# sandyresearch/chipmunk

Measured on AMD Instinct MI355X. Metric: DiT denoise steps/sec at fixed sparsity, higher is better.
Workload: dtype bf16

## Files before the change

chipmunk_amd/_native.py:

```python
from __future__ import annotations

import ctypes
import os

_HERE = os.path.dirname(os.path.abspath(__file__))
LIB_PATH = os.environ.get("CHIPMUNK_HIP_LIB") or os.path.join(_HERE, "lib", "libchipmunk_hip.so")

SYMBOLS = [
    "chipmunk_last_error", "chipmunk_abi_version", "chipmunk_set_option", "chipmunk_set_random_seed",
    "chipmunk_csp_attn", "chipmunk_csp_attn_out", "chipmunk_csp_128_attn", "chipmunk_dense_attn", "chipmunk_dense_colsum_attn",
    "chipmunk_csp_mlp_mm1", "chipmunk_csp_mlp_mm1_scatter", "chipmunk_csp_mlp_mm1_fp8", "chipmunk_csp_mlp_mm2_and_scatter_add", "chipmunk_csp_scatter_add", "chipmunk_csp_mlp_mm2",
    "chipmunk_csp_mlp_mm1_ragged", "chipmunk_csp_mlp_mm1_scatter_ragged", "chipmunk_csp_mlp_mm1_fp8_ragged", "chipmunk_csp_mlp_mm2_ragged",
    "chipmunk_csp_mlp_mm2_and_scatter_add_ragged", "chipmunk_csp_scatter_add_ragged", "chipmunk_block_mean_ragged", "chipmunk_transpose16_pitched",
    "chipmunk_csp_mlp_mm1_batched", "chipmunk_csp_mlp_mm1_scatter_batched", "chipmunk_csp_mlp_mm1_fp8_batched", "chipmunk_csp_mlp_mm2_batched",
    "chipmunk_csp_mlp_mm2_and_scatter_add_batched", "chipmunk_csp_scatter_add_batched",
    "chipmunk_topk_indices", "chipmunk_topk_delta_indices", "chipmunk_topk_mask", "chipmunk_mask_to_indices", "chipmunk_mask_to_sorted_indices", "chipmunk_packed_mask_to_indices", "chipmunk_mask_row_counts", "chipmunk_mask_to_ragged_indices", "chipmunk_copy_indices",
    "chipmunk_bitpack", "chipmunk_bitunpack", "chipmunk_transpose16", "chipmunk_block_mean", "chipmunk_quantize_fp8", "chipmunk_gather_rows", "chipmunk_qkv_split_norm", "chipmunk_split_heads_rownorm", "chipmunk_dense_colsum_topk_mask", "chipmunk_dense_attn_strided", "chipmunk_csp_attn_out_ragged", "chipmunk_compact_indices", "chipmunk_residual_ln_modulate", "chipmunk_dense_colsum_attn_strided", "chipmunk_dense_colsum_topk_mask_strided", "chipmunk_release_scratch", "chipmunk_big_scratch_fallbacks",
    "chipmunk_host_alloc", "chipmunk_host_free", "chipmunk_copy_d2h_async", "chipmunk_copy_h2d_async", "chipmunk_host_bytes",
]

_lib = None


def lib() -> ctypes.CDLL:
    global _lib
    if _lib is None:
        if not os.path.exists(LIB_PATH):
            raise ImportError(
                f"{LIB_PATH} is missing: build it with `python -m chipmunk_amd.build` (hipcc --offload-arch=gfx950). "
                "chipmunk_amd has no CPU fallback.")
        _lib = ctypes.CDLL(LIB_PATH)
        _lib.chipmunk_last_error.restype = ctypes.c_char_p
        _lib.chipmunk_abi_version.restype = ctypes.c_int
        for item in filter(None, os.environ.get("CHIPMUNK_AMD_OPTIONS", "").split(",")):
            name, _, val = item.partition("=")
            if _lib.chipmunk_set_option(name.strip().encode(), int(val)) != 0:
                raise ValueError(f"CHIPMUNK_AMD_OPTIONS: {_lib.chipmunk_last_error().decode()}")
    return _lib


def last_error() -> str:
    return lib().chipmunk_last_error().decode()


def check(rc: int, what: str) -> None:
    if rc != 0:
        raise RuntimeError(f"{what}: {last_error()}")


def set_option(name: str, value: int) -> None:
    check(lib().chipmunk_set_option(name.encode(), int(value)), "chipmunk_set_option")


def manual_seed(seed: int) -> None:
    check(lib().chipmunk_set_random_seed(ctypes.c_uint64(int(seed) & 0xFFFFFFFFFFFFFFFF)), "chipmunk_set_random_seed")


class HostBuffer:

    def __init__(self, numel: int, dtype) -> None:
        import torch
        self.dtype = dtype
        self._numel = int(numel)
        self._itemsize = torch.empty(0, dtype=dtype).element_size()
        self.nbytes = self._numel * self._itemsize
        p = ctypes.c_void_p()
        check(lib().chipmunk_host_alloc(ctypes.c_size_t(max(self.nbytes, 1)), ctypes.byref(p)), "chipmunk_host_alloc")
        self.ptr = p.value

# ... 36 lines not shown
```

chipmunk_amd/csrc/attn.hip:

```cpp
#include "common.h"
#include "attn_params.h"
#include <type_traits>

namespace {

constexpr int QG = 192;
constexpr int QW = 48;
constexpr int KVT = 32;
constexpr int NST = 4;
constexpr int KRING = 8;
constexpr int HD = 128;
constexpr int TILE_BYTES = KVT * HD * 2;
constexpr float SCALE_LOG2E = 0.08838834764f * 1.44269504089f;
constexpr int NSTV = NST + 1;
constexpr int KEY_RING_OFF = (NST + NSTV) * TILE_BYTES;
constexpr int CS_OFF = KEY_RING_OFF + KRING * 256;
constexpr int ATTN_LDS_BYTES = CS_OFF + 2 * 2 * 4 * KVT * 4;

__device__ __forceinline__ f32x4 mfma16(bf16x8 a, bf16x8 b, f32x4 c) {
    return __builtin_amdgcn_mfma_f32_16x16x32_bf16(a, b, c, 0, 0, 0);
}

#ifdef ATTN_PROF
__device__ unsigned long long g_attn_prof[8 * 8];
// ... 1162 lines not shown
    p.B = B, p.H = H, p.Nq = Nq, p.Nk = Nk, p.G = (Nq + QG - 1) / QG;
    p.o_scale = 1.f;
    hipStream_t st = (hipStream_t)stream;
    int rc;
    if (chipmunk_get_option("attn_fused_colsum") == 5) {
        if (use_colsum64(B, H, Nq, Nk)) return chipmunk_colsum64_launch(p, st);
        return launch_attn<false, false, false, true>(p, st);
    }
    if (use_dense64(B, H, Nq, Nk)) {
        CM_CHECK((int64_t)Nk * p.ks[2] * 2 < (1ll << 32) && (int64_t)Nk * p.vs[2] * 2 < (1ll << 32),
                 "attention: one head's K or V spans more than 4 GiB (32-bit DMA offsets)");
        if (chipmunk_get_option("attn_fused_colsum") != 2) {
            int hc = H;
            uint16_t *part = nullptr;
            const int hc_min = chipmunk_get_option("attn_fused_colsum") == 4 ? 1 : 0;
            if (hc_min) hc = 1;
            for (; hc >= 1; hc /= 2) {
                part = (uint16_t *)chipmunk_big_scratch(st, chipmunk_colsum_part_bytes(hc == H ? B : 1, hc, Nq, Nk));
                if (part) break;
            }
            if (part && hc == H) return chipmunk_dense64_colsum_launch(p, part, st);
            if (part) {
                for (int b = 0; b < B; ++b)
                    for (int h0 = 0; h0 < H; h0 += hc) {
                        AttnParams c = p;
                        const int hn = H - h0 < hc ? H - h0 : hc;
                        const int64_t bh0 = (int64_t)b * H + h0;
                        c.q += b * p.qs[0] + h0 * p.qs[1], c.k += b * p.ks[0] + h0 * p.ks[1], c.v += b * p.vs[0] + h0 * p.vs[1];
                        c.o += b * p.os[0] + h0 * p.os[1];
                        c.l_out += bh0 * Nq, c.p_in += bh0 * Nq, c.cs += bh0 * p.G * (int64_t)cs_stride;
                        c.B = 1, c.H = hn;
                        if (int e = chipmunk_dense64_colsum_launch(c, part, st)) return e;
                    }
                return CHIPMUNK_OK;
            }
        }
        rc = chipmunk_dense64_launch(q, k, v, o, l, p.qs, p.ks, p.vs, p.os, B, H, Nq, Nk, st);
    } else {
        rc = launch_attn<false, false, true>(p, st);
    }
    if (rc != CHIPMUNK_OK) return rc;
    if (use_colsum64(B, H, Nq, Nk)) return chipmunk_colsum64_launch(p, st);
    return launch_attn<false, false, false, true>(p, st);
}

extern "C" int chipmunk_dense_colsum_attn(const void *q, const void *k, const void *v, const int64_t q_strides[3],
                                          const int64_t k_strides[3], const int64_t v_strides[3], const float *pin,
                                          void *o, void *cs, float *l, int B, int H, int Nq, int Nk, int cs_stride,
                                          void *stream) {
    return chipmunk_dense_colsum_attn_strided(q, k, v, q_strides, k_strides, v_strides, pin, o, nullptr, cs, l, B, H, Nq, Nk,
                                              cs_stride, stream);
}

extern "C" int chipmunk_dense_colsum_topk_mask_strided(const void *q, const void *k, const void *v, const int64_t q_strides[3],
                                               const int64_t k_strides[3], const int64_t v_strides[3], const float *pin, void *o,
                                               const int64_t *o_strides, float *l, int B, int H, int Nq, int Nk, const void *static_mask,
                                               int64_t static_stride, int static_rows, const void *group_flags, void *mask,
                                               int topk, double random_amount, void *stream) {
    if (int e = check_common(q, k, v, o, B, H, Nq, Nk)) return e;
    CM_CHECK(l && pin && mask, "dense_colsum_topk_mask: p / l / mask missing");
    if (int e = check_strides(q_strides, "q")) return e;
    if (int e = check_strides(k_strides, "k")) return e;
    if (int e = check_strides(v_strides, "v")) return e;
    hipStream_t st = (hipStream_t)stream;
    if (!use_dense64(B, H, Nq, Nk) || chipmunk_get_option("attn_fused_colsum") == 2 || (Nk & 3) || Nk > CHIPMUNK_TOPK_MASK_MAX_N)
        return CHIPMUNK_ERR_UNSUPPORTED;
    AttnParams p = {};
    p.q = (const uint16_t *)q, p.k = (const uint16_t *)k, p.v = (const uint16_t *)v, p.o = (uint16_t *)o;
    for (int i = 0; i < 3; ++i) p.qs[i] = q_strides[i], p.ks[i] = k_strides[i], p.vs[i] = v_strides[i];
    CM_CHECK((int64_t)Nk * p.ks[2] * 2 < (1ll << 32) && (int64_t)Nk * p.vs[2] * 2 < (1ll << 32),
             "attention: one head's K or V spans more than 4 GiB (32-bit DMA offsets)");
    if (int e = output_strides(p.os, o_strides, H, Nq)) return e;
    p.l_out = l, p.p_in = pin, p.cs = nullptr, p.cs_stride = 0;
    p.B = B, p.H = H, p.Nq = Nq, p.Nk = Nk, p.G = (Nq + QG - 1) / QG;
    p.o_scale = 1.f;
    uint16_t *part = (uint16_t *)chipmunk_big_scratch(st, chipmunk_colsum_part_bytes(B, H, Nq, Nk));
    if (!part) return CHIPMUNK_ERR_UNSUPPORTED;
    if (int e = chipmunk_dense64_colsum_launch(p, part, st)) return e;
    const int nrb = ((Nq + 255) / 256) * 2;
    return chipmunk_topk_mask_parts(part, chipmunk_colsum_part_stride(Nk), nrb, p.G, Nq, static_mask, static_stride, static_rows, group_flags, mask, B * H * p.G, Nk,
                                    topk, random_amount, st);
}

extern "C" int chipmunk_dense_colsum_topk_mask(const void *q, const void *k, const void *v, const int64_t q_strides[3],
                                               const int64_t k_strides[3], const int64_t v_strides[3], const float *pin, void *o,
                                               float *l, int B, int H, int Nq, int Nk, const void *static_mask,
                                               int64_t static_stride, int static_rows, const void *group_flags, void *mask,
                                               int topk, double random_amount, void *stream) {
    return chipmunk_dense_colsum_topk_mask_strided(q, k, v, q_strides, k_strides, v_strides, pin, o, nullptr, l, B, H, Nq, Nk,
                                                   static_mask, static_stride, static_rows, group_flags, mask, topk, random_amount,
                                                   stream);
}
```

chipmunk_amd/csrc/attn64.hip:

```cpp
#include "common.h"
#include "attn64_regs.h"
#include "attn_params.h"
#include "attn64_util.h"
#include <type_traits>

namespace {

constexpr int HD = 128;
constexpr int KT = 64;
constexpr int WROWS = 64, WGROWS = 256;
constexpr int TB = KT * HD * 2;
constexpr int NSL = 4;
constexpr int VRING = NSL * TB;
constexpr int LDS_BYTES = 2 * NSL * TB;
constexpr int PSTAGE = 64 * 128;
constexpr int LDS_BYTES_CSUM = LDS_BYTES + 4 * PSTAGE;
constexpr int CS_EXCH_BYTES = 2 * 4 * 64 * 4;
constexpr float SCALE_LOG2E = 0.08838834764f * 1.44269504089f;
constexpr float MAX_LAG = 4.0f;
#ifndef A64_ABL
#define A64_ABL 0
#endif
#ifndef A64_EB
#define A64_EB 20
#endif
#ifndef A64_EA
#define A64_EA 35
#endif
#ifndef A64_CSUM_VALU
#define A64_CSUM_VALU 1
#endif
#ifndef A64_VSPREAD
#define A64_VSPREAD 0
#endif
#ifndef A64_DMA_POS
#define A64_DMA_POS 2
#endif

constexpr int a64_ecum(int k) {
    return k <= 0 ? 0 : k <= 20 ? (k * A64_EB) / 20 : k <= 52 ? A64_EB + ((k - 20) * A64_EA) / 32
                                                              : (A64_EB + A64_EA + (k - 52) < 64 ? A64_EB + A64_EA + (k - 52) : 64);
}
constexpr int a64_cstep(int j) {
    int k = 0;
    while (a64_ecum(k) < 2 * j + 2) ++k;
    return k;
}
constexpr int a64_rk(int u) { return u == 0 ? 36 : u == 1 ? 38 : u == 2 ? 68 : 70; }
constexpr int a64_mk(int u) { return u == 0 ? 46 : u == 1 ? 48 : u == 2 ? 78 : 80; }

#ifdef ATTN64_PROF
__device__ unsigned long long g_a64_prof[4 * 8];
#define P64_DECL unsigned long long pt_ = 0, pacc_[7] = {0, 0, 0, 0, 0, 0, 0}; const bool prof_on_ = blockIdx.x == (gridDim.x / 2)
#define P64_START() do { if (prof_on_) pt_ = __builtin_amdgcn_s_memtime(); } while (0)
#define P64_MARK(i) do { if (prof_on_) { const unsigned long long n_ = __builtin_amdgcn_s_memtime(); pacc_[i] += n_ - pt_; pt_ = n_; } } while (0)
#define P64_END(w, n) do { if (prof_on_ && lane == 0) { for (int i_ = 0; i_ < 7; ++i_) g_a64_prof[(w) * 8 + i_] = pacc_[i_]; g_a64_prof[(w) * 8 + 7] = (n); } } while (0)
#else
#define P64_DECL
#define P64_START()
#define P64_MARK(i)
#define P64_END(w, n)
#endif

template <int KB, int QB, int KS>
__device__ __forceinline__ void mfma_qk(f32x16 &s) {
    constexpr int ka = 192 + (KB * 8 + KS) * 4, qa = 128 + (QB * 8 + KS) * 4;
    if constexpr (A64_ABL & 64) {
        constexpr int oa = (KB * 2 + QB) * 16;
        asm volatile("v_mfma_f32_32x32x16_bf16 a[%c0:%c1], a[%c2:%c3], a[%c4:%c5], a[%c0:%c1]" ::"i"(oa), "i"(oa + 15), "i"(ka), "i"(ka + 3), "i"(qa), "i"(qa + 3));
        return;
    }
    if constexpr (KS == 0)
        asm volatile("v_mfma_f32_32x32x16_bf16 %0, a[%c1:%c2], a[%c3:%c4], 0" : "=v"(s) : "i"(ka), "i"(ka + 3), "i"(qa), "i"(qa + 3));
    else
        asm volatile("v_mfma_f32_32x32x16_bf16 %0, a[%c1:%c2], a[%c3:%c4], %0" : "+v"(s) : "i"(ka), "i"(ka + 3), "i"(qa), "i"(qa + 3));
}
template <int QB, int DB>
__device__ __forceinline__ void mfma_pv(const u32x4 &vf, const u32x4 &pf) {
    constexpr int oa = (QB * 4 + DB) * 16;
    asm volatile("v_mfma_f32_32x32x16_bf16 a[%c2:%c3], %0, %1, a[%c2:%c3]" ::"v"(vf), "v"(pf), "i"(oa), "i"(oa + 15));
}
template <int KB, int KS, int SLOT>
__device__ __forceinline__ void lds_k(uint32_t addr) {
// ... 201 lines not shown

    if constexpr (!GATHER) {
        issue_k(0, 0);
        issue_k(1, 1), issue_v(0, 3);
        issue_k(2, 2), issue_v(0, 0);
        issue_k(3, 3), issue_v(1, 1);
        asm volatile("s_waitcnt vmcnt(24)" ::: "memory");
    }
    __syncthreads();
    static_for<0, 16>([&](auto i) {
        constexpr int I = decltype(i)::value;
        lds_k<(I >> 3), (I & 7), 0>(kad[I & 7]);
    });
    asm volatile("s_waitcnt lgkmcnt(0)" ::: "memory");

    f32x16 s[4];
    float px[64];
    uint32_t pw[2][4][4] = {};
    float m[2] = {-INFINITY, -INFINITY}, nmsc[2] = {0.f, 0.f};
    float mlag[2] = {-INFINITY, -INFINITY};
    float lacc[2][2] = {{0.f, 0.f}, {0.f, 0.f}};
    float alpha[2] = {1.f, 1.f};
    float wq[2] = {0.f, 0.f}, lpq[2] = {-1.0e30f, -1.0e30f}, c4[2] = {0.f, 0.f}, c5 = 0.f;
    uint32_t csoff = 0, ex_w = 0, ex_r = 0;
    int cs_extra = 0;
    float cs_own = 0.f;
    __amdgpu_buffer_rsrc_t prsrc = krsrc;
    uint32_t pst_w = 0, pst_r = 0, csoff_mx = 0;
    u32x2 csf[8] = {};
    f32x4 csacc[2] = {{0.f, 0.f, 0.f, 0.f}, {0.f, 0.f, 0.f, 0.f}};
    float csout = 0.f;
    u32x4 cs_ones = {0x3f803f80u, 0x3f803f80u, 0x3f803f80u, 0x3f803f80u};
    if constexpr (CSUM) {
        static_assert(A64_CSUM_VALU, "the matrix-pipe column-sum probe (A64_CSUM_VALU=0) fills all 160 KiB of LDS with its P stage: no room for the exchange area of the in-workgroup combine; build round 5's tree for it");
        pin(cs_ones);
        const uint32_t pst = lds0 + LDS_BYTES + (uint32_t)w * PSTAGE;
        pst_w = pst + l31 * 128 + ((uint32_t)(hf ^ (l31 & 7)) << 4);
        const int prow = lg * 4 + (l15 >> 2);
        pst_r = pst + prow * 128 + ((uint32_t)(((l15 & 3) >> 1) ^ (prow & 7)) << 4) + (l15 & 1) * 8;
        csoff_mx = 2u * (uint32_t)(16 * lg + 8 * ((l15 >> 2) & 1) + 4 * (l15 >> 3) + (l15 & 3));
#pragma unroll
        for (int qb = 0; qb < 2; ++qb) {
            const int qrow = row0 + qb * 32 + l31;
            const float pl = qrow < p.Nq ? p.p_in[(int64_t)bh * p.Nq + qrow] : 0.f;
            lpq[qb] = pl > 0.f ? __builtin_amdgcn_logf(pl) : -1.0e30f;
        }
        const int rr = ((lane >> 4) & 1) | (((lane >> 3) & 1) << 1) | (((lane >> 2) & 1) << 2);
        csoff = 2u * (uint32_t)(32 * (lane & 1) + (rr & 3) + 8 * (2 * ((lane >> 1) & 1) + (rr >> 2)) + 4 * hf);
        const int nA = 3 - (4 * g) % 3;
        const int lead = w < nA ? 0 : nA, members = w < nA ? nA : 4 - nA;
        cs_extra = w == lead ? members : 0;
        ex_w = lds0 + LDS_BYTES + (uint32_t)w * 256u + (uint32_t)lane * 4u;
        ex_r = lds0 + LDS_BYTES + (uint32_t)(lead + 1) * 256u + (uint32_t)lane * 4u;
        prsrc = make_rsrc(p.cs_part + ((int64_t)bh * (p.G * 2) + (g * 2 + (w < nA ? 0 : 1))) * p.cs_pstride);
    }
#pragma unroll
    for (int e = 0; e < 64; ++e) px[e] = e < 20 ? 0.f : -INFINITY;

    auto vfrag_read = [&](auto dbc, auto offc) __attribute__((always_inline)) {
        constexpr int DB = decltype(dbc)::value, OFF = decltype(offc)::value;
        u32x2 lo, hi;
        asm volatile("ds_read_b64_tr_b16 %0, %2 offset:%c3\n\tds_read_b64_tr_b16 %1, %2 offset:%c4"
                     : "=&v"(lo), "=&v"(hi) : "v"(vad[DB]), "i"(OFF), "i"(OFF + 2048) : "memory");
        return (u32x4){lo[0], lo[1], hi[0], hi[1]};
    };

    static_assert(64 - A64_EB - A64_EA >= 0 && 64 - A64_EB - A64_EA <= 9, "the last steps must finish before gap 12 of the next PV phase");
    auto ecum = [](int k) constexpr { return a64_ecum(k); };
    auto finish_step = [&](auto kk, auto uwc) __attribute__((always_inline)) {
        constexpr int K = decltype(kk)::value;
        constexpr bool UW = decltype(uwc)::value != 0;
        if constexpr (!(A64_ABL & 1)) {
            static_for<ecum(K), ecum(K + 1)>([&](auto ii) {
                constexpr int I = decltype(ii)::value;
                if constexpr (A64_ABL & 32) px[I] = px[I] * 0.5f;
                else px[I] = __builtin_amdgcn_exp2f(px[I]);
                pin(px[I]);
            });
            static_for<ecum(K - 1), ecum(K)>([&](auto ii) {
                constexpr int I = decltype(ii)::value;
                lacc[(I >> 3) & 1][I & 1] += px[I];
                pin(lacc[(I >> 3) & 1][I & 1]);
            });
            static_for<(ecum(K - 1) >> 1), (ecum(K) >> 1)>([&](auto jj) {
                constexpr int J = decltype(jj)::value, I = 2 * J;
                pw[(I >> 3) & 1][I >> 4][(I & 7) >> 1] = pack_bf16x2(px[I], px[I + 1]);
                pin(pw[(I >> 3) & 1][I >> 4][(I & 7) >> 1]);
            });
            if constexpr (CSUM && UW && !A64_CSUM_VALU) {
                static_assert(a64_cstep(8 * 1 + 7) + 1 < a64_rk(0) && a64_cstep(8 * 3 + 7) + 1 < a64_rk(2), "a unit is read after its second fragment is stored");
                static_for<0, 4>([&](auto uu) {
                    constexpr int U = decltype(uu)::value, S = (U & 1) * 4;
                    if constexpr (K == a64_mk(U) || K == a64_mk(U) + 1) {
                        constexpr int H2 = K - a64_mk(U);
                        if constexpr (H2 == 0 && (U & 1) == 0)
                            asm volatile("s_waitcnt lgkmcnt(0)" : "+v"(csf[0]), "+v"(csf[1]), "+v"(csf[2]), "+v"(csf[3]), "+v"(csf[4]), "+v"(csf[5]), "+v"(csf[6]), "+v"(csf[7]) :: "memory");
                        const u32x4 fr = {csf[S + 2 * H2][0], csf[S + 2 * H2][1], csf[S + 2 * H2 + 1][0], csf[S + 2 * H2 + 1][1]};
                        if constexpr (H2 == 0) asm volatile("v_mfma_f32_16x16x32_bf16 %0, %1, %2, 0" : "=&v"(csacc[U & 1]) : "v"(cs_ones), "v"(fr));
                        else asm volatile("v_mfma_f32_16x16x32_bf16 %0, %1, %2, %0" : "+v"(csacc[U & 1]) : "v"(cs_ones), "v"(fr));
                    }
                    if constexpr (K == a64_mk(U) + 3) {
                        if constexpr (U == 0) csout = csacc[0][0];
                        else csout = lg == U ? csacc[U & 1][0] : csout;
                        pin(csout);
                    }
                    if constexpr (K == a64_rk(U) || K == a64_rk(U) + 1) {
                        constexpr int H2 = K - a64_rk(U);
// ... 57 lines not shown
        constexpr int KNSL = (SL + 1) & 3;
        uint32_t ldsw = w * 4096, ksoff = 0, vsoff = 0;
        if constexpr (!(A64_ABL & 16)) {
            if constexpr (!(A64_ABL & 256) && !GATHER) asm volatile("s_waitcnt vmcnt(16)" ::: "memory");
            if constexpr (!(A64_ABL & 128)) __builtin_amdgcn_s_barrier();
            if constexpr (!GATHER) {
                asm volatile("" : "+s"(ldsw));
                ksoff = (uint32_t)tile_base(t + 4) * kstride_b;
                vsoff = (uint32_t)tile_base(t + 2) * vstride_b;
            }
        }
        __builtin_amdgcn_sched_barrier(0);
        P64_MARK(0);

        u32x4 vf[16];
        static_for<0, 32>([&](auto gg) {
            constexpr int G = decltype(gg)::value;
            constexpr int ks = G >> 2, kb = (G >> 1) & 1, qb = G & 1;
            mfma_qk<kb, qb, ks>(s[kb * 2 + qb]);
            if constexpr (!(A64_ABL & 16) && !GATHER && ((A64_DMA_POS == 0 && G < 8) || (A64_DMA_POS == 2 && G >= 16 && (G & 1) == 0))) {
                constexpr int PC = A64_DMA_POS == 0 ? G : (G - 16) >> 1;
                if constexpr (PC < 4) issue_k1(ksoff, ldsw, SL, PC);
                else issue_v1(vsoff, ldsw, (SL + 2) & 3, PC - 4);
            }
            finish_step(ic<20 + G>{}, uwc);
            if constexpr (A64_VSPREAD ? (G & 1) == 0 : G < 16) {
                constexpr int f = A64_VSPREAD ? G >> 1 : G;
                if constexpr (A64_ABL & 4) vf[f] = (u32x4){(uint32_t)t, 1u, 2u, 3u};
                else vf[f] = vfrag_read(ic<(f & 3)>{}, ic<VSL * TB + (f >> 2) * 4096>{});
            }
            __builtin_amdgcn_sched_barrier(0);
        });
        P64_MARK(1);
        asm volatile("s_waitcnt lgkmcnt(0)"
                     : "+v"(vf[0]), "+v"(vf[1]), "+v"(vf[2]), "+v"(vf[3]), "+v"(vf[4]), "+v"(vf[5]), "+v"(vf[6]), "+v"(vf[7]), "+v"(vf[8]),
                       "+v"(vf[9]), "+v"(vf[10]), "+v"(vf[11]), "+v"(vf[12]), "+v"(vf[13]), "+v"(vf[14]), "+v"(vf[15]));
        __builtin_amdgcn_sched_barrier(0);
        P64_MARK(2);

        float mx[2];
        bool moved = false;
        const int dead = GATHER ? 0 : (t * KT - tile_base(t) < KT ? t * KT - tile_base(t) : KT);
        const int vleft = !GATHER ? KT : (t < ntiles ? valid - (tbeg + t) * KT : 0);
        auto phase_b_gap = [&](auto gg) __attribute__((always_inline)) {
            constexpr int G = decltype(gg)::value;
            constexpr int up = G >> 3, db = (G >> 1) & 3, qb = G & 1;
            const u32x4 pf = {pw[qb][up][0], pw[qb][up][1], pw[qb][up][2], pw[qb][up][3]};
            mfma_pv<qb, db>(vf[G >> 1], pf);
            constexpr bool UWT = decltype(uwc)::value != 0 && !A64_CSUM_VALU;
            if constexpr (G < (CSUM ? (UWT ? 32 : 17) : 12)) finish_step(ic<52 + G>{}, uwc);
            if constexpr (CSUM && G == (UWT ? 31 : 17)) {
                const uint32_t par2 = (uint32_t)(t & 1) * 1024u;
                const float mine = UWT ? csout : c5;
                if (!cs_extra) {
                    asm volatile("ds_write_b32 %0, %1" ::"v"(ex_w + (par2 ^ 1024u)), "v"(mine) : "memory");
                } else {
                    float x1 = 0.f, x2 = 0.f;
                    if (cs_extra >= 2) asm volatile("ds_read_b32 %0, %1" : "=v"(x1) : "v"(ex_r + par2) : "memory");
                    if (cs_extra >= 3) asm volatile("ds_read_b32 %0, %1 offset:256" : "=v"(x2) : "v"(ex_r + par2) : "memory");
                    asm volatile("ds_write_b32 %0, %1" ::"v"(ex_w + (par2 ^ 1024u)), "v"(mine) : "memory");
                    asm volatile("s_waitcnt lgkmcnt(1)" : "+v"(x1), "+v"(x2)::"memory");
                    const int tb2 = tile_base(t - 2), dd = (t - 2) * KT - tb2;
                    if (t > 1 && dd < KT) {
                        const uint32_t off = UWT ? csoff_mx : csoff;
                        if (dd <= 0 || (int)(off >> 1) >= dd) {
                            const uint16_t val = (uint16_t)(pack_bf16x2((cs_own + x1) + x2, 0.f) & 0xffffu);
                            if (p.probe & 16) __builtin_amdgcn_raw_buffer_store_b16(val, prsrc, off, (uint32_t)tb2 * 2u, 2);
                            else __builtin_amdgcn_raw_buffer_store_b16(val, prsrc, off, (uint32_t)tb2 * 2u, 0);
                        }
                    }
                }
                cs_own = mine;
            }
            if constexpr (!(A64_ABL & 16) && !GATHER && A64_DMA_POS == 1 && G >= 16 && (G & 1) == 0) {
                constexpr int PC = (G - 16) >> 1;
                if constexpr (PC < 4) issue_k1(ksoff, ldsw, SL, PC);
                else issue_v1(vsoff, ldsw, (SL + 2) & 3, PC - 4);
            }
            if constexpr (G < 16 && !(A64_ABL & 8)) {
                constexpr int J = G;
                lds_k<(J >> 3), (J & 7), KNSL>(kad[J & 7]);
            }
            if constexpr (G == 1 && !(A64_ABL & 2)) {
                if (!GATHER && __builtin_expect(dead > 0, 0)) {
                    int thr = dead - 4 * hf;
                    asm volatile("" : "+v"(thr));
#pragma unroll
                    for (int blk = 0; blk < 4; ++blk)
#pragma unroll
                        for (int r = 0; r < 16; ++r)
                            if ((blk >> 1) * 32 + (r & 3) + 8 * (r >> 2) < thr) s[blk][r] = -INFINITY;
                }
                if (GATHER && __builtin_expect(vleft < KT, 0)) {
                    int thr = vleft - hf;
                    asm volatile("" : "+v"(thr));
#pragma unroll
                    for (int blk = 0; blk < 4; ++blk)
#pragma unroll
                        for (int r = 0; r < 16; ++r)
                            if ((r & 3) * 16 + (blk >> 1) * 8 + 2 * (r >> 2) >= thr) s[blk][r] = -INFINITY;
                }
            }
            if constexpr (G >= 2 && G <= 9 && !(A64_ABL & 2) && !NOMAX) {
                constexpr int j = G - 2;
                constexpr int kb2 = j >> 2, r0 = (j & 3) * 4;
                if constexpr (j == 0)
                    asm volatile("v_max_f32 %0, %2, %3\n\tv_max_f32 %1, %6, %7\n\tv_max3_f32 %0, %0, %4, %5\n\tv_max3_f32 %1, %1, %8, %9"
                                 : "=&v"(mx[0]), "=&v"(mx[1])
                                 : "v"(s[0][0]), "v"(s[0][1]), "v"(s[0][2]), "v"(s[0][3]), "v"(s[1][0]), "v"(s[1][1]), "v"(s[1][2]), "v"(s[1][3]));
                else
                asm volatile("v_max3_f32 %0, %0, %2, %3\n\tv_max3_f32 %1, %1, %6, %7\n\tv_max3_f32 %0, %0, %4, %5\n\tv_max3_f32 %1, %1, %8, %9"
                             : "+v"(mx[0]), "+v"(mx[1])
                             : "v"(s[kb2 * 2][r0]), "v"(s[kb2 * 2][r0 + 1]), "v"(s[kb2 * 2][r0 + 2]), "v"(s[kb2 * 2][r0 + 3]),
                               "v"(s[kb2 * 2 + 1][r0]), "v"(s[kb2 * 2 + 1][r0 + 1]), "v"(s[kb2 * 2 + 1][r0 + 2]), "v"(s[kb2 * 2 + 1][r0 + 3]));
            }
            if constexpr (G == 10 && !(A64_ABL & 2) && !NOMAX) {
#pragma unroll
                for (int q2 = 0; q2 < 2; ++q2) {
                    float a = mx[q2], c = mx[q2];
                    lane_swap32(a, c);
                    mx[q2] = max2(a, c);
                    pin(mx[q2]);
                }
            }
// ... 311 lines not shown
        uint32_t ldsw = w * 4096;
        asm volatile("" : "+s"(ldsw));
        const uint32_t ksoff = (uint32_t)tile_base(t + 4) * kstride_b;
        __builtin_amdgcn_sched_barrier(0);
        static_for<0, 6>([&](auto qq) {
            constexpr int QB = decltype(qq)::value;
            constexpr int PP = SL * 6 + QB;
            constexpr int BUF = PP % 3, B1 = (PP + 2) % 3, B2 = (PP + 1) % 3;
            static_for<0, 16>([&](auto gg) {
                constexpr int G = decltype(gg)::value, ks = G >> 1, kb = G & 1;
                mfma_cs<QB, kb, ks>(s[BUF][kb], offs[QB]);
                if constexpr (QB == 0 && G >= 8 && G < 12) issue_k1(ksoff, ldsw, SL, G - 8);
                if constexpr (QB == 5 && kb == 1) {
                    lds_k<0, ks, KNSL>(kad[ks]);
                    lds_k<1, ks, KNSL>(kad[ks]);
                }
                constexpr int TP1 = QB == 0 ? TP ^ 1 : TP, TP2 = QB <= 1 ? TP ^ 1 : TP;
                if constexpr (G > 2) drain2(ic<B1>{}, ic<TP1>{}, ic<(G - 2) * 2>{}, ic<TP1>{}, ic<(G - 3) * 2>{});
                else if constexpr (G == 2) drain2(ic<B1>{}, ic<TP1>{}, ic<0>{}, ic<TP2>{}, ic<30>{});
                else if constexpr (G == 1) drain2(ic<B2>{}, ic<TP2>{}, ic<30>{}, ic<TP2>{}, ic<28>{});
                else drain2(ic<B2>{}, ic<TP2>{}, ic<28>{}, ic<TP2>{}, ic<26>{});
                if constexpr (QB == 1 && G == 3) {
                    float a = cacc[TP ^ 1][0], c = cacc[TP ^ 1][1];
                    lane_swap32(a, c);
                    const float tot = a + c;
                    cacc[TP ^ 1][0] = 0.f, cacc[TP ^ 1][1] = 0.f;
                    if (g < p.G && t > 0)
                    {
                        const uint32_t u = __float_as_uint(tot);
                        const uint32_t rne = (u + 0x7fffu + ((u >> 16) & 1u)) >> 16, qn = (u >> 16) | 0x0040u;
                        p.cs[((int64_t)bh * p.G + g) * p.cs_stride + tile_base(t - 1) + lane] = (uint16_t)((u & 0x7fffffffu) > 0x7f800000u ? qn : rne);
                    }
                }
                __builtin_amdgcn_sched_barrier(0);
            });
        });
        asm volatile("s_waitcnt lgkmcnt(0)" ::: "memory");
        __builtin_amdgcn_sched_barrier(0);
    };
    for (int tb = 0;; tb += 4) {
        tile(ic<0>{}, tb);
        if (tb >= T4) break;
        tile(ic<1>{}, tb + 1);
        tile(ic<2>{}, tb + 2);
        tile(ic<3>{}, tb + 3);
    }
    asm volatile("s_waitcnt vmcnt(0)" ::: "memory");
}

template <int MODE>
int launch64(const AttnParams &p, int64_t grid, hipStream_t stream) {
    auto kern = attn64_kernel<MODE>;
    static uint64_t lds_set = 0;
    constexpr int LDS = (MODE == 3 && !A64_CSUM_VALU) ? LDS_BYTES_CSUM + CS_EXCH_BYTES : MODE == 3 ? LDS_BYTES + CS_EXCH_BYTES : LDS_BYTES;
    ensure_dynamic_lds((const void *)kern, LDS, lds_set);
    hipLaunchKernelGGL(kern, dim3((unsigned)grid), dim3(256), LDS, stream, p);
    CM_LAUNCH_CHECK();
    return CHIPMUNK_OK;
}

}

#ifdef ATTN64_PROF
extern "C" int chipmunk_attn64_prof_read(unsigned long long *out) {
    return hipMemcpyFromSymbol(out, HIP_SYMBOL(g_a64_prof), sizeof(g_a64_prof)) == hipSuccess ? 0 : 2;
}
#endif

const float *chipmunk_knorm_max(const uint16_t *k, const int64_t ks[3], int B, int H, int Nk, hipStream_t stream) {
    if (chipmunk_get_option("attn_nomax") == 2 || (size_t)B * H * sizeof(float) > (32 << 10)) return nullptr;
    unsigned char *sc = (unsigned char *)chipmunk_scratch(stream, 64 << 10);
    if (!sc) return nullptr;
    float *km = (float *)(sc + (32 << 10));
    if (hipMemsetAsync(km, 0, (size_t)B * H * sizeof(float), stream) != hipSuccess) return nullptr;
    hipLaunchKernelGGL(knorm_max_kernel, dim3(Nk >= 4096 ? 64 : 8, B * H), dim3(256), 0, stream, k, ks[0], ks[1], ks[2], H, Nk, km);
    return km;
}

int chipmunk_dense64_launch(const void *q, const void *k, const void *v, void *o, float *l, const int64_t qs[3],
                            const int64_t ks[3], const int64_t vs[3], const int64_t os[3], int B, int H, int Nq, int Nk,
                            hipStream_t stream) {
    AttnParams p = {};
    p.q = (const uint16_t *)q, p.k = (const uint16_t *)k, p.v = (const uint16_t *)v, p.o = (uint16_t *)o;
    for (int i = 0; i < 3; ++i) p.qs[i] = qs[i], p.ks[i] = ks[i], p.vs[i] = vs[i], p.os[i] = os[i];
    p.l_out = l;
    p.B = B, p.H = H, p.Nq = Nq, p.Nk = Nk, p.G = (Nq + WGROWS - 1) / WGROWS;
    p.o_scale = 1.f;
    p.kmax = chipmunk_knorm_max(p.k, ks, B, H, Nk, stream);
    return launch64<0>(p, (int64_t)B * H * p.G, stream);
}

namespace {
__global__ __launch_bounds__(256) void cs_combine_kernel(const uint16_t *part, int pstride, uint16_t *cs, int NRB, int G, int Nq, int Nk, int cs_stride) {
    const int g = blockIdx.y, bh = blockIdx.z;
    int r0, r1;
    const int nrows = colsum_part_rows(g, NRB / 2, r0, r1);
    const uint16_t *src = part + ((int64_t)bh * NRB + r0) * pstride;
    const int64_t row1 = (int64_t)(r1 - r0) * pstride;
    uint16_t *dst = cs + ((int64_t)bh * G + g) * cs_stride;
    if (((Nk | cs_stride) & 3) == 0) {
        const int j = (blockIdx.x * 256 + threadIdx.x) * 4;
        if (j >= Nk) return;
        float acc[4];
        {
            const u32x2 x = *(const u32x2 *)(src + j);
            acc[0] = __uint_as_float(x[0] << 16), acc[1] = __uint_as_float(x[0] & 0xffff0000u);
            acc[2] = __uint_as_float(x[1] << 16), acc[3] = __uint_as_float(x[1] & 0xffff0000u);
        }
        if (nrows == 2) {
            const u32x2 x = *(const u32x2 *)(src + row1 + j);
            acc[0] += __uint_as_float(x[0] << 16), acc[1] += __uint_as_float(x[0] & 0xffff0000u);
            acc[2] += __uint_as_float(x[1] << 16), acc[3] += __uint_as_float(x[1] & 0xffff0000u);
        }
        *(u32x2 *)(dst + j) = (u32x2){pack_bf16x2(acc[0], acc[1]), pack_bf16x2(acc[2], acc[3])};
    } else {
        for (int e = 0; e < 4; ++e) {
            const int j = (blockIdx.x * 256 + threadIdx.x) * 4 + e;
            if (j >= Nk) return;
            float acc = bf16_bits_to_f32(src[j]);
            if (nrows == 2) acc += bf16_bits_to_f32(src[row1 + j]);
            dst[j] = f32_to_bf16_bits(acc);
        }
    }
}
}

int chipmunk_colsum64_launch(const AttnParams &p, hipStream_t stream) {
    static uint64_t lds_set = 0;
    ensure_dynamic_lds((const void *)colsum64_kernel, NSL * TB, lds_set);
    const int64_t grid = (int64_t)p.B * p.H * ((p.G + 3) / 4);
    hipLaunchKernelGGL(colsum64_kernel, dim3((unsigned)grid), dim3(256), NSL * TB, stream, p);
    CM_LAUNCH_CHECK();
    return CHIPMUNK_OK;
}

int chipmunk_colsum_part_stride(int Nk) { return (chipmunk_get_option("attn_cs_probe") & 1) ? Nk : (Nk + 63) & ~63; }

size_t chipmunk_colsum_part_bytes(int B, int H, int Nq, int Nk) {
    return (size_t)B * H * (((Nq + WGROWS - 1) / WGROWS) * 2) * (size_t)chipmunk_colsum_part_stride(Nk) * sizeof(uint16_t);
}

int chipmunk_dense64_colsum_launch(const AttnParams &p0, uint16_t *part, hipStream_t stream) {
    AttnParams p = p0;
    const int G192 = p.G;
    p.G = (p.Nq + WGROWS - 1) / WGROWS;
    p.cs_part = part, p.cs_pstride = chipmunk_colsum_part_stride(p.Nk);
    if (chipmunk_get_option("attn_cs_probe") & 2) p.probe |= 16;
    if (chipmunk_get_option("attn_fused_colsum") == 3) p.probe |= 4;
    p.kmax = chipmunk_knorm_max(p.k, p.ks, p.B, p.H, p.Nk, stream);
    if (int rc = launch64<3>(p, (int64_t)p.B * p.H * p.G, stream)) return rc;
    if (!p.cs) return CHIPMUNK_OK;
    hipLaunchKernelGGL(cs_combine_kernel, dim3((unsigned)((p.Nk + 1023) / 1024), (unsigned)G192, (unsigned)(p.B * p.H)), dim3(256), 0, stream,
                       part, p.cs_pstride, p.cs, p.G * 2, G192, p.Nq, p.Nk, p.cs_stride);
    CM_LAUNCH_CHECK();
    return CHIPMUNK_OK;
}

int chipmunk_csp64_launch(const AttnParams &p, int inplace, int grid, hipStream_t stream) {
    CM_CHECK(p.plan && p.tickets && p.ws, "csp64: work plan missing");
    return inplace ? launch64<2>(p, grid, stream) : launch64<1>(p, grid, stream);
}
```

chipmunk_amd/csrc/attn_params.h:

```cpp
#pragma once
#include <stdint.h>
#include <hip/hip_runtime.h>

struct AttnParams {
    const uint16_t *q, *k, *v;
    uint16_t *o;
    const uint16_t *o_in;
    int64_t qs[3], ks[3], vs[3], os[3];
    const int32_t *indices, *counts;
    const int64_t *idx_off;
    float *l_out;
    const float *p_in;
    uint16_t *cs;
    int cs_stride;
    int B, H, Nq, Nk, G, idx_stride;
    float o_scale;
    int split_full, nsplit;
    float *ws;
    int32_t *tickets;
    const int32_t *plan;
    int xcd_chunks;
    const float *kmax;
    uint16_t *cs_part;
    int cs_pstride;
    int probe;
};


int chipmunk_csp64_launch(const AttnParams &p, int inplace, int grid, hipStream_t stream);
int chipmunk_dense64_colsum_launch(const AttnParams &p, uint16_t *part, hipStream_t stream);
int chipmunk_topk_mask_parts(const uint16_t *part, int part_stride, int nrb, int groups_per_bh, int Nq, const void *static_mask, int64_t static_stride,
                             int static_rows, const void *group_flags, void *mask, int rows, int n, int k, double random_amount,
                             hipStream_t stream);
size_t chipmunk_colsum_part_bytes(int B, int H, int Nq, int Nk);
int chipmunk_colsum_part_stride(int Nk);
int chipmunk_colsum64_launch(const AttnParams &p, hipStream_t stream);
int chipmunk_csp96_launch(const AttnParams &p, int inplace, int grid, hipStream_t stream);
const float *chipmunk_knorm_max(const uint16_t *k, const int64_t ks[3], int B, int H, int Nk, hipStream_t stream);

__host__ __device__ inline int colsum_part_rows(int j, int nwg, int &r0, int &r1) {
    const int a = (3 * j) >> 2, w0 = 3 * j - 4 * a;
    r0 = 2 * a + (w0 ? 1 : 0);
    r1 = 2 * (a + 1);
    return (w0 >= 2 && a + 1 < nwg) ? 2 : 1;
}

struct IndexRow {
    const int32_t *ptr;
    int width;
};
__device__ __forceinline__ IndexRow index_row(const AttnParams &p, int64_t item) {
    if (p.idx_off) {
        const int64_t o = p.idx_off[item];
        return {p.indices + o, (int)(p.idx_off[item + 1] - o)};
    }
    return {p.indices + item * p.idx_stride, p.idx_stride};
}
```

chipmunk_amd/csrc/indexed_io.hip:

```cpp
#include "common.h"
#include "attn_params.h"

namespace {

__device__ __forceinline__ uint32_t wave_incl_scan(uint32_t x) {
    x += (uint32_t)__builtin_amdgcn_update_dpp(0, (int)x, 0x111, 0xf, 0xf, true);
    x += (uint32_t)__builtin_amdgcn_update_dpp(0, (int)x, 0x112, 0xf, 0xf, true);
    x += (uint32_t)__builtin_amdgcn_update_dpp(0, (int)x, 0x114, 0xf, 0xf, true);
    x += (uint32_t)__builtin_amdgcn_update_dpp(0, (int)x, 0x118, 0xf, 0xf, true);
    x += (uint32_t)__builtin_amdgcn_update_dpp(0, (int)x, 0x142, 0xa, 0xf, false);
    x += (uint32_t)__builtin_amdgcn_update_dpp(0, (int)x, 0x143, 0xc, 0xf, false);
    return x;
}
struct M2IParams {
    const uint8_t *mask;
    int32_t *indices;
    int32_t *counts;
    int n, pad_n, multiple_of;
    const int64_t *offsets;
};

template <bool PACKED, bool SORTED = false, bool RAGGED = false>
__global__ __launch_bounds__(256) void mask_to_indices_kernel(const M2IParams p) {
    extern __shared__ __attribute__((aligned(16))) unsigned char smem[];
// ... 485 lines not shown
    int32_t *dst = flat + o;
    const int width = (int)(offsets[r + 1] - o);
    int c = counts[r];
    c = c < 0 ? 0 : (c < width ? c : width);
    c = c < idx_stride ? c : (int)idx_stride;
    if ((((uintptr_t)src | (uintptr_t)dst) & 15) == 0) {
        const int c4 = c >> 2;
        for (int i = threadIdx.x; i < c4; i += 256) ((u32x4 *)dst)[i] = ((const u32x4 *)src)[i];
        for (int i = (c4 << 2) + threadIdx.x; i < c; i += 256) dst[i] = src[i];
    } else {
        for (int i = threadIdx.x; i < c; i += 256) dst[i] = src[i];
    }
    for (int i = c + threadIdx.x; i < width; i += 256) dst[i] = 0;
}

size_t m2i_lds_bytes(int n, bool sorted) {
    const int NI = (n + 31) >> 5, NB = (NI + 63) >> 6;
    if (sorted) return (size_t)NB * 64 * 4 + (size_t)(NB + 1) * 4 + 16;
    return (size_t)NB * 64 * 4 + (size_t)32 * NB * 8 + (size_t)32 * NB * 4 + 33 * 4 + 16;
}

template <bool PACKED, bool SORTED = false, bool RAGGED = false>
int launch_m2i(const void *mask, int32_t *indices, int32_t *counts, int64_t rows, int n, int pad_n, int multiple_of,
               void *stream, const int64_t *offsets = nullptr) {
    CM_CHECK(mask && indices && (RAGGED ? (const void *)offsets : (const void *)counts), "mask_to_indices: null pointer");
    CM_CHECK(rows >= 0 && n > 0 && pad_n >= n && multiple_of > 0, "mask_to_indices: bad sizes rows=%lld n=%d pad_n=%d multiple_of=%d",
             (long long)rows, n, pad_n, multiple_of);
    CM_CHECK(rows < (1ll << 31), "mask_to_indices: too many rows");
    if (PACKED) CM_CHECK(n % 8 == 0, "packed_mask_to_indices: n must be a multiple of 8 (got %d)", n);
    const size_t lds = m2i_lds_bytes(n, SORTED);
    CM_CHECK(lds <= 160 * 1024, "mask_to_indices: row length %d needs %zu B of LDS (> 160 KiB)", n, lds);
    if (rows == 0) return CHIPMUNK_OK;
    auto kern = mask_to_indices_kernel<PACKED, SORTED, RAGGED>;
    if (lds > 64 * 1024) (void)hipFuncSetAttribute((const void *)kern, hipFuncAttributeMaxDynamicSharedMemorySize, (int)lds);
    M2IParams p = {(const uint8_t *)mask, indices, counts, n, pad_n, multiple_of, offsets};
    hipLaunchKernelGGL(kern, dim3((unsigned)rows), dim3(256), lds, (hipStream_t)stream, p);
    CM_LAUNCH_CHECK();
    return CHIPMUNK_OK;
}


struct TopkMaskParams {
    const uint16_t *cs;
    const uint8_t *stat;
    const uint8_t *groups;
    uint8_t *mask;
    int64_t cs_stride, stat_stride;
    int rows, n, k, stat_rows;
    float random_amount;
    uint32_t salt;
    const uint16_t *parts;
    int64_t pstride;
    int nrb, ngroups, nq;
};

__device__ __forceinline__ uint32_t bf16_key(uint32_t u) {
    return (u & 0x8000u) ? (~u & 0xffffu) : (u | 0x8000u);
}

template <int KPT, bool ALIGNED, bool PARTS = false>
__global__ __launch_bounds__(1024) void topk_mask_kernel(const TopkMaskParams p) {
    constexpr int NV = KPT / 4;
    __shared__ int wave_cnt[16];
    const int tid = threadIdx.x, lane = tid & 63, w = tid >> 6;
    const int row = blockIdx.x;
    const int n = p.n;
    const uint16_t *x = nullptr;
    int prow = 1;
    int64_t row1 = 0;
    if constexpr (PARTS) {
        const int bh = row / p.ngroups, g = row - bh * p.ngroups;
        int r0, r1;
        prow = colsum_part_rows(g, p.nrb / 2, r0, r1);
        x = p.parts + ((int64_t)bh * p.nrb + r0) * p.pstride;
        row1 = (int64_t)(r1 - r0) * p.pstride;
    } else {
        x = p.cs + (int64_t)row * p.cs_stride;
    }
    const uint32_t lane_off8 = 8u * (uint32_t)tid;
    const uint32_t lane_off4 = 4u * (uint32_t)tid;
    uint32_t key[NV][2];
    constexpr int LB = NV % 10 == 0 ? 10 : (NV % 8 == 0 ? 8 : (NV % 6 == 0 ? 6 : 4));
    static_assert(NV % LB == 0, "NV must split into whole load batches");
#pragma unroll
    for (int j0 = 0; j0 < NV; j0 += LB) {
        uint32_t raw[LB][2];
#pragma unroll
        for (int jj = 0; jj < LB; ++jj) {
            const int c = 4 * tid + 4096 * (j0 + jj);
            uint32_t v0 = 0xffffffffu, v1 = 0xffffffffu;
            if constexpr (ALIGNED) {
                if (c < n) {
                    const u32x2 v = *(const u32x2 *)((const unsigned char *)(x + 4096 * (j0 + jj)) + lane_off8);
                    v0 = v[0], v1 = v[1];
                    if constexpr (PARTS) {
                        if (prow == 2) {
                            float a0 = __uint_as_float(v0 << 16), a1 = __uint_as_float(v0 & 0xffff0000u);
                            float a2 = __uint_as_float(v1 << 16), a3 = __uint_as_float(v1 & 0xffff0000u);
                            const u32x2 y = *(const u32x2 *)((const unsigned char *)(x + row1 + 4096 * (j0 + jj)) + lane_off8);
                            a0 += __uint_as_float(y[0] << 16), a1 += __uint_as_float(y[0] & 0xffff0000u);
                            a2 += __uint_as_float(y[1] << 16), a3 += __uint_as_float(y[1] & 0xffff0000u);
                            v0 = pack_bf16x2(a0, a1), v1 = pack_bf16x2(a2, a3);
                        }
                    }
                }
            } else if (c < n) {
                v0 = v1 = 0;
#pragma unroll
                for (int e = 0; e < 4; ++e) {
                    const uint32_t u = c + e < n ? x[c + e] : 0xffffu;
                    if (e < 2) v0 |= u << (16 * e);
                    else v1 |= u << (16 * (e - 2));
                }
            }
// ... 28 lines not shown
            const uint32_t cm1 = (cand - 1u) | ((cand - 1u) << 16);
            const uint32_t one2 = 0x00010001u;
            uint32_t cnt2 = 0;
#pragma unroll
            for (int j = 0; j < NV; ++j)
#pragma unroll
                for (int h = 0; h < 2; ++h) {
                    uint32_t d;
                    asm volatile("v_pk_sub_u16 %0, %1, %2 clamp\n\tv_pk_min_u16 %0, %0, %3" : "=&v"(d) : "v"(key[j][h]), "v"(cm1), "v"(one2));
                    asm volatile("v_pk_add_u16 %0, %0, %1" : "+v"(cnt2) : "v"(d));
                }
            const int mine = (int)(cnt2 & 0xffffu) + (int)(cnt2 >> 16);
            if (block_count(mine) >= k) res = cand;
        }
        thr = res;
        int gt = 0;
#pragma unroll
        for (int j = 0; j < NV; ++j)
#pragma unroll
            for (int h = 0; h < 2; ++h) {
                uint32_t kw = key[j][h];
                asm volatile("" : "+v"(kw));
                gt += ((kw & 0xffffu) > thr ? 1 : 0) + ((kw >> 16) > thr ? 1 : 0);
            }
        ties_to_take = k - block_count(gt);
    }
    int my_ties = 0;
    if (ties_to_take > 0) {
#pragma unroll
        for (int j = 0; j < NV; ++j)
#pragma unroll
            for (int h = 0; h < 2; ++h) {
                uint32_t kw = key[j][h];
                asm volatile("" : "+v"(kw));
                my_ties += ((kw & 0xffffu) == thr ? 1 : 0) + ((kw >> 16) == thr ? 1 : 0);
            }
    }
    int tie_budget = 0;
    {
        int incl = my_ties;
#pragma unroll
        for (int d = 1; d < 64; d <<= 1) {
            const int o = __shfl_up(incl, d);
            if (lane >= d) incl += o;
        }
        if (lane == 63) wave_cnt[w] = incl;
        __syncthreads();
        int before = incl - my_ties;
#pragma unroll
        for (int i = 0; i < 16; ++i) before += i < w ? wave_cnt[i] : 0;
        __syncthreads();
        tie_budget = ties_to_take - before;
    }
    uint8_t *out = p.mask + (int64_t)row * n;
    const uint8_t *st = p.stat ? p.stat + (int64_t)(row % p.stat_rows) * p.stat_stride : nullptr;
    const bool rnd = active && p.random_amount > 0.f;
    auto combined4 = [&](int c0, uint32_t &v0, uint32_t &v1) {
        const u32x2 v = *(const u32x2 *)(x + c0);
        v0 = v[0], v1 = v[1];
        if constexpr (PARTS) {
            float a0 = __uint_as_float(v0 << 16), a1 = __uint_as_float(v0 & 0xffff0000u);
            float a2 = __uint_as_float(v1 << 16), a3 = __uint_as_float(v1 & 0xffff0000u);
            if (prow == 2) {
                const u32x2 y = *(const u32x2 *)(x + row1 + c0);
                a0 += __uint_as_float(y[0] << 16), a1 += __uint_as_float(y[0] & 0xffff0000u);
                a2 += __uint_as_float(y[1] << 16), a3 += __uint_as_float(y[1] & 0xffff0000u);
            }
            v0 = pack_bf16x2(a0, a1), v1 = pack_bf16x2(a2, a3);
        }
    };
    uint32_t first = x[0];
    if constexpr (PARTS) {
        uint32_t f0, f1;
        combined4(0, f0, f1);
        first = f0 & 0xffffu;
    }
    const uint32_t salt = p.salt ^ (first * 0x27D4EB2Fu);
    const int nsteps = (n + 4095) / 4096;
    auto emit = [&](auto keyed, int c, uint32_t v0, uint32_t v1, uint32_t sb) {
        uint32_t bytes = 0;
        if constexpr (decltype(keyed)::value) asm volatile("" : "+v"(v0), "+v"(v1));
#pragma unroll
        for (int e = 0; e < 4; ++e) {
            const uint32_t half = ((e < 2 ? v0 : v1) >> (16 * (e & 1))) & 0xffffu;
            const uint32_t kv = decltype(keyed)::value ? half : bf16_key(half);
            bool keep = kv > thr;
            const bool tie = kv == thr && tie_budget > 0 && c + e < n;
            tie_budget -= tie ? 1 : 0;
            keep = keep || tie;
            if (rnd && !keep) keep = hash_uniform(row, c + e, salt) < p.random_amount;
            keep = keep || ((sb >> (8 * e)) & 0xffu) != 0;
            bytes |= (keep ? 1u : 0u) << (8 * e);
        }
        if constexpr (ALIGNED) {
            *(uint32_t *)(out + c) = bytes;
        } else {
#pragma unroll
            for (int e = 0; e < 4; ++e)
                if (c + e < n) out[c + e] = (uint8_t)(bytes >> (8 * e));
        }
    };
    if constexpr (ALIGNED) {
        constexpr int OB = 5;
#pragma unroll
        for (int j0 = 0; j0 < NV; j0 += OB) {
            uint32_t sbv[OB];
#pragma unroll
            for (int jj = 0; jj < OB; ++jj) {
                const int c = 4 * tid + 4096 * (j0 + jj);
                sbv[jj] = (j0 + jj < NV && st && c < n) ? *(const uint32_t *)(st + c) : 0u;
            }
            __builtin_amdgcn_sched_barrier(0);
#pragma unroll
            for (int jj = 0; jj < OB; ++jj) {
                if constexpr (true) {
                    const int c = 4 * tid + 4096 * (j0 + jj);
                    if (j0 + jj < NV && c < n) emit(std::integral_constant<int, 1>{}, c, key[(j0 + jj) < NV ? (j0 + jj) : 0][0], key[(j0 + jj) < NV ? (j0 + jj) : 0][1], sbv[jj]);
                    asm volatile("" ::: "memory");
                }
            }
            __builtin_amdgcn_sched_barrier(0);
        }
    } else {
        for (int j = 0; j < nsteps; ++j) {
            const int c = 4 * tid + 4096 * j;
            if (c >= n) break;
            uint32_t v0 = 0, v1 = 0, sb = 0;
#pragma unroll
            for (int e = 0; e < 4; ++e) {
                const uint32_t u = c + e < n ? x[c + e] : 0xffffu;
                if (e < 2) v0 |= u << (16 * e);
                else v1 |= u << (16 * (e - 2));
                if (st && c + e < n) sb |= (uint32_t)st[c + e] << (8 * e);
            }
            emit(std::integral_constant<int, 0>{}, c, v0, v1, sb);
        }
    }
}

__device__ __forceinline__ uint32_t bf16_key2(uint32_t u) {
    uint32_t s;
    const uint32_t fifteen2 = 0x000f000fu;
    asm("v_pk_ashrrev_i16 %0, %1, %2" : "=v"(s) : "v"(fifteen2), "v"(u));
    return u ^ (s | 0x80008000u);
}

template <bool ALIGNED, bool PARTS>
__global__ __launch_bounds__(1024) void topk_mask_stream_kernel(const TopkMaskParams p) {
    __shared__ int wave_cnt[16];
    const int tid = threadIdx.x, lane = tid & 63, w = tid >> 6;
    const int row = blockIdx.x;
    const int n = p.n;
    const uint16_t *x = nullptr;
    int prow = 1;
    int64_t row1 = 0;
    if constexpr (PARTS) {
        const int bh = row / p.ngroups, g = row - bh * p.ngroups;
        int r0, r1;
        prow = colsum_part_rows(g, p.nrb / 2, r0, r1);
        x = p.parts + ((int64_t)bh * p.nrb + r0) * p.pstride;
        row1 = (int64_t)(r1 - r0) * p.pstride;
    } else {
        x = p.cs + (int64_t)row * p.cs_stride;
    }
    const uint32_t lane_off8 = 8u * (uint32_t)tid;
    const int nsteps = (n + 4095) / 4096;
    const bool active = p.groups == nullptr || p.groups[row] != 0;
    const int k = p.k < n ? p.k : n;
    const bool select = active && k > 0;
    const bool rnd = active && p.random_amount > 0.f;

    auto combined4 = [&](int c0, uint32_t &v0, uint32_t &v1) {
        const u32x2 v = *(const u32x2 *)(x + c0);
        v0 = v[0], v1 = v[1];
        if constexpr (PARTS) {
            if (prow == 2) {
                float a0 = __uint_as_float(v0 << 16), a1 = __uint_as_float(v0 & 0xffff0000u);
                float a2 = __uint_as_float(v1 << 16), a3 = __uint_as_float(v1 & 0xffff0000u);
                const u32x2 y = *(const u32x2 *)(x + row1 + c0);
                a0 += __uint_as_float(y[0] << 16), a1 += __uint_as_float(y[0] & 0xffff0000u);
                a2 += __uint_as_float(y[1] << 16), a3 += __uint_as_float(y[1] & 0xffff0000u);
                v0 = pack_bf16x2(a0, a1), v1 = pack_bf16x2(a2, a3);
            }
        }
    };
    uint32_t first = 0;
    if (rnd) {
        first = x[0];
        if constexpr (PARTS) {
            uint32_t f0, f1;
            combined4(0, f0, f1);
            first = f0 & 0xffffu;
        }
    }
    const uint32_t salt = p.salt ^ (first * 0x27D4EB2Fu);
    if constexpr (PARTS) {
        __syncthreads();
        if (select) {
            uint16_t *xk = const_cast<uint16_t *>(x);
            for (int j = 0; j < nsteps; ++j) {
                const int c = 4 * tid + 4096 * j;
// ... 55 lines not shown
            for (int j0 = 0; j0 < nsteps; j0 += U) {
                uint32_t kw[U][2];
#pragma unroll
                for (int jj = 0; jj < U; ++jj) load_raw(j0 + jj, kw[jj][0], kw[jj][1]);
#pragma unroll
                for (int jj = 0; jj < U; ++jj) {
                    to_keys(kw[jj][0], kw[jj][1]);
#pragma unroll
                    for (int h = 0; h < 2; ++h) {
                        uint32_t d;
                        asm volatile("v_pk_sub_u16 %0, %1, %2 clamp\n\tv_pk_min_u16 %0, %0, %3" : "=&v"(d) : "v"(kw[jj][h]), "v"(cm1), "v"(one2));
                        asm volatile("v_pk_add_u16 %0, %0, %1" : "+v"(cnt2) : "v"(d));
                    }
                }
            }
            const int mine = (int)(cnt2 & 0xffffu) + (int)(cnt2 >> 16);
            if (block_count(mine) >= k) res = cand;
        }
        thr = res;
        int gt = 0;
        for (int j0 = 0; j0 < nsteps; j0 += U) {
            uint32_t kw[U][2];
#pragma unroll
            for (int jj = 0; jj < U; ++jj) load_raw(j0 + jj, kw[jj][0], kw[jj][1]);
#pragma unroll
            for (int jj = 0; jj < U; ++jj) {
                to_keys(kw[jj][0], kw[jj][1]);
#pragma unroll
                for (int h = 0; h < 2; ++h) {
                    const uint32_t lo = kw[jj][h] & 0xffffu, hi = kw[jj][h] >> 16;
                    gt += (lo > thr ? 1 : 0) + (hi > thr ? 1 : 0);
                    my_ties += (lo == thr ? 1 : 0) + (hi == thr ? 1 : 0);
                }
            }
        }
        ties_to_take = k - block_count(gt);
    }
    int tie_budget = 0;
    {
        int incl = my_ties;
#pragma unroll
        for (int d = 1; d < 64; d <<= 1) {
            const int o = __shfl_up(incl, d);
            if (lane >= d) incl += o;
        }
        if (lane == 63) wave_cnt[w] = incl;
        __syncthreads();
        int before = incl - my_ties;
#pragma unroll
        for (int i = 0; i < 16; ++i) before += i < w ? wave_cnt[i] : 0;
        __syncthreads();
        tie_budget = ties_to_take - before;
    }
    uint8_t *out = p.mask + (int64_t)row * n;
    const uint8_t *st = p.stat ? p.stat + (int64_t)(row % p.stat_rows) * p.stat_stride : nullptr;
    for (int j0 = 0; j0 < nsteps; j0 += U) {
        uint32_t kw[U][2], sbv[U];
#pragma unroll
        for (int jj = 0; jj < U; ++jj) {
            const int c = 4 * tid + 4096 * (j0 + jj);
            kw[jj][0] = kw[jj][1] = 0;
            if (select) load_raw(j0 + jj, kw[jj][0], kw[jj][1]);
            sbv[jj] = 0;
            if constexpr (ALIGNED) {
                if (st && c < n) sbv[jj] = *(const uint32_t *)(st + c);
            } else if (st) {
#pragma unroll
                for (int e = 0; e < 4; ++e)
                    if (c + e < n) sbv[jj] |= (uint32_t)st[c + e] << (8 * e);
            }
        }
#pragma unroll
        for (int jj = 0; jj < U; ++jj) {
            const int c = 4 * tid + 4096 * (j0 + jj);
            if (c >= n) continue;
            if (select) to_keys(kw[jj][0], kw[jj][1]);
            uint32_t bytes = 0;
#pragma unroll
            for (int e = 0; e < 4; ++e) {
                const uint32_t kv = (kw[jj][e >> 1] >> (16 * (e & 1))) & 0xffffu;
                bool keep = kv > thr;
                const bool tie = kv == thr && tie_budget > 0 && c + e < n;
                tie_budget -= tie ? 1 : 0;
                keep = keep || tie;
                if (rnd && !keep) keep = hash_uniform(row, c + e, salt) < p.random_amount;
                keep = keep || ((sbv[jj] >> (8 * e)) & 0xffu) != 0;
                bytes |= (keep ? 1u : 0u) << (8 * e);
            }
            if constexpr (ALIGNED) {
                *(uint32_t *)(out + c) = bytes;
            } else {
#pragma unroll
                for (int e = 0; e < 4; ++e)
                    if (c + e < n) out[c + e] = (uint8_t)(bytes >> (8 * e));
            }
        }
    }
}

}

extern "C" int chipmunk_mask_to_indices(const void *mask, int32_t *indices, int32_t *counts, int64_t rows, int n,
                                        int pad_n, int multiple_of, void *stream) {
    return launch_m2i<false>(mask, indices, counts, rows, n, pad_n, multiple_of, stream);
}

extern "C" int chipmunk_packed_mask_to_indices(const void *packed, int32_t *indices, int32_t *counts, int64_t rows,
                                               int n, int pad_n, int multiple_of, void *stream) {
    return launch_m2i<true>(packed, indices, counts, rows, n, pad_n, multiple_of, stream);
}

static int launch_topk(const void *activation, void *cache, int dtype, int32_t *indices, int32_t *counts, int rows,
                       int cols, double sparsity_amount, int multiple_of, double random_amount, void *stream) {
    CM_CHECK(activation && indices && counts, "topk_indices: null pointer");
    CM_CHECK(rows >= 0 && cols >= 1024, "topk_indices: rows >= 0 and cols >= 1024 required (the quantile is taken over the first 1024 columns); got rows=%d cols=%d", rows, cols);
    CM_CHECK(multiple_of > 0, "topk_indices: multiple_of must be positive");
    CM_CHECK(sparsity_amount >= 0.0 && sparsity_amount <= 1.0, "topk_indices: sparsity_amount must be in [0,1]");
    if (rows == 0) return CHIPMUNK_OK;
    TopkParams p = {activation, cache, indices, counts, rows, cols, multiple_of, (float)sparsity_amount, (float)random_amount,
                    random_amount > 0.0 ? chipmunk_next_random_salt() : 0u};
    hipStream_t s = (hipStream_t)stream;
#define LAUNCH_TOPK(T)                                                                                           \
    do {                                                                                                         \
        if (cache) hipLaunchKernelGGL((topk_indices_kernel<T, true>), dim3(rows), dim3(1024), 0, s, p);          \
        else hipLaunchKernelGGL((topk_indices_kernel<T, false>), dim3(rows), dim3(1024), 0, s, p);               \
    } while (0)
    switch (dtype) {
        case CHIPMUNK_DTYPE_BF16: LAUNCH_TOPK(uint16_t); break;
        case CHIPMUNK_DTYPE_FP16: LAUNCH_TOPK(_Float16); break;
        case CHIPMUNK_DTYPE_FP32: LAUNCH_TOPK(float); break;
        default: CM_CHECK(false, "topk_indices: unsupported dtype code %d", dtype);
    }
#undef LAUNCH_TOPK
    CM_LAUNCH_CHECK();
    return CHIPMUNK_OK;
}

extern "C" int chipmunk_mask_to_sorted_indices(const void *mask, int packed, int32_t *indices, int32_t *counts,
                                               int64_t rows, int n, int pad_n, int multiple_of, void *stream) {
    return packed ? launch_m2i<true, true>(mask, indices, counts, rows, n, pad_n, multiple_of, stream)
                  : launch_m2i<false, true>(mask, indices, counts, rows, n, pad_n, multiple_of, stream);
}

extern "C" int chipmunk_mask_row_counts(const void *mask, int packed, int32_t *counts, int64_t *lengths, int64_t rows, int n,
                                        int pad_n, int multiple_of, void *stream) {
    CM_CHECK(mask && counts && lengths, "mask_row_counts: null pointer");
    CM_CHECK(rows >= 0 && n > 0 && pad_n >= n && multiple_of > 0, "mask_row_counts: bad sizes rows=%lld n=%d pad_n=%d multiple_of=%d",
             (long long)rows, n, pad_n, multiple_of);
    CM_CHECK(rows < (1ll << 31), "mask_row_counts: too many rows");
// ... 75 lines not shown

extern "C" int chipmunk_transpose16(const void *src, void *dst, int B, int R, int C, void *stream) {
    CM_CHECK(src && dst && B > 0 && R > 0 && C > 0, "transpose16: bad arguments");
    CM_CHECK((C & 7) == 0 || true, "unreachable");
    hipLaunchKernelGGL(transpose16_kernel, dim3((C + 63) / 64, (R + 63) / 64, B), dim3(256), 0, (hipStream_t)stream,
                       (const uint16_t *)src, (uint16_t *)dst, R, C, R);
    CM_LAUNCH_CHECK();
    return CHIPMUNK_OK;
}

extern "C" int chipmunk_transpose16_pitched(const void *src, void *dst, int B, int R, int C, int ld, void *stream) {
    CM_CHECK(src && dst && B > 0 && R > 0 && C > 0, "transpose16: bad arguments");
    CM_CHECK(ld >= R, "transpose16: the output pitch ld (%d) must be at least R (%d)", ld, R);
    hipLaunchKernelGGL(transpose16_kernel, dim3((C + 63) / 64, (ld + 63) / 64, B), dim3(256), 0, (hipStream_t)stream,
                       (const uint16_t *)src, (uint16_t *)dst, R, C, ld);
    CM_LAUNCH_CHECK();
    return CHIPMUNK_OK;
}

template <typename V>
__global__ __launch_bounds__(256) void gather_rows_kernel(const V *src, V *dst, const int32_t *map, int64_t n_out,
                                                          int64_t n_src, int64_t cpr, int64_t total) {
    for (int64_t idx = (int64_t)blockIdx.x * 256 + threadIdx.x; idx < total; idx += (int64_t)gridDim.x * 256) {
        const int64_t row = idx / cpr, c = idx - row * cpr;
        const int64_t o = row / n_out, r = row - o * n_out;
        dst[idx] = src[(o * n_src + map[r]) * cpr + c];
    }
}

extern "C" int chipmunk_gather_rows(const void *src, void *dst, const int32_t *map, int64_t outer, int64_t n_src,
                                    int64_t n_out, int64_t row_bytes, void *stream) {
    CM_CHECK(src && dst && map, "gather_rows: null pointer");
    CM_CHECK(outer >= 0 && n_src > 0 && n_out >= 0 && row_bytes > 0, "gather_rows: bad sizes");
    if (outer == 0 || n_out == 0) return CHIPMUNK_OK;
    hipStream_t s = (hipStream_t)stream;
    const uintptr_t align = (uintptr_t)src | (uintptr_t)dst | (uintptr_t)row_bytes;
#define LAUNCH_GATHER(V)                                                                                              \
    do {                                                                                                              \
        const int64_t cpr = row_bytes / (int64_t)sizeof(V), total = outer * n_out * cpr;                               \
        const int64_t blocks = (total + 255) / 256;                                                                    \
        hipLaunchKernelGGL((gather_rows_kernel<V>), dim3((unsigned)(blocks > 65536 * 16 ? 65536 * 16 : blocks)),       \
                           dim3(256), 0, s, (const V *)src, (V *)dst, map, n_out, n_src, cpr, total);                  \
    } while (0)
    if ((align & 15) == 0) LAUNCH_GATHER(u32x4);
    else if ((align & 3) == 0) LAUNCH_GATHER(uint32_t);
    else if ((align & 1) == 0) LAUNCH_GATHER(uint16_t);
    else LAUNCH_GATHER(uint8_t);
#undef LAUNCH_GATHER
    CM_LAUNCH_CHECK();
    return CHIPMUNK_OK;
}

int chipmunk_topk_mask_parts(const uint16_t *part, int part_stride, int nrb, int groups_per_bh, int Nq, const void *static_mask, int64_t static_stride,
                             int static_rows, const void *group_flags, void *mask, int rows, int n, int k, double random_amount,
                             hipStream_t s) {
    CM_CHECK(part && mask && rows >= 0 && n > 0 && (n & 3) == 0 && n <= CHIPMUNK_TOPK_MASK_MAX_N && k >= 0 && part_stride >= n && (part_stride & 3) == 0, "topk_mask_parts: bad arguments");
    CM_CHECK(!static_mask || (static_rows > 0 && static_stride >= n && (static_stride & 3) == 0 && ((uintptr_t)static_mask & 3) == 0),
             "topk_mask_parts: bad static mask geometry");
    CM_CHECK(((uintptr_t)mask & 3) == 0 && ((uintptr_t)part & 7) == 0, "topk_mask_parts: unaligned buffers");
    if (rows == 0) return CHIPMUNK_OK;
    TopkMaskParams p = {nullptr, (const uint8_t *)static_mask, (const uint8_t *)group_flags, (uint8_t *)mask, 0, static_stride,
                        rows, n, k, static_mask ? static_rows : 1, (float)random_amount,
                        random_amount > 0.0 ? chipmunk_next_random_salt() : 0u};
    p.parts = part, p.pstride = part_stride, p.nrb = nrb, p.ngroups = groups_per_bh, p.nq = Nq;
    if (n > 1024 * 120 || chipmunk_get_option("topk_mask_stream") == 1) hipLaunchKernelGGL((topk_mask_stream_kernel<true, true>), dim3(rows), dim3(1024), 0, s, p);
    else if (n <= 1024 * 16) hipLaunchKernelGGL((topk_mask_kernel<16, true, true>), dim3(rows), dim3(1024), 0, s, p);
    else if (n <= 1024 * 48) hipLaunchKernelGGL((topk_mask_kernel<48, true, true>), dim3(rows), dim3(1024), 0, s, p);
    else hipLaunchKernelGGL((topk_mask_kernel<120, true, true>), dim3(rows), dim3(1024), 0, s, p);
    CM_LAUNCH_CHECK();
    return CHIPMUNK_OK;
}

__global__ __launch_bounds__(256) void qkv_split_norm_kernel(const uint16_t *qkv, int64_t row_stride, const uint16_t *qw,
                                                             const uint16_t *kw, uint16_t *q, uint16_t *k, uint16_t *v, int64_t n,
                                                             int H, float eps, int64_t segments, const float *fcos, const float *fsin,
                                                             int64_t rope_rows) {
    const int l15 = threadIdx.x & 15;
    u32x4 wq = {0x3f803f80u, 0x3f803f80u, 0x3f803f80u, 0x3f803f80u}, wk = wq;
    if (qw) wq = *(const u32x4 *)(qw + l15 * 8);
    if (kw) wk = *(const u32x4 *)(kw + l15 * 8);
    for (int64_t seg = ((int64_t)blockIdx.x * 256 + threadIdx.x) >> 4; seg < segments; seg += ((int64_t)gridDim.x * 256) >> 4) {
        const int64_t tok = seg / (3 * H);
        const int rem = (int)(seg - tok * 3 * H), which = rem / H, h = rem - which * H;
        u32x4 x = *(const u32x4 *)(qkv + tok * row_stride + (int64_t)rem * 128 + l15 * 8);
        uint16_t *dst = (which == 0 ? q : which == 1 ? k : v) + ((int64_t)h * n + tok) * 128 + l15 * 8;
        if (which < 2) {
            float f[8], ss = 0.f;
#pragma unroll
            for (int e = 0; e < 4; ++e) {
                f[2 * e] = __uint_as_float(x[e] << 16), f[2 * e + 1] = __uint_as_float(x[e] & 0xffff0000u);
                ss = __builtin_fmaf(f[2 * e], f[2 * e], ss);
                ss = __builtin_fmaf(f[2 * e + 1], f[2 * e + 1], ss);
            }
            ss = row16_sum(ss);
            const float r = 1.0f / __builtin_sqrtf(ss * (1.0f / 128.0f) + eps);
            const u32x4 w = which == 0 ? wq : wk;
#pragma unroll
            for (int e = 0; e < 4; ++e) {
                float a = f[2 * e] * r, b = f[2 * e + 1] * r;
                round_bf16_pair(a, b);
                x[e] = pack_bf16x2(a * __uint_as_float(w[e] << 16), b * __uint_as_float(w[e] & 0xffff0000u));
            }
            if (fcos && tok < rope_rows) {
                const f32x4 c0 = *(const f32x4 *)(fcos + tok * 128 + l15 * 8), c1 = *(const f32x4 *)(fcos + tok * 128 + l15 * 8 + 4);
                const f32x4 s0 = *(const f32x4 *)(fsin + tok * 128 + l15 * 8), s1 = *(const f32x4 *)(fsin + tok * 128 + l15 * 8 + 4);
#pragma unroll
                for (int e = 0; e < 4; ++e) {
                    const float re = __uint_as_float(x[e] << 16), im = __uint_as_float(x[e] & 0xffff0000u);
                    const float cr = e < 2 ? c0[2 * e] : c1[2 * e - 4], ci = e < 2 ? c0[2 * e + 1] : c1[2 * e - 3];
                    const float sr = e < 2 ? s0[2 * e] : s1[2 * e - 4], si = e < 2 ? s0[2 * e + 1] : s1[2 * e - 3];
                    x[e] = pack_bf16x2(re * cr + (-im) * sr, im * ci + re * si);
                }
            }
        }
        *(u32x4 *)dst = x;
    }
}

extern "C" int chipmunk_qkv_split_norm(const void *qkv, int64_t row_stride, const void *q_weight, const void *k_weight, void *q,
                                       void *k, void *v, int64_t n, int heads, float eps, const float *freqs_cos,
                                       const float *freqs_sin, int64_t rope_rows, void *stream) {
    CM_CHECK(qkv && q && k && v, "qkv_split_norm: null pointer");
    CM_CHECK(n >= 0 && heads > 0 && row_stride >= (int64_t)3 * heads * 128, "qkv_split_norm: bad sizes");
    CM_CHECK((((uintptr_t)qkv | (uintptr_t)q | (uintptr_t)k | (uintptr_t)v | (uintptr_t)q_weight | (uintptr_t)k_weight) & 15) == 0 &&
                 (row_stride & 7) == 0 && (((uintptr_t)freqs_cos | (uintptr_t)freqs_sin) & 15) == 0,
             "qkv_split_norm: pointers and the row stride must be 16-byte aligned");
    CM_CHECK((freqs_cos == nullptr) == (freqs_sin == nullptr) && rope_rows >= 0 && rope_rows <= n, "qkv_split_norm: bad rotary arguments");
    if (n == 0) return CHIPMUNK_OK;
    const int64_t segments = n * 3 * heads, blocks = (segments + 15) / 16;
    hipLaunchKernelGGL(qkv_split_norm_kernel, dim3((unsigned)(blocks > 256 * 64 ? 256 * 64 : blocks)), dim3(256), 0, (hipStream_t)stream,
                       (const uint16_t *)qkv, row_stride, (const uint16_t *)q_weight, (const uint16_t *)k_weight, (uint16_t *)q,
                       (uint16_t *)k, (uint16_t *)v, n, heads, eps, segments, freqs_cos, freqs_sin, freqs_cos ? rope_rows : 0);
    CM_LAUNCH_CHECK();
    return CHIPMUNK_OK;
}

extern "C" int chipmunk_topk_mask(const void *cs, int64_t cs_stride, const void *static_mask, int64_t static_stride,
                                  int static_rows, const void *group_flags, void *mask, int rows, int n, int k,
                                  double random_amount, void *stream) {
    CM_CHECK(cs && mask, "topk_mask: null pointer");
    CM_CHECK(rows >= 0 && n > 0 && k >= 0, "topk_mask: bad sizes (rows=%d n=%d k=%d)", rows, n, k);
    CM_CHECK(cs_stride >= n, "topk_mask: cs row stride %lld < n %d", (long long)cs_stride, n);
    CM_CHECK(n <= CHIPMUNK_TOPK_MASK_MAX_N, "topk_mask: rows of more than %d columns are not supported (got %d)", CHIPMUNK_TOPK_MASK_MAX_N, n);
    CM_CHECK(!static_mask || (static_rows > 0 && static_stride >= n), "topk_mask: bad static mask geometry");
    CM_CHECK(random_amount >= 0.0 && random_amount <= 1.0, "topk_mask: random_amount must be in [0,1]");
    if (rows == 0) return CHIPMUNK_OK;
    TopkMaskParams p = {(const uint16_t *)cs, (const uint8_t *)static_mask, (const uint8_t *)group_flags, (uint8_t *)mask,
                        cs_stride, static_stride, rows, n, k, static_mask ? static_rows : 1, (float)random_amount,
                        random_amount > 0.0 ? chipmunk_next_random_salt() : 0u};
    hipStream_t s = (hipStream_t)stream;
    const bool aligned = n % 4 == 0 && (((uintptr_t)cs) & 7) == 0 && (cs_stride * 2) % 8 == 0 && (((uintptr_t)mask) & 3) == 0 &&
                         (!static_mask || ((((uintptr_t)static_mask) & 3) == 0 && static_stride % 4 == 0));
#define LAUNCH_TM(KPT)                                                                                       \
    do {                                                                                                     \
        if (aligned) hipLaunchKernelGGL((topk_mask_kernel<KPT, true>), dim3(rows), dim3(1024), 0, s, p);     \
        else hipLaunchKernelGGL((topk_mask_kernel<KPT, false>), dim3(rows), dim3(1024), 0, s, p);            \
    } while (0)
    if (n > 1024 * 120 || chipmunk_get_option("topk_mask_stream") == 1) {
        if (aligned) hipLaunchKernelGGL((topk_mask_stream_kernel<true, false>), dim3(rows), dim3(1024), 0, s, p);
        else hipLaunchKernelGGL((topk_mask_stream_kernel<false, false>), dim3(rows), dim3(1024), 0, s, p);
    } else if (n <= 1024 * 16) LAUNCH_TM(16);
    else if (n <= 1024 * 48) LAUNCH_TM(48);
    else LAUNCH_TM(120);
#undef LAUNCH_TM
    CM_LAUNCH_CHECK();
    return CHIPMUNK_OK;
}

extern "C" int chipmunk_compact_indices(const int32_t *indices, int64_t idx_stride, const int32_t *counts, const int64_t *offsets,
                                        int32_t *flat, int64_t rows, void *stream) {
    CM_CHECK(indices && counts && offsets && flat, "compact_indices: null pointer");
    CM_CHECK(rows >= 0 && rows < (1ll << 31) && idx_stride > 0, "compact_indices: bad sizes rows=%lld idx_stride=%lld", (long long)rows,
             (long long)idx_stride);
    if (rows == 0) return CHIPMUNK_OK;
    hipLaunchKernelGGL(compact_indices_kernel, dim3((unsigned)rows), dim3(256), 0, (hipStream_t)stream, indices, idx_stride, counts,
                       offsets, flat);
    CM_LAUNCH_CHECK();
    return CHIPMUNK_OK;
}
```

chipmunk_amd/csrc/torch_registry.cpp:

```cpp
#include <ATen/ATen.h>
#include <ATen/hip/impl/HIPStreamMasqueradingAsCUDA.h>
#include <Python.h>
#include <c10/core/DeviceGuard.h>
#include <torch/library.h>

#include <vector>

#include "../../include/chipmunk_hip.h"

extern "C" {
PyObject *PyInit_cuda(void) {
    static struct PyModuleDef module_def = {PyModuleDef_HEAD_INIT, "cuda", NULL, -1, NULL};
    return PyModule_Create(&module_def);
}
}

namespace chipmunk {
namespace {

void *cur_stream(const at::Tensor &t) {
    return (void *)c10::hip::getCurrentHIPStreamMasqueradingAsCUDA(t.device().index()).stream();
}
void check(int rc, const char *op) { TORCH_CHECK(rc == 0, "chipmunk::", op, ": ", chipmunk_last_error()); }

// ... 620 lines not shown
}

std::vector<at::Tensor> mask_to_sorted_indices(at::Tensor mask, at::IntArrayRef shape, int64_t multiple_of,
                                               int64_t pad_to_multiple_of) {
    CHECK_DEV(mask);
    const bool packed = mask.scalar_type() == at::kByte;
    TORCH_CHECK(packed || mask.scalar_type() == at::kBool, "mask must be bool, or uint8 bit-packed with a shape");
    mask = mask.contiguous();
    std::vector<int64_t> shp = packed ? shape.vec() : mask.sizes().vec();
    TORCH_CHECK(shp.size() == 4, "shape must be [b, h, m, n]");
    const int64_t b = shp[0], h = shp[1], m = shp[2], n = shp[3];
    if (packed) TORCH_CHECK(n % 8 == 0 && mask.numel() * 8 >= b * h * m * n, "bad packed mask");
    const int64_t pad_n = ((n + pad_to_multiple_of - 1) / pad_to_multiple_of) * pad_to_multiple_of;
    c10::DeviceGuard guard(mask.device());
    at::Tensor indices = at::empty({b, h, m, pad_n}, mask.options().dtype(at::kInt));
    at::Tensor counts = at::empty({b, h, m}, mask.options().dtype(at::kInt));
    check(chipmunk_mask_to_sorted_indices(mask.data_ptr(), packed ? 1 : 0, indices.data_ptr<int>(),
                                          counts.data_ptr<int>(), b * h * m, (int)n, (int)pad_n, (int)multiple_of,
                                          cur_stream(mask)),
          "mask_to_sorted_indices");
    return {indices, counts};
}

std::vector<at::Tensor> mask_to_ragged_indices(at::Tensor mask, at::IntArrayRef shape, int64_t multiple_of, int64_t pad_to_multiple_of,
                                               bool sorted) {
    CHECK_DEV(mask);
    const bool packed = mask.scalar_type() == at::kByte;
    TORCH_CHECK(packed || mask.scalar_type() == at::kBool, "mask must be bool, or uint8 bit-packed with a shape");
    TORCH_CHECK(multiple_of > 0 && pad_to_multiple_of > 0, "multiple_of and pad_to_multiple_of must be positive");
    mask = mask.contiguous();
    std::vector<int64_t> shp = packed ? shape.vec() : mask.sizes().vec();
    TORCH_CHECK(shp.size() == 4, "shape must be [b, h, m, n]");
    const int64_t b = shp[0], h = shp[1], m = shp[2], n = shp[3], rows = b * h * m;
    if (packed) TORCH_CHECK(n % 8 == 0 && mask.numel() * 8 >= rows * n, "bad packed mask");
    const int64_t pad_n = ((n + pad_to_multiple_of - 1) / pad_to_multiple_of) * pad_to_multiple_of;
    TORCH_CHECK(n > 0 && pad_n <= INT_MAX, "rows must have between 1 and 2^31 - 1 columns");
    c10::DeviceGuard guard(mask.device());
    at::Tensor counts = at::empty({b, h, m}, mask.options().dtype(at::kInt));
    at::Tensor len = at::empty({rows}, mask.options().dtype(at::kLong));
    check(chipmunk_mask_row_counts(mask.data_ptr(), packed ? 1 : 0, counts.data_ptr<int>(), len.data_ptr<int64_t>(), rows, (int)n,
                                   (int)pad_n, (int)multiple_of, cur_stream(mask)),
          "mask_to_ragged_indices");
    at::Tensor offsets = at::zeros({rows + 1}, len.options());
    if (rows) offsets.narrow(0, 1, rows).copy_(len.cumsum(0));
    const int64_t total = rows ? offsets[rows].item<int64_t>() : 0;
    at::Tensor flat = at::empty({total + 64}, counts.options());
    flat.narrow(0, total, 64).zero_();
    check(chipmunk_mask_to_ragged_indices(mask.data_ptr(), packed ? 1 : 0, sorted ? 1 : 0, offsets.data_ptr<int64_t>(), flat.data_ptr<int>(),
                                          rows, (int)n, (int)multiple_of, cur_stream(mask)),
          "mask_to_ragged_indices");
    return {flat, offsets, counts};
}

std::vector<at::Tensor> dense_colsum_attn_layout(at::Tensor q, at::Tensor k, at::Tensor v, at::Tensor p, bool token_major_o);
at::Tensor topk_mask(at::Tensor cs, int64_t k, double random_amount, const c10::optional<at::Tensor> &groups,
                     const c10::optional<at::Tensor> &static_mask);
std::vector<at::Tensor> dense_colsum_topk_mask(at::Tensor q, at::Tensor k, at::Tensor v, at::Tensor p, int64_t k_top, double random_amount,
                                               const c10::optional<at::Tensor> &groups, const c10::optional<at::Tensor> &static_mask,
                                               bool token_major_o) {
    CHECK_DEV(q); CHECK_DEV(k); CHECK_DEV(v); CHECK_DEV(p);
    CHECK_BF16(q); CHECK_BF16(k); CHECK_BF16(v);
    const bool shapes_ok = q.dim() == 4 && k.dim() == 4 && v.dim() == 4 && q.size(3) == 128 && q.stride(3) == 1 && k.stride(3) == 1 &&
                           v.stride(3) == 1 && p.scalar_type() == at::kFloat && p.is_contiguous();
    if (shapes_ok) {
        const int64_t B = q.size(0), H = q.size(1), Nq = q.size(2), Nk = k.size(2), G = (Nq + 191) / 192;
        const void *st = nullptr, *gf = nullptr;
        int64_t st_stride = 0, st_rows = 1;
        at::Tensor stc, gfc;
        bool ok = p.numel() == B * H * Nq;
        if (ok && static_mask.has_value() && static_mask->defined()) {
            stc = *static_mask;
            ok = stc.is_cuda() && stc.scalar_type() == at::kBool && stc.dim() == 4 && stc.size(3) == Nk && stc.size(2) == G && stc.size(1) == H &&
                 (stc.size(0) == 1 || stc.size(0) == B) && stc.stride(3) == 1 && stc.stride(1) == G * stc.stride(2) &&
                 (stc.size(0) == 1 || stc.stride(0) == H * stc.stride(1));
            if (ok) st = stc.data_ptr(), st_stride = stc.stride(2), st_rows = stc.size(0) * H * G;
        }
        if (ok && groups.has_value() && groups->defined()) {
            gfc = *groups;
            ok = gfc.is_cuda() && gfc.scalar_type() == at::kBool && gfc.dim() == 4 && gfc.size(3) == 1 && gfc.size(2) == G && gfc.size(1) == H &&
                 (gfc.size(0) == 1 || gfc.size(0) == B);
            if (ok) {
                gfc = gfc.expand({B, H, G, 1}).contiguous();
                gf = gfc.data_ptr();
            }
        }
        if (ok) {
            c10::DeviceGuard guard(q.device());
            at::Tensor o = alloc_o(q, q, token_major_o);
            const int64_t os[3] = {o.stride(0), o.stride(1), o.stride(2)};
            at::Tensor l = at::empty({B, H, Nq, 1}, q.options().dtype(at::kFloat));
            at::Tensor mask = at::empty({B, H, G, Nk}, q.options().dtype(at::kBool));
            const int64_t qs[3] = {q.stride(0), q.stride(1), q.stride(2)}, ks[3] = {k.stride(0), k.stride(1), k.stride(2)},
                          vs[3] = {v.stride(0), v.stride(1), v.stride(2)};
            const int rc = chipmunk_dense_colsum_topk_mask_strided(q.data_ptr(), k.data_ptr(), v.data_ptr(), qs, ks, vs, p.data_ptr<float>(), o.data_ptr(),
                                                           os, l.data_ptr<float>(), (int)B, (int)H, (int)Nq, (int)Nk, st, st_stride, (int)st_rows, gf,
                                                           mask.data_ptr(), (int)k_top, random_amount, cur_stream(q));
            if (rc == CHIPMUNK_OK) return {o, mask, l};
            if (rc != CHIPMUNK_ERR_UNSUPPORTED) check(rc, "dense_colsum_topk_mask");
        }
    }
    auto ocl = dense_colsum_attn_layout(q, k, v, p, token_major_o);
    at::Tensor cs = ocl[1];
    const int64_t Nk = k.size(2), G = (q.size(2) + 191) / 192;
    if (cs.size(-1) != Nk || cs.size(-2) != G) cs = cs.slice(-2, 0, G).slice(-1, 0, Nk);
    return {ocl[0], topk_mask(cs, k_top, random_amount, groups, static_mask), ocl[2]};
}

at::Tensor topk_mask(at::Tensor cs, int64_t k, double random_amount, const c10::optional<at::Tensor> &groups,
                     const c10::optional<at::Tensor> &static_mask) {
    CHECK_DEV(cs); CHECK_BF16(cs);
    TORCH_CHECK(cs.dim() == 4 && cs.stride(3) == 1, "cs must be [B, H, G, N] with a contiguous last dim");
    const int64_t B = cs.size(0), H = cs.size(1), G = cs.size(2), N = cs.size(3);
    if (!(cs.stride(1) == G * cs.stride(2) && (B == 1 || cs.stride(0) == H * cs.stride(1)))) cs = cs.contiguous();
    const int64_t rows = B * H * G;
    c10::DeviceGuard guard(cs.device());
    at::Tensor mask = at::empty({B, H, G, N}, cs.options().dtype(at::kBool));
    const void *st = nullptr, *gf = nullptr;
    int64_t st_stride = 0, st_rows = 1;
    at::Tensor stc, gfc;
    if (static_mask.has_value() && static_mask->defined()) {
        stc = *static_mask;
        CHECK_DEV(stc);
        TORCH_CHECK(stc.scalar_type() == at::kBool && stc.dim() == 4 && stc.size(3) == N && stc.size(2) == G &&
                    stc.size(1) == H && (stc.size(0) == 1 || stc.size(0) == B), "static_mask must be bool [1|B, H, G, N]");
        if (!(stc.stride(3) == 1 && stc.stride(1) == G * stc.stride(2) && (stc.size(0) == 1 || stc.stride(0) == H * stc.stride(1))))
            stc = stc.contiguous();
        st = stc.data_ptr(), st_stride = stc.stride(2), st_rows = stc.size(0) * H * G;
    }
    if (groups.has_value() && groups->defined()) {
        gfc = *groups;
        CHECK_DEV(gfc);
        TORCH_CHECK(gfc.scalar_type() == at::kBool && gfc.dim() == 4 && gfc.size(3) == 1 && gfc.size(2) == G &&
                    gfc.size(1) == H && (gfc.size(0) == 1 || gfc.size(0) == B), "groups must be bool [1|B, H, G, 1]");
        gfc = gfc.expand({B, H, G, 1}).contiguous();
        gf = gfc.data_ptr();
    }
    check(chipmunk_topk_mask(cs.data_ptr(), cs.stride(2), st, st_stride, (int)st_rows, gf, mask.data_ptr(), (int)rows, (int)N,
                             (int)k, random_amount, cur_stream(cs)),
          "topk_mask");
    return mask;
}

at::Tensor bitpack(at::Tensor mask) {
    TORCH_CHECK(mask.scalar_type() == at::kBool, "mask must be bool type");
    CHECK_DEV(mask);
    mask = mask.contiguous();
    c10::DeviceGuard guard(mask.device());
    at::Tensor packed = at::empty({(mask.numel() + 7) / 8}, mask.options().dtype(at::kByte));
    check(chipmunk_bitpack(mask.data_ptr(), packed.data_ptr(), mask.numel(), cur_stream(mask)), "bitpack");
    return packed;
}
at::Tensor bitunpack(at::Tensor packed, at::IntArrayRef shape) {
    TORCH_CHECK(packed.scalar_type() == at::kByte && packed.is_contiguous(), "packed must be a contiguous uint8 tensor");
    CHECK_DEV(packed);
    int64_t n = 1;
    for (auto d : shape) n *= d;
    TORCH_CHECK(packed.numel() * 8 >= n, "packed is too short for the given shape");
    c10::DeviceGuard guard(packed.device());
// ... 80 lines not shown
          "split_heads_rownorm");
    return res;
}

at::Tensor gather_rows(at::Tensor src, at::Tensor map) {
    CHECK_DEV(src);
    CHECK_DEV(map);
    TORCH_CHECK(src.dim() >= 2, "gather_rows: src must be [..., n, d]");
    TORCH_CHECK(map.scalar_type() == at::kInt && map.dim() == 1 && map.is_contiguous(), "gather_rows: map must be a contiguous int32 vector");
    src = src.contiguous();
    const int64_t n_src = src.size(-2), d = src.size(-1), n_out = map.numel();
    const int64_t outer = n_src * d == 0 ? 0 : src.numel() / (n_src * d);
    auto sizes = src.sizes().vec();
    sizes[sizes.size() - 2] = n_out;
    c10::DeviceGuard guard(src.device());
    at::Tensor dst = at::empty(sizes, src.options());
    if (dst.numel() == 0) return dst;
    check(chipmunk_gather_rows(src.data_ptr(), dst.data_ptr(), map.data_ptr<int>(), outer, n_src, n_out,
                               d * (int64_t)src.element_size(), cur_stream(src)),
          "gather_rows");
    return dst;
}

}

TORCH_LIBRARY(chipmunk, m) {
    m.def("csp_mlp_mm1(Tensor a, Tensor b_colmajor, Tensor(c!) c, Tensor bias, Tensor pa_cache_colmajor, Tensor indices, Tensor indices_counts) -> ()");
    m.def("csp_mlp_mm2_and_scatter_add(Tensor packed, Tensor(unpacked_colmajor!) unpacked_colmajor, Tensor sp_inds, Tensor sp_counts, Tensor mma_a, Tensor mma_b, Tensor mma_c, int num_sms_scatter_add, int matmul_kernel) -> ()");

    m.def("csp_attn(Tensor q, Tensor k, Tensor v, Tensor o, Tensor indices, Tensor indices_counts, int o_scale) -> ()");
    m.def("csp_128_attn(Tensor q, Tensor k, Tensor v, Tensor indices, Tensor indices_counts) -> Tensor");
    m.def("dense_attn(Tensor q, Tensor k, Tensor v) -> Tensor[]");
    m.def("dense_colsum_attn(Tensor q, Tensor k, Tensor v, Tensor p) -> Tensor[]");

    m.def("copy_indices(Tensor bmfc1, Tensor(bm_mid_cache!) bm_mid_cache, Tensor sp_inds, Tensor sp_counts) -> ()");
    m.def("topk_indices(Tensor activation, Tensor(indices!) indices, Tensor counts, float sparsity_amount, int multiple_of, float random_amount) -> ()");
    m.def("csp_scatter_add(Tensor packed, Tensor(unpacked_colmajor!) unpacked_colmajor, Tensor sp_inds, Tensor sp_counts, int num_sms) -> ()");
    m.def("mask_to_indices(Tensor mask, int multiple_of, int pad_to_multiple_of) -> Tensor[]");

    m.def("csp_attn_out(Tensor q, Tensor k, Tensor v, Tensor o_in, Tensor indices, Tensor indices_counts, int o_scale) -> Tensor");
    m.def("csp_mlp_mm1_scatter(Tensor a, Tensor b_colmajor, Tensor(c!) c, Tensor bias, Tensor(pa_cache_colmajor!) pa_cache_colmajor, Tensor indices, Tensor indices_counts) -> ()");
    m.def("csp_mlp_mm2(Tensor mma_a, Tensor mma_b, Tensor indices, Tensor counts, Tensor(mma_c!) mma_c) -> ()");
    m.def("csp_mlp_mm1_fp8(Tensor a, Tensor b, Tensor(c!) c, Tensor bias, Tensor(pa_cache_colmajor!) pa_cache_colmajor, Tensor indices, Tensor indices_counts, Tensor scale_a, Tensor scale_b, bool update_cache) -> ()");
    m.def("csp_mlp_mm1_fp8_scatter(Tensor a, Tensor b, Tensor(c!) c, Tensor bias, Tensor(pa_cache_colmajor!) pa_cache_colmajor, Tensor indices, Tensor indices_counts, Tensor scale_a, Tensor scale_b) -> ()");
    m.def("topk_delta_indices(Tensor activation, Tensor(cache!) cache, Tensor(indices!) indices, Tensor(counts!) counts, float sparsity_amount, int multiple_of, float random_amount) -> ()");
    m.def("packed_mask_to_indices(Tensor packed, int[] shape, int multiple_of, int pad_to_multiple_of) -> Tensor[]");
    m.def("mask_to_sorted_indices(Tensor mask, int[] shape, int multiple_of, int pad_to_multiple_of) -> Tensor[]");
    m.def("topk_mask(Tensor cs, int k, float random_amount, Tensor? groups, Tensor? static_mask) -> Tensor");
    m.def("dense_colsum_topk_mask(Tensor q, Tensor k, Tensor v, Tensor p, int k_top, float random_amount, Tensor? groups, Tensor? static_mask, bool token_major_o=False) -> Tensor[]");
    m.def("dense_attn_layout(Tensor q, Tensor k, Tensor v, bool token_major_o) -> Tensor[]");
    m.def("dense_colsum_attn_layout(Tensor q, Tensor k, Tensor v, Tensor p, bool token_major_o) -> Tensor[]");
    m.def("compact_indices(Tensor indices, Tensor counts) -> Tensor[]");
    m.def("mask_to_ragged_indices(Tensor mask, int[] shape, int multiple_of, int pad_to_multiple_of, bool sorted) -> Tensor[]");
    m.def("csp_attn_out_ragged(Tensor q, Tensor k, Tensor v, Tensor o_in, Tensor indices, Tensor offsets, Tensor indices_counts, int o_scale) -> Tensor");
    m.def("residual_ln_modulate(Tensor x, Tensor? y, Tensor? gate, Tensor shift, Tensor scale, float eps) -> Tensor[]");
    m.def("transpose_last2(Tensor x) -> Tensor");
    m.def("transpose_last2_pitched(Tensor x, int ld) -> Tensor");
    m.def("block_mean(Tensor x, int mbm) -> Tensor");
    m.def("quantize_fp8(Tensor x, Tensor scale, float max_value) -> Tensor");
    m.def("bitpack(Tensor mask) -> Tensor");
    m.def("bitunpack(Tensor packed, int[] shape) -> Tensor");
    m.def("gather_rows(Tensor src, Tensor map) -> Tensor");
    m.def("qkv_split_norm(Tensor qkv, Tensor? q_weight, Tensor? k_weight, int heads, float eps, Tensor? freqs_cos=None, Tensor? freqs_sin=None) -> Tensor[]");
    m.def("split_heads_rownorm(Tensor x, int heads, int parts, Tensor? w0, Tensor? w1, Tensor? w2, int norm_mask, int rope_mask, float eps, Tensor? freqs_cos=None, Tensor? freqs_sin=None) -> Tensor[]");
}

TORCH_LIBRARY_IMPL(chipmunk, CUDA, m) {
    m.impl("qkv_split_norm", &qkv_split_norm);
    m.impl("split_heads_rownorm", &split_heads_rownorm);
    m.impl("csp_mlp_mm1_fp8_scatter", &csp_mlp_mm1_fp8_scatter);
    m.impl("dense_colsum_topk_mask", &dense_colsum_topk_mask);
    m.impl("csp_mlp_mm1", &csp_mlp_mm1);
    m.impl("csp_mlp_mm2_and_scatter_add", &csp_mlp_mm2_and_scatter_add);
    m.impl("copy_indices", &copy_indices);
    m.impl("topk_indices", &topk_indices);
    m.impl("csp_scatter_add", &csp_scatter_add);
    m.impl("mask_to_indices", &mask_to_indices);
    m.impl("csp_attn", &csp_attn);
    m.impl("csp_128_attn", &csp_128_attn);
    m.impl("dense_attn", &dense_attn);
    m.impl("dense_colsum_attn", &dense_colsum_attn);
    m.impl("compact_indices", &compact_indices);
    m.impl("residual_ln_modulate", &residual_ln_modulate);
    m.impl("csp_attn_out_ragged", &csp_attn_out_ragged);
    m.impl("dense_attn_layout", &dense_attn_layout);
    m.impl("dense_colsum_attn_layout", &dense_colsum_attn_layout);
    m.impl("csp_attn_out", &csp_attn_out);
    m.impl("csp_mlp_mm1_scatter", &csp_mlp_mm1_scatter);
    m.impl("csp_mlp_mm2", &csp_mlp_mm2);
    m.impl("csp_mlp_mm1_fp8", &csp_mlp_mm1_fp8);
    m.impl("topk_delta_indices", &topk_delta_indices);
    m.impl("packed_mask_to_indices", &packed_mask_to_indices);
    m.impl("mask_to_sorted_indices", &mask_to_sorted_indices);
    m.impl("mask_to_ragged_indices", &mask_to_ragged_indices);
    m.impl("topk_mask", &topk_mask);
    m.impl("transpose_last2", &transpose_last2);
    m.impl("transpose_last2_pitched", &transpose_last2_pitched);
    m.impl("block_mean", &block_mean);
    m.impl("quantize_fp8", &quantize_fp8);
    m.impl("bitpack", &bitpack);
    m.impl("bitunpack", &bitunpack);
    m.impl("gather_rows", &gather_rows);
}

}
```

chipmunk_amd/modules/attn.py:

```python
from __future__ import annotations

from typing import Optional, Tuple

import torch
import torch.nn.functional as F
from torch import Tensor, nn

from .. import ops
from ..ops.voxel import get_local_indices_with_text
from ..util.config import GLOBAL_CONFIG, amd_key
from ..util.layer_counter import LayerCounter
from ..util.storage import AttnStorage
from ..util.storage.offloaded_tensor import release_kept_offloaded, release_resident, reserve_kept_offloaded, reserve_resident

singleton_static_mask: Optional[Tensor] = None
singleton_video_query_groups: Optional[Tensor] = None


def _cdiv(a: int, b: int) -> int:
    return (a + b - 1) // b


def _dense_attn_raw(q: Tensor, k: Tensor, v: Tensor, token_major_o: bool):
    return torch.ops.chipmunk.dense_attn_layout(q, k, v, True) if token_major_o else torch.ops.chipmunk.dense_attn(q, k, v)
# ... 102 lines not shown
    def _stored_mask(self):
        if self.storage.indices.is_suppressed():
            self.storage.indices.suppress_current(False)
            self.storage.indices.load_async()
            self.storage.indices.load_async_wait()
        return self.storage.get_indices(), self.mask_shape[self.layer_counter.cur_model_invocation_per_step]

    @staticmethod
    def _ragged_enabled(x: Tensor) -> bool:
        return bool(x.is_cuda and GLOBAL_CONFIG["attn"]["should_compress_indices"] and amd_key("attn", "fused_residual")
                    and amd_key("attn", "fused_packed_mask_to_indices") and amd_key("attn", "ragged_mask_to_indices"))

    @torch.compiler.disable
    def _ragged_indices(self, packed: Tensor, shape, multiple_of: int, bm: int, mask: Optional[Tensor] = None):
        if shape[-1] % 8 != 0:
            packed = mask if mask is not None else ops.bitunpack(packed, shape)
        return ops.mask_to_ragged_indices(packed, shape, multiple_of, bm, bool(amd_key("attn", "sorted_indices")))

    def _stored_indices(self, multiple_of: int, bm: int):
        cfg = GLOBAL_CONFIG["attn"]
        if cfg["should_compress_indices"]:
            packed, shape = self._stored_mask()
            if amd_key("attn", "fused_packed_mask_to_indices") and packed.is_cuda and shape[-1] % 8 == 0:
                if amd_key("attn", "sorted_indices"):
                    return ops.mask_to_sorted_indices(packed, shape, multiple_of, bm)
                return ops.packed_mask_to_indices(packed, shape, multiple_of, bm)
            return ops.mask_to_indices(ops.bitunpack(packed, shape), multiple_of, bm)
        return self.storage.get_indices(), self.storage.get_counts()

    def _fast_attention(self, q: Tensor, k: Tensor, v: Tensor, inference_step: int, do_full_step: bool) -> Tensor:
        cfg = GLOBAL_CONFIG["attn"]
        bm = cfg["mbm"]
        assert bm == 192, "The kernel was written for BM=192. You may need to change the kernel."
        do_padding = cfg["pad_qkv_before_kernel"]
        multiple_of = 128 if do_padding else cfg["counts_multiple_of"]

        tm = bool(q.is_cuda and amd_key("attn", "token_major_output"))
        use_ragged = self._ragged_enabled(q)
        if self.layer_num < cfg["first_n_dense_layers"]:
            o, _ = ops.dense_attn(q, k, v, tm)
            return o

        if do_full_step:
            if inference_step == 0:
                o, lse = ops.dense_attn(q, k, v, tm) if do_padding else _dense_attn_raw(q, k, v, tm)
                lse[..., k.shape[-2]:, :] = 0
                self.storage.set_lse_constants(lse)
                return o

            ragged = None
            if inference_step == 1 or cfg["recompute_mask"]:
                prev_lse = self.storage.get_lse_constants()
                tk = int(multiple_of * round((cfg["top_keys"] * k.shape[-2]) / multiple_of))
                mask = bs = None
                if (q.is_cuda and cfg["should_compress_indices"] and tk > 0 and amd_key("attn", "fused_colsum_topk")
                        and amd_key("attn", "fused_topk_mask") and k.shape[-2] <= ops.TOPK_MASK_MAX_N):
                    static, groups = self._static(q.shape[1], _cdiv(q.shape[-2], bm), k.shape[-2])
                    o, mask, lse = ops.dense_colsum_topk_mask(q, k, v, prev_lse, tk, 0.01, groups, static, tm)
                elif do_padding:
                    o, bs, lse = ops.dense_colsum_attn(q, k, v, prev_lse, tm)
                else:
                    o, bs, lse = (torch.ops.chipmunk.dense_colsum_attn_layout(q, k, v, prev_lse, True) if tm else
                                  torch.ops.chipmunk.dense_colsum_attn(q, k, v, prev_lse))
                lse[..., k.shape[-2]:, :] = 0
                self.storage.set_lse_constants(lse)
                if cfg["should_compress_indices"]:
                    if mask is not None:
                        pass
                    elif tk > 0:
                        mask = self.random_and_topk(bs, tk)
                    else:
                        mask = self._static(bs.shape[1], bs.shape[-2], bs.shape[-1])[0]
                    packed, mask_shape = ops.bitpack(mask)
                    self.mask_shape[self.layer_counter.cur_model_invocation_per_step] = mask_shape
                    self.storage.set_indices(packed)
                    if use_ragged:
                        ragged = self._ragged_indices(packed, mask_shape, multiple_of, bm, mask)
                        self._remember_indices(None, ragged[2], ragged[:2])
                    else:
                        if mask.is_cuda and amd_key("attn", "fused_packed_mask_to_indices") and amd_key("attn", "sorted_indices"):
                            inds, counts = ops.mask_to_sorted_indices(mask, mask.shape, multiple_of, bm)
                        else:
                            inds, counts = ops.mask_to_indices(mask, multiple_of, bm)
                        self._remember_indices(inds, counts)
                else:
                    kseq = k.shape[-2]
                    bs = bs[..., :_cdiv(kseq, bm), :kseq]
                    inds = torch.topk(bs, k=tk, dim=-1).indices
                    counts = torch.full((q.shape[0], q.shape[1], _cdiv(q.shape[-2], bm)), tk, device=q.device,
                                        dtype=torch.int32)
                    pad = torch.empty((*counts.shape, q.shape[-2] - tk), device=q.device, dtype=torch.int32)
                    inds = torch.cat([inds, pad], dim=-1).to(torch.int32)
                    self.storage.set_indices(inds)
                    self.storage.set_counts(counts)
            else:
                o, _ = ops.dense_attn(q, k, v, tm)

            if use_ragged:
                if ragged is None:
                    ragged = self._ragged_indices(*self._stored_mask(), multiple_of, bm)
            elif not cfg["recompute_mask"]:
                inds, counts = self._stored_indices(multiple_of, bm)

            if ragged is not None:
                o_cache = ops.csp_attn_out_ragged(q, k, v, o, ragged[0], ragged[1], ragged[2], -1)
            elif o.is_cuda and amd_key("attn", "fused_residual"):
                o_cache = ops.csp_attn_out(q, k, v, o, inds, counts, -1)
            elif do_padding:
                o_cache = o - ops.csp_attn(q, k, v, inds, counts)
            else:
                o_cache = o.clone()
                ops.csp_attn_inplace(q, k, v, o_cache, inds, counts, -1)
            self.storage.set_out_cache(o_cache)
            return o

        o = self.storage.get_out_cache()
        kept = self._kept_indices() if (o.is_cuda and amd_key("attn", "fused_residual")) else None
        if kept is not None:
            return ops.csp_attn_out_ragged(q, k, v, o, kept[0], kept[1], kept[2], 1)
# ... 27 lines not shown
```

chipmunk_amd/ops/__init__.py:

```python
from .mlp import run_e2e as mlp
from .indexed_io import (copy_indices, topk_indices, mask_to_indices, scatter_add, packed_mask_to_indices,
                         mask_to_sorted_indices, mask_to_ragged_indices, topk_mask, manual_seed, TOPK_MASK_MAX_N)
from .attn import compact_indices, csp_attn, csp_attn_inplace, csp_attn_out, csp_attn_out_ragged, dense_attn, dense_colsum_attn, dense_colsum_topk_mask
from .patch import patchify, unpatchify, patchify_rope
from .bitpack import bitpack, bitunpack
from . import voxel
from .qkv import qkv_split_norm, residual_ln_modulate, split_heads_rownorm, wan_rope_table

__all__ = ["mlp", "copy_indices", "topk_indices", "mask_to_indices", "scatter_add", "csp_attn", "dense_attn",
           "dense_colsum_attn", "patchify", "unpatchify", "patchify_rope", "bitpack", "bitunpack",
           "packed_mask_to_indices", "mask_to_sorted_indices", "csp_attn_inplace", "csp_attn_out", "topk_mask", "TOPK_MASK_MAX_N", "voxel", "manual_seed", "qkv_split_norm", "dense_colsum_topk_mask", "compact_indices", "csp_attn_out_ragged", "residual_ln_modulate",
           "split_heads_rownorm", "wan_rope_table", "mask_to_ragged_indices"]

from . import _fake
```

chipmunk_amd/ops/_fake.py:

```python
import torch


def _o_like(q, token_major):
    B, H, N, D = q.shape
    return q.new_empty((B, N, H, D)).permute(0, 2, 1, 3) if token_major else q.new_empty((B, H, N, D))


def _register():
    lib = torch.library

    @lib.register_fake("chipmunk::csp_128_attn")
    def _(q, k, v, indices, indices_counts):
        return torch.empty_like(q)

    @lib.register_fake("chipmunk::csp_attn_out")
    def _(q, k, v, o_in, indices, indices_counts, o_scale):
        return torch.empty_like(o_in)

    @lib.register_fake("chipmunk::residual_ln_modulate")
    def _(x, y, gate, shift, scale, eps):
        return [torch.empty_like(x), torch.empty_like(x)] if y is not None else [torch.empty_like(x)]

    @lib.register_fake("chipmunk::csp_attn_out_ragged")
    def _(q, k, v, o_in, indices, offsets, indices_counts, o_scale):
# ... 24 lines not shown
    @lib.register_fake("chipmunk::mask_to_indices")
    def _(mask, multiple_of, pad_to_multiple_of):
        b, h, m, n = mask.shape
        pad_n = (n + pad_to_multiple_of - 1) // pad_to_multiple_of * pad_to_multiple_of
        return [mask.new_empty((b, h, m, pad_n), dtype=torch.int32), mask.new_empty((b, h, m), dtype=torch.int32)]

    @lib.register_fake("chipmunk::packed_mask_to_indices")
    def _(packed, shape, multiple_of, pad_to_multiple_of):
        b, h, m, n = shape
        pad_n = (n + pad_to_multiple_of - 1) // pad_to_multiple_of * pad_to_multiple_of
        return [packed.new_empty((b, h, m, pad_n), dtype=torch.int32), packed.new_empty((b, h, m), dtype=torch.int32)]

    @lib.register_fake("chipmunk::topk_mask")
    def _(cs, k, random_amount, groups, static_mask):
        return cs.new_empty(cs.shape, dtype=torch.bool)

    @lib.register_fake("chipmunk::block_mean")
    def _(x, mbm):
        return x.new_empty((x.shape[0], (x.shape[1] + mbm - 1) // mbm, x.shape[2]))

    @lib.register_fake("chipmunk::transpose_last2")
    def _(x):
        return x.new_empty(x.shape[:-2] + (x.shape[-1], x.shape[-2]))

    @lib.register_fake("chipmunk::transpose_last2_pitched")
    def _(x, ld):
        return x.new_empty(x.shape[:-2] + (x.shape[-1], ld))

    @lib.register_fake("chipmunk::quantize_fp8")
    def _(x, scale, max_value):
        return x.new_empty(x.shape, dtype=torch.float8_e4m3fn)

    @lib.register_fake("chipmunk::bitpack")
    def _(mask):
        return mask.new_empty(((mask.numel() + 7) // 8,), dtype=torch.uint8)

    @lib.register_fake("chipmunk::bitunpack")
    def _(packed, shape):
        return packed.new_empty(tuple(shape), dtype=torch.bool)

    @lib.register_fake("chipmunk::gather_rows")
    def _(src, map):
        shape = list(src.shape)
        shape[-2] = map.shape[0]
        return src.new_empty(shape)

    @lib.register_fake("chipmunk::dense_colsum_topk_mask")
    def _(q, k, v, p, k_top, random_amount, groups, static_mask, token_major_o=False):
        B, H, Nq, D = q.shape
        G = (Nq + 191) // 192
        return [_o_like(q, token_major_o), q.new_empty((B, H, G, k.shape[2]), dtype=torch.bool),
                q.new_empty((B, H, Nq, 1), dtype=torch.float32)]

    @lib.register_fake("chipmunk::qkv_split_norm")
    def _(qkv, q_weight, k_weight, heads, eps, freqs_cos=None, freqs_sin=None):
        out = qkv.new_empty((3, 1, heads, qkv.shape[0], 128))
        return [out[0], out[1], out[2]]

    @lib.register_fake("chipmunk::split_heads_rownorm")
    def _(x, heads, parts, w0, w1, w2, norm_mask, rope_mask, eps, freqs_cos=None, freqs_sin=None):
        out = x.new_empty((parts, x.shape[0] if x.dim() == 3 else 1, heads, x.shape[-2], 128))
        return [out[p] for p in range(parts)]


_register()
```

chipmunk_amd/ops/attn.py:

```python
from __future__ import annotations

from typing import Tuple

import torch
import torch.nn.functional as F

PM = 192


def _pad_len(n: int) -> int:
    return ((n + PM - 1) // PM) * PM


def _last_dim_contiguous(t: torch.Tensor) -> torch.Tensor:
    return t if t.stride(-1) == 1 else t.contiguous()


def dense_attn(q: torch.Tensor, k: torch.Tensor, v: torch.Tensor, token_major_o: bool = False) -> Tuple[torch.Tensor, torch.Tensor]:
    n = q.shape[-2]
    q, k, v = _last_dim_contiguous(q), _last_dim_contiguous(k), _last_dim_contiguous(v)
    o, l = torch.ops.chipmunk.dense_attn_layout(q, k, v, True) if token_major_o else torch.ops.chipmunk.dense_attn(q, k, v)
    padded = _pad_len(n)
    if padded != n:
        l = F.pad(l, (0, 0, 0, padded - n))
    return o, l


def dense_colsum_attn(q: torch.Tensor, k: torch.Tensor, v: torch.Tensor, p: torch.Tensor, token_major_o: bool = False
                      ) -> Tuple[torch.Tensor, torch.Tensor, torch.Tensor]:
    n = q.shape[-2]
    padded = _pad_len(n)
    assert p.shape[-2] in (n, padded), "p must be the l vector of the previous full step"
    p_rows = p[..., :n, :].contiguous()
    q, k, v = _last_dim_contiguous(q), _last_dim_contiguous(k), _last_dim_contiguous(v)
    if token_major_o:
        o, cs, l = torch.ops.chipmunk.dense_colsum_attn_layout(q, k, v, p_rows, True)
    else:
        o, cs, l = torch.ops.chipmunk.dense_colsum_attn(q, k, v, p_rows)
    if padded != n:
        l = F.pad(l, (0, 0, 0, padded - n))
    kseq = k.shape[-2]
    kgroups = (kseq + PM - 1) // PM
    if cs.shape[-2] != kgroups or cs.shape[-1] != kseq:
        cs = cs[..., :kgroups, :kseq]
    return o, cs, l


def dense_colsum_topk_mask(q: torch.Tensor, k: torch.Tensor, v: torch.Tensor, p: torch.Tensor, k_top: int, random_amount: float,
                           groups, static_mask, token_major_o: bool = False) -> Tuple[torch.Tensor, torch.Tensor, torch.Tensor]:
    n = q.shape[-2]
    padded = _pad_len(n)
    assert p.shape[-2] in (n, padded), "p must be the l vector of the previous full step"
    o, mask, l = torch.ops.chipmunk.dense_colsum_topk_mask(_last_dim_contiguous(q), _last_dim_contiguous(k), _last_dim_contiguous(v),
                                                           p[..., :n, :].contiguous(), k_top, random_amount, groups, static_mask,
                                                           token_major_o)
    if padded != n:
        l = F.pad(l, (0, 0, 0, padded - n))
    return o, mask, l


def csp_attn(q: torch.Tensor, k: torch.Tensor, v: torch.Tensor, indices: torch.Tensor,
             indices_counts: torch.Tensor) -> torch.Tensor:
    return torch.ops.chipmunk.csp_128_attn(q.contiguous(), k.contiguous(), v.contiguous(), indices.contiguous(),
                                           indices_counts.contiguous())


def csp_attn_inplace(q: torch.Tensor, k: torch.Tensor, v: torch.Tensor, o: torch.Tensor, indices: torch.Tensor,
                     indices_counts: torch.Tensor, o_scale: int) -> None:
    torch.ops.chipmunk.csp_attn(q, k, v, o, indices, indices_counts, o_scale)


def csp_attn_out(q: torch.Tensor, k: torch.Tensor, v: torch.Tensor, o_in: torch.Tensor, indices: torch.Tensor,
                 indices_counts: torch.Tensor, o_scale: int) -> torch.Tensor:
    return torch.ops.chipmunk.csp_attn_out(q, k, v, o_in, indices, indices_counts, o_scale)


def compact_indices(indices: torch.Tensor, indices_counts: torch.Tensor) -> Tuple[torch.Tensor, torch.Tensor]:
    return tuple(torch.ops.chipmunk.compact_indices(indices.contiguous(), indices_counts.contiguous()))


def csp_attn_out_ragged(q: torch.Tensor, k: torch.Tensor, v: torch.Tensor, o_in: torch.Tensor, indices: torch.Tensor,
                        offsets: torch.Tensor, indices_counts: torch.Tensor, o_scale: int) -> torch.Tensor:
    return torch.ops.chipmunk.csp_attn_out_ragged(q, k, v, o_in, indices, offsets, indices_counts, o_scale)


__all__ = ["csp_attn", "csp_attn_inplace", "csp_attn_out", "csp_attn_out_ragged", "compact_indices", "dense_attn", "dense_colsum_attn",
           "dense_colsum_topk_mask"]
```

chipmunk_amd/ops/indexed_io.py:

```python
from __future__ import annotations

from typing import List, Optional, Sequence

import torch

TOPK_MASK_MAX_N = 1024 * 512


def copy_indices(bm_fc1: torch.Tensor, bm_mid_cache: torch.Tensor, indices: torch.Tensor, counts: torch.Tensor) -> None:
    torch.ops.chipmunk.copy_indices(bm_fc1, bm_mid_cache, indices, counts)


def topk_indices(activations: torch.Tensor, indices_out: torch.Tensor, counts_out: torch.Tensor,
                 sparsity_amount: float, multiple_of: int, rk: float) -> None:
    torch.ops.chipmunk.topk_indices(activations, indices_out, counts_out, sparsity_amount, multiple_of, rk)


def scatter_add(packed: torch.Tensor, unpacked: torch.Tensor, indices: torch.Tensor, counts: torch.Tensor,
                num_sms: int) -> None:
    if packed.ndim == 3:
        torch.ops.chipmunk.csp_scatter_add(packed, unpacked, indices, counts, num_sms)
        return
    torch.ops.chipmunk.csp_scatter_add(packed.unsqueeze(0), unpacked.unsqueeze(0), indices.unsqueeze(0),
                                       counts.unsqueeze(0), num_sms)


def mask_to_indices(mask: torch.Tensor, multiple_of: int, pad_to_multiple_of: int) -> List[torch.Tensor]:
    return torch.ops.chipmunk.mask_to_indices(mask, multiple_of, pad_to_multiple_of)


def packed_mask_to_indices(packed: torch.Tensor, shape: Sequence[int], multiple_of: int,
                           pad_to_multiple_of: int) -> List[torch.Tensor]:
    return torch.ops.chipmunk.packed_mask_to_indices(packed, list(shape), multiple_of, pad_to_multiple_of)


def mask_to_sorted_indices(mask: torch.Tensor, shape: Sequence[int], multiple_of: int,
                           pad_to_multiple_of: int) -> List[torch.Tensor]:
    return torch.ops.chipmunk.mask_to_sorted_indices(mask, list(shape), multiple_of, pad_to_multiple_of)


def mask_to_ragged_indices(mask: torch.Tensor, shape: Sequence[int], multiple_of: int, pad_to_multiple_of: int,
                           sorted: bool = True) -> List[torch.Tensor]:
    if mask.is_cuda:
        return torch.ops.chipmunk.mask_to_ragged_indices(mask, list(shape), multiple_of, pad_to_multiple_of, sorted)
    if mask.dtype == torch.uint8:
        from .bitpack import bitunpack
        mask = bitunpack(mask, shape)
    b, h, m, n = mask.shape
    pad_n = (n + pad_to_multiple_of - 1) // pad_to_multiple_of * pad_to_multiple_of
    rows = mask.reshape(-1, n) != 0
    kept = rows.sum(dim=1)
    counts = (kept + multiple_of - 1) // multiple_of * multiple_of
    lengths = (counts.clamp(max=pad_n) + 31) // 32 * 32
    offsets = torch.zeros(rows.shape[0] + 1, dtype=torch.int64)
    offsets[1:] = lengths.cumsum(0)
    flat = torch.zeros(int(offsets[-1]) + 64, dtype=torch.int32)
    cols = torch.arange(n, dtype=torch.int32)
    for r in range(rows.shape[0]):
        true = cols[rows[r]]
        if not sorted:
            true = true[torch.argsort(true % 32, stable=True)]
        row = torch.cat([true, cols[~rows[r]][:int(counts[r] - kept[r])]])
        flat[int(offsets[r]):int(offsets[r]) + row.numel()] = row
    return [flat, offsets, counts.to(torch.int32).view(b, h, m)]


def topk_mask(cs: torch.Tensor, k: int, random_amount: float = 0.0, groups: Optional[torch.Tensor] = None,
              static_mask: Optional[torch.Tensor] = None) -> torch.Tensor:
    return torch.ops.chipmunk.topk_mask(cs, k, random_amount, groups, static_mask)


def manual_seed(seed: int) -> None:
    from .._native import manual_seed as _seed
    _seed(seed)
```

chipmunk_amd/util/config.py:

```python
from __future__ import annotations

import copy
from typing import Any, Dict

import yaml

BASE_CONFIG: Dict[str, Any] = {
    "num_model_invocations_per_inference_step": 1,
    "should_profile": False,
    "generation_index": 0,
    "steps": 50,
    "world_size": 1,
    "mlp": {
        "is_enabled": True,
        "is_fp8": False,
        "top_keys": "dd",
        "random_keys": 0.05,
        "full_step_every": 10,
        "block_mask_cache": 2,
        "first_n_dense_layers": 2,
        "counts_multiple_of": 256,
        "bm": 128,
        "mbm": 128,
    },
# ... 5 lines not shown
    "attn": {
        "is_enabled": True,
        "top_keys": 0.05,
        "random_keys": 0.01,
        "local_voxels": 0,
        "local_1d_window": 0,
        "first_n_dense_layers": 2,
        "full_step_every": 10,
        "full_step_schedule": None,
        "recompute_mask": True,
        "should_compress_indices": True,
        "counts_multiple_of": 128,
        "pad_qkv_before_kernel": True,
        "mbm": 192,
    },
    "offloading": {
        "global_disable_offloading": False,
        "mlp.out_cache": False,
        "mlp.indices": False,
        "mlp.counts": False,
        "mlp.sparse_act_T": False,
        "mlp.blockmean_mid_cache": False,
        "attn.out_cache": True,
        "attn.indices": True,
        "attn.counts": False,
        "attn.lse_constants": False,
        "text_encoders": True,
    },
    "step_caching": {
        "is_enabled": True,
        "skip_step_schedule": {7, 11, 13, 14, 15, 17, 18, 19, 21, 22, 23, 25, 26, 27, 29, 31, 33, 34, 35, 37, 38, 39,
                               41, 42, 43},
    },
}

AMD_EXTRA_KEYS: Dict[str, Any] = {
    "offloading.keep_resident_if_fits": False,
    "offloading.hbm_budget_gb": 200.0,
    "offloading.native_host_pool": True,
    "attn.fused_packed_mask_to_indices": True,
    "attn.sorted_indices": True,
    "mlp.fused_topk_delta": True,
    "mlp.fused_block_mean": True,
    "mlp.fused_fp8_quantize": True,
    "attn.fused_residual": True,
    "attn.fused_topk_mask": True,
    "attn.fused_colsum_topk": True,
    "mlp.fused_scatter": True,
    "attn.token_major_output": False,
    "attn.keep_unpacked_indices": True,
    "attn.keep_unpacked_indices_offloaded": True,
    "attn.kept_indices_offloaded_budget_gb": 8.0,
    "attn.ragged_mask_to_indices": True,
}
BASE_CONFIG["offloading"]["keep_resident_if_fits"] = AMD_EXTRA_KEYS["offloading.keep_resident_if_fits"]
BASE_CONFIG["offloading"]["hbm_budget_gb"] = AMD_EXTRA_KEYS["offloading.hbm_budget_gb"]
BASE_CONFIG["offloading"]["native_host_pool"] = AMD_EXTRA_KEYS["offloading.native_host_pool"]
BASE_CONFIG["attn"]["fused_packed_mask_to_indices"] = AMD_EXTRA_KEYS["attn.fused_packed_mask_to_indices"]
BASE_CONFIG["attn"]["sorted_indices"] = AMD_EXTRA_KEYS["attn.sorted_indices"]
BASE_CONFIG["mlp"]["fused_topk_delta"] = AMD_EXTRA_KEYS["mlp.fused_topk_delta"]
BASE_CONFIG["attn"]["fused_residual"] = AMD_EXTRA_KEYS["attn.fused_residual"]
BASE_CONFIG["attn"]["fused_topk_mask"] = AMD_EXTRA_KEYS["attn.fused_topk_mask"]
BASE_CONFIG["attn"]["fused_colsum_topk"] = AMD_EXTRA_KEYS["attn.fused_colsum_topk"]
BASE_CONFIG["mlp"]["fused_scatter"] = AMD_EXTRA_KEYS["mlp.fused_scatter"]
BASE_CONFIG["attn"]["token_major_output"] = AMD_EXTRA_KEYS["attn.token_major_output"]
BASE_CONFIG["attn"]["keep_unpacked_indices"] = AMD_EXTRA_KEYS["attn.keep_unpacked_indices"]
BASE_CONFIG["attn"]["keep_unpacked_indices_offloaded"] = AMD_EXTRA_KEYS["attn.keep_unpacked_indices_offloaded"]
BASE_CONFIG["attn"]["kept_indices_offloaded_budget_gb"] = AMD_EXTRA_KEYS["attn.kept_indices_offloaded_budget_gb"]
BASE_CONFIG["attn"]["ragged_mask_to_indices"] = AMD_EXTRA_KEYS["attn.ragged_mask_to_indices"]

GLOBAL_CONFIG: Dict[str, Any] = copy.deepcopy(BASE_CONFIG)


def amd_key(section: str, key: str) -> Any:
    return GLOBAL_CONFIG.get(section, {}).get(key, AMD_EXTRA_KEYS[f"{section}.{key}"])


def update_global_config(config: Dict[str, Any]) -> None:
    GLOBAL_CONFIG.update(config)


def _deep_update(dst: Dict[str, Any], src: Dict[str, Any]) -> None:
    for key, value in src.items():
        if isinstance(value, dict) and isinstance(dst.get(key), dict):
            _deep_update(dst[key], value)
        else:
            dst[key] = value


def load_from_file(config_file: str) -> None:
    with open(config_file, "r") as f:
        loaded = yaml.safe_load(f)
    if loaded:
        _deep_update(GLOBAL_CONFIG, loaded)
        print(f"CHIPMUNK: using config file {config_file}")


def reset_to_base() -> None:
    fresh = copy.deepcopy(BASE_CONFIG)
    GLOBAL_CONFIG.clear()
    GLOBAL_CONFIG.update(fresh)
```

include/chipmunk_hip.h:

```cpp
#ifndef CHIPMUNK_HIP_H
#define CHIPMUNK_HIP_H

#include <stdint.h>

#ifdef __cplusplus
extern "C" {
#endif

#define CHIPMUNK_OK 0
#define CHIPMUNK_ERR_INVALID 1
#define CHIPMUNK_ERR_LAUNCH 2
#define CHIPMUNK_ERR_UNSUPPORTED 3

#define CHIPMUNK_DTYPE_BF16 0
#define CHIPMUNK_DTYPE_FP16 1
#define CHIPMUNK_DTYPE_FP32 2

const char *chipmunk_last_error(void);
int chipmunk_abi_version(void);
int chipmunk_set_option(const char *name, int value);
int chipmunk_set_random_seed(uint64_t seed);

int chipmunk_csp_attn(const void *q, const void *k, const void *v, void *o, const int64_t q_strides[3],
                      const int64_t k_strides[3], const int64_t v_strides[3], const int64_t o_strides[3],
                      const int32_t *indices, const int32_t *counts, int B, int H, int Nq, int Nk, int idx_stride,
                      int o_scale, void *stream);

int chipmunk_csp_attn_out(const void *q, const void *k, const void *v, const void *o_in, void *o_out,
                          const int64_t q_strides[3], const int64_t k_strides[3], const int64_t v_strides[3],
                          const int64_t o_strides[3], const int32_t *indices, const int32_t *counts, int B, int H,
                          int Nq, int Nk, int idx_stride, int o_scale, void *stream);

int chipmunk_csp_attn_out_ragged(const void *q, const void *k, const void *v, const void *o_in, void *o_out,
                                 const int64_t q_strides[3], const int64_t k_strides[3], const int64_t v_strides[3],
                                 const int64_t o_strides[3], const int32_t *indices, const int64_t *idx_offsets,
                                 const int32_t *counts, int B, int H, int Nq, int Nk, int o_scale, void *stream);
int chipmunk_compact_indices(const int32_t *indices, int64_t idx_stride, const int32_t *counts, const int64_t *offsets,
                             int32_t *flat, int64_t rows, void *stream);

int chipmunk_csp_128_attn(const void *q, const void *k, const void *v, void *o, const int32_t *indices,
                          const int32_t *counts, int B, int H, int Nq, int Nk, int idx_stride, void *stream);

int chipmunk_dense_attn(const void *q, const void *k, const void *v, const int64_t q_strides[3],
                        const int64_t k_strides[3], const int64_t v_strides[3], void *o, float *l, int B, int H,
                        int Nq, int Nk, void *stream);

int chipmunk_dense_attn_strided(const void *q, const void *k, const void *v, const int64_t q_strides[3],
                                const int64_t k_strides[3], const int64_t v_strides[3], void *o, const int64_t *o_strides,
                                float *l, int B, int H, int Nq, int Nk, void *stream);
int chipmunk_dense_colsum_attn_strided(const void *q, const void *k, const void *v, const int64_t q_strides[3],
                                       const int64_t k_strides[3], const int64_t v_strides[3], const float *p, void *o,
                                       const int64_t *o_strides, void *cs, float *l, int B, int H, int Nq, int Nk,
                                       int cs_stride, void *stream);
int chipmunk_dense_colsum_topk_mask_strided(const void *q, const void *k, const void *v, const int64_t q_strides[3],
                                            const int64_t k_strides[3], const int64_t v_strides[3], const float *p, void *o,
                                            const int64_t *o_strides, float *l, int B, int H, int Nq, int Nk,
                                            const void *static_mask, int64_t static_stride, int static_rows,
                                            const void *group_flags, void *mask, int k_top, double random_amount, void *stream);

int chipmunk_dense_colsum_attn(const void *q, const void *k, const void *v, const int64_t q_strides[3],
                               const int64_t k_strides[3], const int64_t v_strides[3], const float *p, void *o,
                               void *cs, float *l, int B, int H, int Nq, int Nk, int cs_stride, void *stream);

int chipmunk_residual_ln_modulate(const void *x, const void *y, const void *gate, const void *shift, const void *scale,
                                  void *x_out, void *xm, int64_t rows, int cols, double eps, void *stream);

int chipmunk_csp_mlp_mm1(const void *a, const void *b, void *c, const void *bias, const void *pa_cache,
                         const int32_t *indices, const int32_t *counts, int M, int K, int F, void *stream);

int chipmunk_csp_mlp_mm1_scatter(const void *a, const void *b, void *c, const void *bias, void *pa_cache,
                                 const int32_t *indices, const int32_t *counts, int M, int K, int F, void *stream);

int chipmunk_csp_mlp_mm1_fp8(const void *a, const void *b, void *c, const void *bias, void *pa_cache,
                             const int32_t *indices, const int32_t *counts, const float *scale_a,
                             const float *scale_b, int M, int K, int F, int update_cache, void *stream);

int chipmunk_csp_mlp_mm2_and_scatter_add(const void *packed, void *unpacked_colmajor, const int32_t *indices,
                                         const int32_t *counts, const void *mma_a, const void *mma_b, void *mma_c,
                                         int M, int F, int N2, int num_sms_scatter_add, void *stream);

int chipmunk_csp_scatter_add(const void *packed, void *unpacked_colmajor, const int32_t *indices,
                             const int32_t *counts, int M, int F, int num_sms, void *stream);

int chipmunk_csp_mlp_mm2(const void *mma_a, const void *mma_b, void *mma_c, const int32_t *indices,
                         const int32_t *counts, int M, int F, int N2, void *stream);

int chipmunk_csp_mlp_mm1_ragged(const void *a, const void *b, void *c, const void *bias, const void *pa_cache,
                                const int32_t *indices, const int32_t *counts, int M, int K, int F, int ldc, void *stream);
int chipmunk_csp_mlp_mm1_scatter_ragged(const void *a, const void *b, void *c, const void *bias, void *pa_cache,
                                        const int32_t *indices, const int32_t *counts, int M, int K, int F, int ldc,
                                        void *stream);
int chipmunk_csp_mlp_mm1_fp8_ragged(const void *a, const void *b, void *c, const void *bias, void *pa_cache,
                                    const int32_t *indices, const int32_t *counts, const float *scale_a,
                                    const float *scale_b, int M, int K, int F, int ldc, int update_cache, void *stream);
int chipmunk_csp_mlp_mm2_ragged(const void *mma_a, const void *mma_b, void *mma_c, const int32_t *indices,
                                const int32_t *counts, int M, int F, int N2, void *stream);
int chipmunk_csp_mlp_mm2_and_scatter_add_ragged(const void *packed, void *unpacked_colmajor, const int32_t *indices,
                                                const int32_t *counts, const void *mma_a, const void *mma_b, void *mma_c,
                                                int M, int F, int N2, int ldc, void *stream);
int chipmunk_csp_scatter_add_ragged(const void *packed, void *unpacked_colmajor, const int32_t *indices,
                                    const int32_t *counts, int M, int F, int ldc, void *stream);

int chipmunk_csp_mlp_mm1_batched(const void *a, const void *b, void *c, const void *bias, const void *pa_cache,
                                 const int32_t *indices, const int32_t *counts, int M, int K, int F, int ldc, int B,
                                 int64_t cache_batch_stride, void *stream);
int chipmunk_csp_mlp_mm1_scatter_batched(const void *a, const void *b, void *c, const void *bias, void *pa_cache,
                                         const int32_t *indices, const int32_t *counts, int M, int K, int F, int ldc, int B,
                                         int64_t cache_batch_stride, void *stream);
int chipmunk_csp_mlp_mm1_fp8_batched(const void *a, const void *b, void *c, const void *bias, void *pa_cache,
                                     const int32_t *indices, const int32_t *counts, const float *scale_a, const float *scale_b,
                                     int M, int K, int F, int ldc, int update_cache, int B, int64_t cache_batch_stride,
                                     void *stream);
int chipmunk_csp_mlp_mm2_batched(const void *mma_a, const void *mma_b, void *mma_c, const int32_t *indices,
                                 const int32_t *counts, int M, int F, int N2, int B, void *stream);
int chipmunk_csp_mlp_mm2_and_scatter_add_batched(const void *packed, void *unpacked_colmajor, const int32_t *indices,
                                                 const int32_t *counts, const void *mma_a, const void *mma_b, void *mma_c,
                                                 int M, int F, int N2, int ldc, int B, int64_t cache_batch_stride,
                                                 void *stream);
int chipmunk_csp_scatter_add_batched(const void *packed, void *unpacked_colmajor, const int32_t *indices,
                                     const int32_t *counts, int M, int F, int ldc, int B, int64_t cache_batch_stride,
                                     void *stream);

int chipmunk_topk_indices(const void *activation, int dtype, int32_t *indices, int32_t *counts, int rows, int cols,
                          double sparsity_amount, int multiple_of, double random_amount, void *stream);

int chipmunk_topk_delta_indices(const void *activation, void *cache, int dtype, int32_t *indices, int32_t *counts,
                                int rows, int cols, double sparsity_amount, int multiple_of, double random_amount,
                                void *stream);

int chipmunk_dense_colsum_topk_mask(const void *q, const void *k, const void *v, const int64_t q_strides[3],
                                    const int64_t k_strides[3], const int64_t v_strides[3], const float *p, void *o, float *l,
                                    int B, int H, int Nq, int Nk, const void *static_mask, int64_t static_stride, int static_rows,
                                    const void *group_flags, void *mask, int k_top, double random_amount, void *stream);

int chipmunk_topk_mask(const void *cs, int64_t cs_stride, const void *static_mask, int64_t static_stride,
                       int static_rows, const void *group_flags, void *mask, int rows, int n, int k,
                       double random_amount, void *stream);

int chipmunk_mask_to_indices(const void *mask, int32_t *indices, int32_t *counts, int64_t rows, int n, int pad_n,
                             int multiple_of, void *stream);

int chipmunk_packed_mask_to_indices(const void *packed, int32_t *indices, int32_t *counts, int64_t rows, int n,
                                    int pad_n, int multiple_of, void *stream);

int chipmunk_mask_to_sorted_indices(const void *mask, int packed, int32_t *indices, int32_t *counts, int64_t rows,
                                    int n, int pad_n, int multiple_of, void *stream);

int chipmunk_mask_row_counts(const void *mask, int packed, int32_t *counts, int64_t *lengths, int64_t rows, int n, int pad_n,
                             int multiple_of, void *stream);
int chipmunk_mask_to_ragged_indices(const void *mask, int packed, int sorted, const int64_t *offsets, int32_t *flat, int64_t rows,
                                    int n, int multiple_of, void *stream);

int chipmunk_copy_indices(const void *src, void *dst, const int32_t *inds, const int32_t *counts, int B, int M, int R,
                          int F, int elem_size, void *stream);

int chipmunk_transpose16(const void *src, void *dst, int B, int R, int C, void *stream);
int chipmunk_transpose16_pitched(const void *src, void *dst, int B, int R, int C, int ld, void *stream);

int chipmunk_block_mean(const void *x, void *out, int64_t rows, int C, int mbm, void *stream);
int chipmunk_block_mean_ragged(const void *x, void *out, int64_t rows, int C, int mbm, void *stream);

int chipmunk_quantize_fp8(const void *x, const float *scale, void *out, int64_t n, float max_value, void *stream);

int chipmunk_bitpack(const void *mask, void *packed, int64_t n, void *stream);
int chipmunk_bitunpack(const void *packed, void *mask, int64_t n, void *stream);

int chipmunk_gather_rows(const void *src, void *dst, const int32_t *map, int64_t outer, int64_t n_src, int64_t n_out,
                         int64_t row_bytes, void *stream);

int chipmunk_host_alloc(size_t bytes, void **host_ptr);
int chipmunk_host_free(void *host_ptr);
int chipmunk_copy_d2h_async(void *host_dst, const void *dev_src, size_t bytes, void *stream);
int chipmunk_copy_h2d_async(void *dev_dst, const void *host_src, size_t bytes, void *stream);
size_t chipmunk_host_bytes(void);

int chipmunk_release_scratch(void);
int chipmunk_big_scratch_fallbacks(void);

int chipmunk_qkv_split_norm(const void *qkv, int64_t row_stride, const void *q_weight, const void *k_weight, void *q, void *k,
                            void *v, int64_t n, int heads, float eps, const float *freqs_cos, const float *freqs_sin,
                            int64_t rope_rows, void *stream);

int chipmunk_split_heads_rownorm(const void *x, int64_t batch_stride, int64_t row_stride, int parts, const void *w0, int w0_dtype,
                                 const void *w1, int w1_dtype, const void *w2, int w2_dtype, void *out0, void *out1, void *out2,
                                 unsigned norm_mask, unsigned rope_mask, int64_t B, int64_t n, int heads, float eps,
                                 const float *freqs_cos, const float *freqs_sin, int64_t rope_rows, void *stream);

#ifdef __cplusplus
}
#endif
#endif
```

Baseline: 0.5811.

## Emit bit-packed top-k masks with per-row counts from fused colsum attention

Adds a packed-output variant of the top-k mask kernels. It writes one bit per key instead of one byte and records per-row kept counts, and this variant is enabled by default through a new config flag. Downstream ragged index construction can then take the counts directly instead of recounting the mask, which cuts mask memory traffic and removes a counting pass. The colsum partial-store path in the attention kernel is also made branchless, using masked buffer stores with an out-of-range offset in place of divergent branches, and some LDS padding is added. The cost is extra cross-lane DPP packing work and new code paths that could diverge from the byte-mask semantics.

```diff
diff --git a/chipmunk_amd/_native.py b/chipmunk_amd/_native.py
--- a/chipmunk_amd/_native.py
+++ b/chipmunk_amd/_native.py
@@ -14,7 +14,7 @@
     "chipmunk_csp_mlp_mm2_and_scatter_add_ragged", "chipmunk_csp_scatter_add_ragged", "chipmunk_block_mean_ragged", "chipmunk_transpose16_pitched",
     "chipmunk_csp_mlp_mm1_batched", "chipmunk_csp_mlp_mm1_scatter_batched", "chipmunk_csp_mlp_mm1_fp8_batched", "chipmunk_csp_mlp_mm2_batched",
     "chipmunk_csp_mlp_mm2_and_scatter_add_batched", "chipmunk_csp_scatter_add_batched",
-    "chipmunk_topk_indices", "chipmunk_topk_delta_indices", "chipmunk_topk_mask", "chipmunk_mask_to_indices", "chipmunk_mask_to_sorted_indices", "chipmunk_packed_mask_to_indices", "chipmunk_mask_row_counts", "chipmunk_mask_to_ragged_indices", "chipmunk_copy_indices",
+    "chipmunk_topk_indices", "chipmunk_topk_delta_indices", "chipmunk_topk_mask", "chipmunk_mask_to_indices", "chipmunk_mask_to_sorted_indices", "chipmunk_packed_mask_to_indices", "chipmunk_mask_row_counts", "chipmunk_mask_to_ragged_indices", "chipmunk_bit_counts_to_row_counts", "chipmunk_topk_mask_packed", "chipmunk_dense_colsum_topk_mask_packed_strided", "chipmunk_copy_indices",
     "chipmunk_bitpack", "chipmunk_bitunpack", "chipmunk_transpose16", "chipmunk_block_mean", "chipmunk_quantize_fp8", "chipmunk_gather_rows", "chipmunk_qkv_split_norm", "chipmunk_split_heads_rownorm", "chipmunk_dense_colsum_topk_mask", "chipmunk_dense_attn_strided", "chipmunk_csp_attn_out_ragged", "chipmunk_compact_indices", "chipmunk_residual_ln_modulate", "chipmunk_dense_colsum_attn_strided", "chipmunk_dense_colsum_topk_mask_strided", "chipmunk_release_scratch", "chipmunk_big_scratch_fallbacks",
     "chipmunk_host_alloc", "chipmunk_host_free", "chipmunk_copy_d2h_async", "chipmunk_copy_h2d_async", "chipmunk_host_bytes",
 ]
diff --git a/chipmunk_amd/csrc/attn.hip b/chipmunk_amd/csrc/attn.hip
--- a/chipmunk_amd/csrc/attn.hip
+++ b/chipmunk_amd/csrc/attn.hip
@@ -1238,11 +1238,11 @@
                                               cs_stride, stream);
 }
 
-extern "C" int chipmunk_dense_colsum_topk_mask_strided(const void *q, const void *k, const void *v, const int64_t q_strides[3],
-                                               const int64_t k_strides[3], const int64_t v_strides[3], const float *pin, void *o,
-                                               const int64_t *o_strides, float *l, int B, int H, int Nq, int Nk, const void *static_mask,
-                                               int64_t static_stride, int static_rows, const void *group_flags, void *mask,
-                                               int topk, double random_amount, void *stream) {
+static int dense_colsum_topk_mask_impl(const void *q, const void *k, const void *v, const int64_t q_strides[3],
+                                       const int64_t k_strides[3], const int64_t v_strides[3], const float *pin, void *o,
+                                       const int64_t *o_strides, float *l, int B, int H, int Nq, int Nk, const void *static_mask,
+                                       int64_t static_stride, int static_rows, const void *group_flags, void *mask, int32_t *bit_counts,
+                                       int topk, double random_amount, void *stream) {
     if (int e = check_common(q, k, v, o, B, H, Nq, Nk)) return e;
     CM_CHECK(l && pin && mask, "dense_colsum_topk_mask: p / l / mask missing");
     if (int e = check_strides(q_strides, "q")) return e;
@@ -1264,8 +1264,28 @@
     if (!part) return CHIPMUNK_ERR_UNSUPPORTED;
     if (int e = chipmunk_dense64_colsum_launch(p, part, st)) return e;
     const int nrb = ((Nq + 255) / 256) * 2;
-    return chipmunk_topk_mask_parts(part, chipmunk_colsum_part_stride(Nk), nrb, p.G, Nq, static_mask, static_stride, static_rows, group_flags, mask, B * H * p.G, Nk,
+    return chipmunk_topk_mask_parts(part, chipmunk_colsum_part_stride(Nk), nrb, p.G, Nq, static_mask, static_stride, static_rows, group_flags, mask, bit_counts, B * H * p.G, Nk,
                                     topk, random_amount, st);
+}
+
+extern "C" int chipmunk_dense_colsum_topk_mask_strided(const void *q, const void *k, const void *v, const int64_t q_strides[3],
+                                               const int64_t k_strides[3], const int64_t v_strides[3], const float *pin, void *o,
+                                               const int64_t *o_strides, float *l, int B, int H, int Nq, int Nk, const void *static_mask,
+                                               int64_t static_stride, int static_rows, const void *group_flags, void *mask,
+                                               int topk, double random_amount, void *stream) {
+    return dense_colsum_topk_mask_impl(q, k, v, q_strides, k_strides, v_strides, pin, o, o_strides, l, B, H, Nq, Nk, static_mask, static_stride,
+                                       static_rows, group_flags, mask, nullptr, topk, random_amount, stream);
+}
+
+extern "C" int chipmunk_dense_colsum_topk_mask_packed_strided(const void *q, const void *k, const void *v, const int64_t q_strides[3],
+                                               const int64_t k_strides[3], const int64_t v_strides[3], const float *pin, void *o,
+                                               const int64_t *o_strides, float *l, int B, int H, int Nq, int Nk, const void *static_mask,
+                                               int64_t static_stride, int static_rows, const void *group_flags, void *packed,
+                                               int32_t *bit_counts, int topk, double random_amount, void *stream) {
+    CM_CHECK(packed && bit_counts, "dense_colsum_topk_mask_packed: packed / bit_counts missing");
+    CM_CHECK(Nk % 8 == 0, "dense_colsum_topk_mask_packed: Nk must be a multiple of 8 (got %d)", Nk);
+    return dense_colsum_topk_mask_impl(q, k, v, q_strides, k_strides, v_strides, pin, o, o_strides, l, B, H, Nq, Nk, static_mask, static_stride,
+                                       static_rows, group_flags, packed, bit_counts, topk, random_amount, stream);
 }
 
 extern "C" int chipmunk_dense_colsum_topk_mask(const void *q, const void *k, const void *v, const int64_t q_strides[3],
diff --git a/chipmunk_amd/csrc/attn64.hip b/chipmunk_amd/csrc/attn64.hip
--- a/chipmunk_amd/csrc/attn64.hip
+++ b/chipmunk_amd/csrc/attn64.hip
@@ -16,6 +16,8 @@
 constexpr int PSTAGE = 64 * 128;
 constexpr int LDS_BYTES_CSUM = LDS_BYTES + 4 * PSTAGE;
 constexpr int CS_EXCH_BYTES = 2 * 4 * 64 * 4;
+constexpr int CS_EXCH_PAD = 512;
+constexpr uint32_t CS_NO_STORE = 0x80000000u;
 constexpr float SCALE_LOG2E = 0.08838834764f * 1.44269504089f;
 constexpr float MAX_LAG = 4.0f;
 #ifndef A64_ABL
@@ -29,6 +31,9 @@
 #endif
 #ifndef A64_CSUM_VALU
 #define A64_CSUM_VALU 1
+#endif
+#ifndef A64_CS_NT
+#define A64_CS_NT 0
 #endif
 #ifndef A64_VSPREAD
 #define A64_VSPREAD 0
@@ -336,7 +341,8 @@
         cs_extra = w == lead ? members : 0;
         ex_w = lds0 + LDS_BYTES + (uint32_t)w * 256u + (uint32_t)lane * 4u;
         ex_r = lds0 + LDS_BYTES + (uint32_t)(lead + 1) * 256u + (uint32_t)lane * 4u;
-        prsrc = make_rsrc(p.cs_part + ((int64_t)bh * (p.G * 2) + (g * 2 + (w < nA ? 0 : 1))) * p.cs_pstride);
+        prsrc = make_rsrc(p.cs_part + ((int64_t)bh * (p.G * 2) + (g * 2 + (w < nA ? 0 : 1))) * p.cs_pstride, (uint32_t)p.cs_pstride * 2u);
+        if (!cs_extra) csoff = csoff_mx = CS_NO_STORE;
     }
 #pragma unroll
     for (int e = 0; e < 64; ++e) px[e] = e < 20 ? 0.f : -INFINITY;
@@ -500,24 +506,17 @@
             if constexpr (CSUM && G == (UWT ? 31 : 17)) {
                 const uint32_t par2 = (uint32_t)(t & 1) * 1024u;
                 const float mine = UWT ? csout : c5;
-                if (!cs_extra) {
-                    asm volatile("ds_write_b32 %0, %1" ::"v"(ex_w + (par2 ^ 1024u)), "v"(mine) : "memory");
-                } else {
-                    float x1 = 0.f, x2 = 0.f;
-                    if (cs_extra >= 2) asm volatile("ds_read_b32 %0, %1" : "=v"(x1) : "v"(ex_r + par2) : "memory");
-                    if (cs_extra >= 3) asm volatile("ds_read_b32 %0, %1 offset:256" : "=v"(x2) : "v"(ex_r + par2) : "memory");
-                    asm volatile("ds_write_b32 %0, %1" ::"v"(ex_w + (par2 ^ 1024u)), "v"(mine) : "memory");
-                    asm volatile("s_waitcnt lgkmcnt(1)" : "+v"(x1), "+v"(x2)::"memory");
-                    const int tb2 = tile_base(t - 2), dd = (t - 2) * KT - tb2;
-                    if (t > 1 && dd < KT) {
-                        const uint32_t off = UWT ? csoff_mx : csoff;
-                        if (dd <= 0 || (int)(off >> 1) >= dd) {
-                            const uint16_t val = (uint16_t)(pack_bf16x2((cs_own + x1) + x2, 0.f) & 0xffffu);
-                            if (p.probe & 16) __builtin_amdgcn_raw_buffer_store_b16(val, prsrc, off, (uint32_t)tb2 * 2u, 2);
-                            else __builtin_amdgcn_raw_buffer_store_b16(val, prsrc, off, (uint32_t)tb2 * 2u, 0);
-                        }
-                    }
-                }
+                uint32_t x1, x2;
+                asm volatile("ds_read_b32 %0, %1" : "=v"(x1) : "v"(ex_r + par2) : "memory");
+                asm volatile("ds_read_b32 %0, %1 offset:256" : "=v"(x2) : "v"(ex_r + par2) : "memory");
+                asm volatile("ds_write_b32 %0, %1" ::"v"(ex_w + (par2 ^ 1024u)), "v"(mine) : "memory");
+                asm volatile("s_waitcnt lgkmcnt(1)" : "+v"(x1), "+v"(x2)::"memory");
+                const uint32_t cs_x1 = cs_extra >= 2 ? ~0u : 0u, cs_x2 = cs_extra >= 3 ? ~0u : 0u;
+                const int tb2 = tile_base(t - 2), dd2 = t > 1 ? 2 * ((t - 2) * KT - tb2) : 2 * KT;
+                const uint32_t off = UWT ? csoff_mx : csoff;
+                const uint32_t voff = (int)off >= dd2 ? off : CS_NO_STORE;
+                const uint16_t val = (uint16_t)(pack_bf16x2((cs_own + __uint_as_float(x1 & cs_x1)) + __uint_as_float(x2 & cs_x2), 0.f) & 0xffffu);
+                __builtin_amdgcn_raw_buffer_store_b16(val, prsrc, voff, (uint32_t)(tb2 > 0 ? tb2 : 0) * 2u, A64_CS_NT ? 2 : 0);
                 cs_own = mine;
             }
             if constexpr (!(A64_ABL & 16) && !GATHER && A64_DMA_POS == 1 && G >= 16 && (G & 1) == 0) {
@@ -935,7 +934,7 @@
 int launch64(const AttnParams &p, int64_t grid, hipStream_t stream) {
     auto kern = attn64_kernel<MODE>;
     static uint64_t lds_set = 0;
-    constexpr int LDS = (MODE == 3 && !A64_CSUM_VALU) ? LDS_BYTES_CSUM + CS_EXCH_BYTES : MODE == 3 ? LDS_BYTES + CS_EXCH_BYTES : LDS_BYTES;
+    constexpr int LDS = (MODE == 3 && !A64_CSUM_VALU) ? LDS_BYTES_CSUM + CS_EXCH_BYTES : MODE == 3 ? LDS_BYTES + CS_EXCH_BYTES + CS_EXCH_PAD : LDS_BYTES;
     ensure_dynamic_lds((const void *)kern, LDS, lds_set);
     hipLaunchKernelGGL(kern, dim3((unsigned)grid), dim3(256), LDS, stream, p);
     CM_LAUNCH_CHECK();
@@ -1028,7 +1027,6 @@
     const int G192 = p.G;
     p.G = (p.Nq + WGROWS - 1) / WGROWS;
     p.cs_part = part, p.cs_pstride = chipmunk_colsum_part_stride(p.Nk);
-    if (chipmunk_get_option("attn_cs_probe") & 2) p.probe |= 16;
     if (chipmunk_get_option("attn_fused_colsum") == 3) p.probe |= 4;
     p.kmax = chipmunk_knorm_max(p.k, p.ks, p.B, p.H, p.Nk, stream);
     if (int rc = launch64<3>(p, (int64_t)p.B * p.H * p.G, stream)) return rc;
diff --git a/chipmunk_amd/csrc/attn_params.h b/chipmunk_amd/csrc/attn_params.h
--- a/chipmunk_amd/csrc/attn_params.h
+++ b/chipmunk_amd/csrc/attn_params.h
@@ -30,7 +30,7 @@
 int chipmunk_csp64_launch(const AttnParams &p, int inplace, int grid, hipStream_t stream);
 int chipmunk_dense64_colsum_launch(const AttnParams &p, uint16_t *part, hipStream_t stream);
 int chipmunk_topk_mask_parts(const uint16_t *part, int part_stride, int nrb, int groups_per_bh, int Nq, const void *static_mask, int64_t static_stride,
-                             int static_rows, const void *group_flags, void *mask, int rows, int n, int k, double random_amount,
+                             int static_rows, const void *group_flags, void *mask, int32_t *bit_counts, int rows, int n, int k, double random_amount,
                              hipStream_t stream);
 size_t chipmunk_colsum_part_bytes(int B, int H, int Nq, int Nk);
 int chipmunk_colsum_part_stride(int Nk);
diff --git a/chipmunk_amd/csrc/indexed_io.hip b/chipmunk_amd/csrc/indexed_io.hip
--- a/chipmunk_amd/csrc/indexed_io.hip
+++ b/chipmunk_amd/csrc/indexed_io.hip
@@ -561,14 +561,35 @@
     const uint16_t *parts;
     int64_t pstride;
     int nrb, ngroups, nq;
+    uint8_t *packed;
+    int32_t *bit_counts;
 };
+
+__device__ __forceinline__ void store_packed32(uint8_t *prow, int c, int n, int lane, uint32_t nib) {
+    uint32_t w = nib << (4 * (lane & 7));
+    w |= (uint32_t)__builtin_amdgcn_update_dpp(0, (int)w, 0xB1, 0xf, 0xf, true);
+    w |= (uint32_t)__builtin_amdgcn_update_dpp(0, (int)w, 0x4E, 0xf, 0xf, true);
+    w |= (uint32_t)__builtin_amdgcn_update_dpp(0, (int)w, 0x141, 0xf, 0xf, true);
+    if ((lane & 7) == 0 && c < n) {
+        uint8_t *d = prow + (c >> 3);
+        if (c + 32 <= n) {
+            typedef uint32_t __attribute__((aligned(1))) u32_any;
+            *(u32_any *)d = w;
+        } else {
+#pragma unroll
+            for (int b = 0; b < 3; ++b)
+                if (c + 8 * b < n) d[b] = (uint8_t)(w >> (8 * b));
+        }
+    }
+}
 
 __device__ __forceinline__ uint32_t bf16_key(uint32_t u) {
     return (u & 0x8000u) ? (~u & 0xffffu) : (u | 0x8000u);
 }
 
-template <int KPT, bool ALIGNED, bool PARTS = false>
+template <int KPT, bool ALIGNED, bool PARTS = false, bool PACKED = false>
 __global__ __launch_bounds__(1024) void topk_mask_kernel(const TopkMaskParams p) {
+    static_assert(!PACKED || ALIGNED, "the packed output is a form of the aligned kernel");
     constexpr int NV = KPT / 4;
     __shared__ int wave_cnt[16];
     const int tid = threadIdx.x, lane = tid & 63, w = tid >> 6;
@@ -703,7 +724,8 @@
         __syncthreads();
         tie_budget = ties_to_take - before;
     }
-    uint8_t *out = p.mask + (int64_t)row * n;
+    uint8_t *out = PACKED ? p.packed + (((int64_t)row * n) >> 3) : p.mask + (int64_t)row * n;
+    int kept = 0;
     const uint8_t *st = p.stat ? p.stat + (int64_t)(row % p.stat_rows) * p.stat_stride : nullptr;
     const bool rnd = active && p.random_amount > 0.f;
     auto combined4 = [&](int c0, uint32_t &v0, uint32_t &v1) {
@@ -728,7 +750,7 @@
     }
     const uint32_t salt = p.salt ^ (first * 0x27D4EB2Fu);
     const int nsteps = (n + 4095) / 4096;
-    auto emit = [&](auto keyed, int c, uint32_t v0, uint32_t v1, uint32_t sb) {
+    auto emit = [&](auto keyed, int c, uint32_t v0, uint32_t v1, uint32_t sb) -> uint32_t {
         uint32_t bytes = 0;
         if constexpr (decltype(keyed)::value) asm volatile("" : "+v"(v0), "+v"(v1));
 #pragma unroll
@@ -741,15 +763,18 @@
             keep = keep || tie;
             if (rnd && !keep) keep = hash_uniform(row, c + e, salt) < p.random_amount;
             keep = keep || ((sb >> (8 * e)) & 0xffu) != 0;
-            bytes |= (keep ? 1u : 0u) << (8 * e);
-        }
-        if constexpr (ALIGNED) {
+            bytes |= (keep ? 1u : 0u) << (PACKED ? e : 8 * e);
+        }
+        if constexpr (PACKED) {
+            return bytes;
+        } else if constexpr (ALIGNED) {
             *(uint32_t *)(out + c) = bytes;
         } else {
 #pragma unroll
             for (int e = 0; e < 4; ++e)
                 if (c + e < n) out[c + e] = (uint8_t)(bytes >> (8 * e));
         }
+        return 0u;
     };
     if constexpr (ALIGNED) {
         constexpr int OB = 5;
@@ -766,7 +791,14 @@
             for (int jj = 0; jj < OB; ++jj) {
                 if constexpr (true) {
                     const int c = 4 * tid + 4096 * (j0 + jj);
-                    if (j0 + jj < NV && c < n) emit(std::integral_constant<int, 1>{}, c, key[(j0 + jj) < NV ? (j0 + jj) : 0][0], key[(j0 + jj) < NV ? (j0 + jj) : 0][1], sbv[jj]);
+                    uint32_t nib = 0;
+                    if (j0 + jj < NV && c < n) nib = emit(std::integral_constant<int, 1>{}, c, key[(j0 + jj) < NV ? (j0 + jj) : 0][0], key[(j0 + jj) < NV ? (j0 + jj) : 0][1], sbv[jj]);
+                    if constexpr (PACKED) {
+                        if (j0 + jj < NV && 4096 * (j0 + jj) < n) {
+                            kept += __popc(nib);
+                            store_packed32(out, c, n, lane, nib);
+                        }
+                    }
                     asm volatile("" ::: "memory");
                 }
             }
@@ -787,6 +819,10 @@
             emit(std::integral_constant<int, 0>{}, c, v0, v1, sb);
         }
     }
+    if constexpr (PACKED) {
+        const int total = block_count(kept);
+        if (tid == 0) p.bit_counts[row] = total;
+    }
 }
 
 __device__ __forceinline__ uint32_t bf16_key2(uint32_t u) {
@@ -796,8 +832,9 @@
     return u ^ (s | 0x80008000u);
 }
 
-template <bool ALIGNED, bool PARTS>
+template <bool ALIGNED, bool PARTS, bool PACKED = false>
 __global__ __launch_bounds__(1024) void topk_mask_stream_kernel(const TopkMaskParams p) {
+    static_assert(!PACKED || ALIGNED, "the packed output is a form of the aligned kernel");
     __shared__ int wave_cnt[16];
     const int tid = threadIdx.x, lane = tid & 63, w = tid >> 6;
     const int row = blockIdx.x;
@@ -959,7 +996,8 @@
         __syncthreads();
         tie_budget = ties_to_take - before;
     }
-    uint8_t *out = p.mask + (int64_t)row * n;
+    uint8_t *out = PACKED ? p.packed + (((int64_t)row * n) >> 3) : p.mask + (int64_t)row * n;
+    int kept = 0;
     const uint8_t *st = p.stat ? p.stat + (int64_t)(row % p.stat_rows) * p.stat_stride : nullptr;
     for (int j0 = 0; j0 < nsteps; j0 += U) {
         uint32_t kw[U][2], sbv[U];
@@ -980,7 +1018,9 @@
 #pragma unroll
         for (int jj = 0; jj < U; ++jj) {
             const int c = 4 * tid + 4096 * (j0 + jj);
-            if (c >= n) continue;
+            if constexpr (PACKED) {
+                if (4096 * (j0 + jj) >= n) break;
+            } else if (c >= n) continue;
             if (select) to_keys(kw[jj][0], kw[jj][1]);
             uint32_t bytes = 0;
 #pragma unroll
@@ -992,9 +1032,13 @@
                 keep = keep || tie;
                 if (rnd && !keep) keep = hash_uniform(row, c + e, salt) < p.random_amount;
                 keep = keep || ((sbv[jj] >> (8 * e)) & 0xffu) != 0;
-                bytes |= (keep ? 1u : 0u) << (8 * e);
-            }
-            if constexpr (ALIGNED) {
+                bytes |= (keep ? 1u : 0u) << (PACKED ? e : 8 * e);
+            }
+            if constexpr (PACKED) {
+                if (c >= n) bytes = 0;
+                kept += __popc(bytes);
+                store_packed32(out, c, n, lane, bytes);
+            } else if constexpr (ALIGNED) {
                 *(uint32_t *)(out + c) = bytes;
             } else {
 #pragma unroll
@@ -1002,6 +1046,10 @@
                     if (c + e < n) out[c + e] = (uint8_t)(bytes >> (8 * e));
             }
         }
+    }
+    if constexpr (PACKED) {
+        const int total = block_count(kept);
+        if (tid == 0) p.bit_counts[row] = total;
     }
 }
 
@@ -1183,17 +1231,28 @@
 }
 
 int chipmunk_topk_mask_parts(const uint16_t *part, int part_stride, int nrb, int groups_per_bh, int Nq, const void *static_mask, int64_t static_stride,
-                             int static_rows, const void *group_flags, void *mask, int rows, int n, int k, double random_amount,
+                             int static_rows, const void *group_flags, void *mask, int32_t *bit_counts, int rows, int n, int k, double random_amount,
                              hipStream_t s) {
     CM_CHECK(part && mask && rows >= 0 && n > 0 && (n & 3) == 0 && n <= CHIPMUNK_TOPK_MASK_MAX_N && k >= 0 && part_stride >= n && (part_stride & 3) == 0, "topk_mask_parts: bad arguments");
     CM_CHECK(!static_mask || (static_rows > 0 && static_stride >= n && (static_stride & 3) == 0 && ((uintptr_t)static_mask & 3) == 0),
              "topk_mask_parts: bad static mask geometry");
-    CM_CHECK(((uintptr_t)mask & 3) == 0 && ((uintptr_t)part & 7) == 0, "topk_mask_parts: unaligned buffers");
+    CM_CHECK((bit_counts || ((uintptr_t)mask & 3) == 0) && ((uintptr_t)part & 7) == 0, "topk_mask_parts: unaligned buffers");
+    CM_CHECK(!bit_counts || n % 8 == 0, "topk_mask_parts: n must be a multiple of 8 for the packed output (got %d)", n);
     if (rows == 0) return CHIPMUNK_OK;
     TopkMaskParams p = {nullptr, (const uint8_t *)static_mask, (const uint8_t *)group_flags, (uint8_t *)mask, 0, static_stride,
                         rows, n, k, static_mask ? static_rows : 1, (float)random_amount,
                         random_amount > 0.0 ? chipmunk_next_random_salt() : 0u};
     p.parts = part, p.pstride = part_stride, p.nrb = nrb, p.ngroups = groups_per_bh, p.nq = Nq;
+    const bool stream_form = n > 1024 * 120 || chipmunk_get_option("topk_mask_stream") == 1;
+    if (bit_counts) {
+        p.mask = nullptr, p.packed = (uint8_t *)mask, p.bit_counts = bit_counts;
+        if (stream_form) hipLaunchKernelGGL((topk_mask_stream_kernel<true, true, true>), dim3(rows), dim3(1024), 0, s, p);
+        else if (n <= 1024 * 16) hipLaunchKernelGGL((topk_mask_kernel<16, true, true, true>), dim3(rows), dim3(1024), 0, s, p);
+        else if (n <= 1024 * 48) hipLaunchKernelGGL((topk_mask_kernel<48, true, true, true>), dim3(rows), dim3(1024), 0, s, p);
+        else hipLaunchKernelGGL((topk_mask_kernel<120, true, true, true>), dim3(rows), dim3(1024), 0, s, p);
+        CM_LAUNCH_CHECK();
+        return CHIPMUNK_OK;
+    }
     if (n > 1024 * 120 || chipmunk_get_option("topk_mask_stream") == 1) hipLaunchKernelGGL((topk_mask_stream_kernel<true, true>), dim3(rows), dim3(1024), 0, s, p);
     else if (n <= 1024 * 16) hipLaunchKernelGGL((topk_mask_kernel<16, true, true>), dim3(rows), dim3(1024), 0, s, p);
     else if (n <= 1024 * 48) hipLaunchKernelGGL((topk_mask_kernel<48, true, true>), dim3(rows), dim3(1024), 0, s, p);
@@ -1298,6 +1357,58 @@
     return CHIPMUNK_OK;
 }
 
+extern "C" int chipmunk_topk_mask_packed(const void *cs, int64_t cs_stride, const void *static_mask, int64_t static_stride,
+                                         int static_rows, const void *group_flags, void *packed, int32_t *bit_counts, int rows, int n, int k,
+                                         double random_amount, void *stream) {
+    CM_CHECK(cs && packed && bit_counts, "topk_mask_packed: null pointer");
+    CM_CHECK(rows >= 0 && n > 0 && k >= 0, "topk_mask_packed: bad sizes (rows=%d n=%d k=%d)", rows, n, k);
+    CM_CHECK(n % 8 == 0, "topk_mask_packed: n must be a multiple of 8 (got %d)", n);
+    CM_CHECK(cs_stride >= n, "topk_mask_packed: cs row stride %lld < n %d", (long long)cs_stride, n);
+    CM_CHECK(n <= CHIPMUNK_TOPK_MASK_MAX_N, "topk_mask_packed: rows of more than %d columns are not supported (got %d)", CHIPMUNK_TOPK_MASK_MAX_N, n);
+    CM_CHECK(!static_mask || (static_rows > 0 && static_stride >= n), "topk_mask_packed: bad static mask geometry");
+    CM_CHECK(random_amount >= 0.0 && random_amount <= 1.0, "topk_mask_packed: random_amount must be in [0,1]");
+    CM_CHECK((((uintptr_t)cs) & 7) == 0 && (cs_stride * 2) % 8 == 0 && (!static_mask || ((((uintptr_t)static_mask) & 3) == 0 && static_stride % 4 == 0)),
+             "topk_mask_packed: unaligned rows (cs rows on 8 bytes, static mask rows on 4)");
+    if (rows == 0) return CHIPMUNK_OK;
+    TopkMaskParams p = {(const uint16_t *)cs, (const uint8_t *)static_mask, (const uint8_t *)group_flags, nullptr,
+                        cs_stride, static_stride, rows, n, k, static_mask ? static_rows : 1, (float)random_amount,
+                        random_amount > 0.0 ? chipmunk_next_random_salt() : 0u};
+    p.packed = (uint8_t *)packed, p.bit_counts = bit_counts;
+    hipStream_t s = (hipStream_t)stream;
+    if (n > 1024 * 120 || chipmunk_get_option("topk_mask_stream") == 1) hipLaunchKernelGGL((topk_mask_stream_kernel<true, false, true>), dim3(rows), dim3(1024), 0, s, p);
+    else if (n <= 1024 * 16) hipLaunchKernelGGL((topk_mask_kernel<16, true, false, true>), dim3(rows), dim3(1024), 0, s, p);
+    else if (n <= 1024 * 48) hipLaunchKernelGGL((topk_mask_kernel<48, true, false, true>), dim3(rows), dim3(1024), 0, s, p);
+    else hipLaunchKernelGGL((topk_mask_kernel<120, true, false, true>), dim3(rows), dim3(1024), 0, s, p);
+    CM_LAUNCH_CHECK();
+    return CHIPMUNK_OK;
+}
+
+__global__ __launch_bounds__(256) void counts_from_bits_kernel(const int32_t *bits, int32_t *counts, int64_t *lengths, int64_t rows, int pad_n,
+                                                               int multiple_of) {
+    const int64_t row = (int64_t)blockIdx.x * 256 + threadIdx.x;
+    if (row >= rows) return;
+    const int64_t kept = (uint32_t)bits[row];
+    const int64_t padded = ((kept + multiple_of - 1) / multiple_of) * multiple_of;
+    counts[row] = (int32_t)padded;
+    lengths[row] = (min(padded, (int64_t)pad_n) + 31) / 32 * 32;
+}
+
+extern "C" int chipmunk_bit_counts_to_row_counts(const int32_t *bit_counts, int32_t *counts, int64_t *lengths, int64_t rows, int n, int pad_n,
+                                                 int multiple_of, void *stream) {
+    CM_CHECK(bit_counts && counts && lengths, "bit_counts_to_row_counts: null pointer");
+    CM_CHECK(rows >= 0 && n > 0 && pad_n >= n && multiple_of > 0, "bit_counts_to_row_counts: bad sizes rows=%lld n=%d pad_n=%d multiple_of=%d",
+             (long long)rows, n, pad_n, multiple_of);
+    CM_CHECK(rows < (1ll << 31), "bit_counts_to_row_counts: too many rows");
+    CM_CHECK(n % 8 == 0, "bit_counts_to_row_counts: n must be a multiple of 8 for a packed mask (got %d)", n);
+    const size_t lds = m2i_lds_bytes(n, true);
+    CM_CHECK(lds <= 160 * 1024, "mask_to_indices: row length %d needs %zu B of LDS (> 160 KiB)", n, lds);
+    if (rows == 0) return CHIPMUNK_OK;
+    hipLaunchKernelGGL(counts_from_bits_kernel, dim3((unsigned)((rows + 255) / 256)), dim3(256), 0, (hipStream_t)stream, bit_counts, counts, lengths,
+                       rows, pad_n, multiple_of);
+    CM_LAUNCH_CHECK();
+    return CHIPMUNK_OK;
+}
+
 extern "C" int chipmunk_compact_indices(const int32_t *indices, int64_t idx_stride, const int32_t *counts, const int64_t *offsets,
                                         int32_t *flat, int64_t rows, void *stream) {
     CM_CHECK(indices && counts && offsets && flat, "compact_indices: null pointer");
diff --git a/chipmunk_amd/csrc/torch_registry.cpp b/chipmunk_amd/csrc/torch_registry.cpp
--- a/chipmunk_amd/csrc/torch_registry.cpp
+++ b/chipmunk_amd/csrc/torch_registry.cpp
@@ -696,12 +696,41 @@
     return {flat, offsets, counts};
 }
 
+std::vector<at::Tensor> mask_to_ragged_indices_counted(at::Tensor packed, at::IntArrayRef shape, at::Tensor bit_counts, int64_t multiple_of,
+                                                       int64_t pad_to_multiple_of, bool sorted) {
+    CHECK_DEV(packed); CHECK_DEV(bit_counts);
+    TORCH_CHECK(packed.scalar_type() == at::kByte && bit_counts.scalar_type() == at::kInt, "packed must be uint8 and bit_counts int32");
+    TORCH_CHECK(multiple_of > 0 && pad_to_multiple_of > 0, "multiple_of and pad_to_multiple_of must be positive");
+    TORCH_CHECK(shape.size() == 4, "shape must be [b, h, m, n]");
+    packed = packed.contiguous();
+    bit_counts = bit_counts.contiguous();
+    const int64_t b = shape[0], h = shape[1], m = shape[2], n = shape[3], rows = b * h * m;
+    TORCH_CHECK(n % 8 == 0 && packed.numel() * 8 >= rows * n && bit_counts.numel() == rows, "bad packed mask or bit counts");
+    const int64_t pad_n = ((n + pad_to_multiple_of - 1) / pad_to_multiple_of) * pad_to_multiple_of;
+    TORCH_CHECK(n > 0 && pad_n <= INT_MAX, "rows must have between 1 and 2^31 - 1 columns");
+    c10::DeviceGuard guard(packed.device());
+    at::Tensor counts = at::empty({b, h, m}, packed.options().dtype(at::kInt));
+    at::Tensor len = at::empty({rows}, packed.options().dtype(at::kLong));
+    check(chipmunk_bit_counts_to_row_counts(bit_counts.data_ptr<int>(), counts.data_ptr<int>(), len.data_ptr<int64_t>(), rows, (int)n, (int)pad_n,
+                                            (int)multiple_of, cur_stream(packed)),
+          "mask_to_ragged_indices_counted");
+    at::Tensor offsets = at::zeros({rows + 1}, len.options());
+    if (rows) offsets.narrow(0, 1, rows).copy_(len.cumsum(0));
+    const int64_t total = rows ? offsets[rows].item<int64_t>() : 0;
+    at::Tensor flat = at::empty({total + 64}, counts.options());
+    flat.narrow(0, total, 64).zero_();
+    check(chipmunk_mask_to_ragged_indices(packed.data_ptr(), 1, sorted ? 1 : 0, offsets.data_ptr<int64_t>(), flat.data_ptr<int>(), rows, (int)n,
+                                          (int)multiple_of, cur_stream(packed)),
+          "mask_to_ragged_indices_counted");
+    return {flat, offsets, counts};
+}
+
 std::vector<at::Tensor> dense_colsum_attn_layout(at::Tensor q, at::Tensor k, at::Tensor v, at::Tensor p, bool token_major_o);
 at::Tensor topk_mask(at::Tensor cs, int64_t k, double random_amount, const c10::optional<at::Tensor> &groups,
                      const c10::optional<at::Tensor> &static_mask);
-std::vector<at::Tensor> dense_colsum_topk_mask(at::Tensor q, at::Tensor k, at::Tensor v, at::Tensor p, int64_t k_top, double random_amount,
-                                               const c10::optional<at::Tensor> &groups, const c10::optional<at::Tensor> &static_mask,
-                                               bool token_major_o) {
+static std::vector<at::Tensor> dense_colsum_topk_mask_any(at::Tensor q, at::Tensor k, at::Tensor v, at::Tensor p, int64_t k_top, double random_amount,
+                                                          const c10::optional<at::Tensor> &groups, const c10::optional<at::Tensor> &static_mask,
+                                                          bool token_major_o, bool packed_out) {
     CHECK_DEV(q); CHECK_DEV(k); CHECK_DEV(v); CHECK_DEV(p);
     CHECK_BF16(q); CHECK_BF16(k); CHECK_BF16(v);
     const bool shapes_ok = q.dim() == 4 && k.dim() == 4 && v.dim() == 4 && q.size(3) == 128 && q.stride(3) == 1 && k.stride(3) == 1 &&
@@ -733,13 +762,18 @@
             at::Tensor o = alloc_o(q, q, token_major_o);
             const int64_t os[3] = {o.stride(0), o.stride(1), o.stride(2)};
             at::Tensor l = at::empty({B, H, Nq, 1}, q.options().dtype(at::kFloat));
-            at::Tensor mask = at::empty({B, H, G, Nk}, q.options().dtype(at::kBool));
+            at::Tensor mask = packed_out ? at::empty({B, H, G, Nk / 8}, q.options().dtype(at::kByte)) : at::empty({B, H, G, Nk}, q.options().dtype(at::kBool));
+            at::Tensor bits = packed_out ? at::empty({B, H, G}, q.options().dtype(at::kInt)) : at::Tensor();
             const int64_t qs[3] = {q.stride(0), q.stride(1), q.stride(2)}, ks[3] = {k.stride(0), k.stride(1), k.stride(2)},
                           vs[3] = {v.stride(0), v.stride(1), v.stride(2)};
-            const int rc = chipmunk_dense_colsum_topk_mask_strided(q.data_ptr(), k.data_ptr(), v.data_ptr(), qs, ks, vs, p.data_ptr<float>(), o.data_ptr(),
+            const int rc = packed_out
+                ? chipmunk_dense_colsum_topk_mask_packed_strided(q.data_ptr(), k.data_ptr(), v.data_ptr(), qs, ks, vs, p.data_ptr<float>(), o.data_ptr(),
+                                                                 os, l.data_ptr<float>(), (int)B, (int)H, (int)Nq, (int)Nk, st, st_stride, (int)st_rows, gf,
+                                                                 mask.data_ptr(), bits.data_ptr<int>(), (int)k_top, random_amount, cur_stream(q))
+                : chipmunk_dense_colsum_topk_mask_strided(q.data_ptr(), k.data_ptr(), v.data_ptr(), qs, ks, vs, p.data_ptr<float>(), o.data_ptr(),
                                                            os, l.data_ptr<float>(), (int)B, (int)H, (int)Nq, (int)Nk, st, st_stride, (int)st_rows, gf,
                                                            mask.data_ptr(), (int)k_top, random_amount, cur_stream(q));
-            if (rc == CHIPMUNK_OK) return {o, mask, l};
+            if (rc == CHIPMUNK_OK) return packed_out ? std::vector<at::Tensor>{o, mask, bits, l} : std::vector<at::Tensor>{o, mask, l};
             if (rc != CHIPMUNK_ERR_UNSUPPORTED) check(rc, "dense_colsum_topk_mask");
         }
     }
@@ -747,7 +781,24 @@
     at::Tensor cs = ocl[1];
     const int64_t Nk = k.size(2), G = (q.size(2) + 191) / 192;
     if (cs.size(-1) != Nk || cs.size(-2) != G) cs = cs.slice(-2, 0, G).slice(-1, 0, Nk);
-    return {ocl[0], topk_mask(cs, k_top, random_amount, groups, static_mask), ocl[2]};
+    at::Tensor mask = topk_mask(cs, k_top, random_amount, groups, static_mask);
+    if (!packed_out) return {ocl[0], mask, ocl[2]};
+    at::Tensor packed = at::empty({mask.size(0), mask.size(1), mask.size(2), Nk / 8}, mask.options().dtype(at::kByte));
+    check(chipmunk_bitpack(mask.data_ptr(), packed.data_ptr(), mask.numel(), cur_stream(mask)), "bitpack");
+    return {ocl[0], packed, mask.sum({-1}, false, at::kInt), ocl[2]};
+}
+
+std::vector<at::Tensor> dense_colsum_topk_mask(at::Tensor q, at::Tensor k, at::Tensor v, at::Tensor p, int64_t k_top, double random_amount,
+                                               const c10::optional<at::Tensor> &groups, const c10::optional<at::Tensor> &static_mask,
+                                               bool token_major_o) {
+    return dense_colsum_topk_mask_any(q, k, v, p, k_top, random_amount, groups, static_mask, token_major_o, false);
+}
+
+std::vector<at::Tensor> dense_colsum_topk_mask_packed(at::Tensor q, at::Tensor k, at::Tensor v, at::Tensor p, int64_t k_top, double random_amount,
+                                                      const c10::optional<at::Tensor> &groups, const c10::optional<at::Tensor> &static_mask,
+                                                      bool token_major_o) {
+    TORCH_CHECK(k.dim() == 4 && k.size(2) % 8 == 0, "dense_colsum_topk_mask_packed: the number of keys must be a multiple of 8");
+    return dense_colsum_topk_mask_any(q, k, v, p, k_top, random_amount, groups, static_mask, token_major_o, true);
 }
 
 at::Tensor topk_mask(at::Tensor cs, int64_t k, double random_amount, const c10::optional<at::Tensor> &groups,
@@ -934,6 +985,8 @@
     m.def("dense_colsum_attn_layout(Tensor q, Tensor k, Tensor v, Tensor p, bool token_major_o) -> Tensor[]");
     m.def("compact_indices(Tensor indices, Tensor counts) -> Tensor[]");
     m.def("mask_to_ragged_indices(Tensor mask, int[] shape, int multiple_of, int pad_to_multiple_of, bool sorted) -> Tensor[]");
+    m.def("mask_to_ragged_indices_counted(Tensor packed, int[] shape, Tensor bit_counts, int multiple_of, int pad_to_multiple_of, bool sorted) -> Tensor[]");
+    m.def("dense_colsum_topk_mask_packed(Tensor q, Tensor k, Tensor v, Tensor p, int k_top, float random_amount, Tensor? groups, Tensor? static_mask, bool token_major_o=False) -> Tensor[]");
     m.def("csp_attn_out_ragged(Tensor q, Tensor k, Tensor v, Tensor o_in, Tensor indices, Tensor offsets, Tensor indices_counts, int o_scale) -> Tensor");
     m.def("residual_ln_modulate(Tensor x, Tensor? y, Tensor? gate, Tensor shift, Tensor scale, float eps) -> Tensor[]");
     m.def("transpose_last2(Tensor x) -> Tensor");
@@ -975,6 +1028,8 @@
     m.impl("packed_mask_to_indices", &packed_mask_to_indices);
     m.impl("mask_to_sorted_indices", &mask_to_sorted_indices);
     m.impl("mask_to_ragged_indices", &mask_to_ragged_indices);
+    m.impl("mask_to_ragged_indices_counted", &mask_to_ragged_indices_counted);
+    m.impl("dense_colsum_topk_mask_packed", &dense_colsum_topk_mask_packed);
     m.impl("topk_mask", &topk_mask);
     m.impl("transpose_last2", &transpose_last2);
     m.impl("transpose_last2_pitched", &transpose_last2_pitched);
diff --git a/chipmunk_amd/modules/attn.py b/chipmunk_amd/modules/attn.py
--- a/chipmunk_amd/modules/attn.py
+++ b/chipmunk_amd/modules/attn.py
@@ -178,11 +178,15 @@
             if inference_step == 1 or cfg["recompute_mask"]:
                 prev_lse = self.storage.get_lse_constants()
                 tk = int(multiple_of * round((cfg["top_keys"] * k.shape[-2]) / multiple_of))
-                mask = bs = None
+                mask = bs = packed_sel = None
                 if (q.is_cuda and cfg["should_compress_indices"] and tk > 0 and amd_key("attn", "fused_colsum_topk")
                         and amd_key("attn", "fused_topk_mask") and k.shape[-2] <= ops.TOPK_MASK_MAX_N):
                     static, groups = self._static(q.shape[1], _cdiv(q.shape[-2], bm), k.shape[-2])
-                    o, mask, lse = ops.dense_colsum_topk_mask(q, k, v, prev_lse, tk, 0.01, groups, static, tm)
+                    if use_ragged and k.shape[-2] % 8 == 0 and amd_key("attn", "packed_selection"):
+                        o, packed, bit_counts, lse = ops.dense_colsum_topk_mask(q, k, v, prev_lse, tk, 0.01, groups, static, tm, packed=True)
+                        packed_sel = (packed, bit_counts, (q.shape[0], q.shape[1], _cdiv(q.shape[-2], bm), k.shape[-2]))
+                    else:
+                        o, mask, lse = ops.dense_colsum_topk_mask(q, k, v, prev_lse, tk, 0.01, groups, static, tm)
                 elif do_padding:
                     o, bs, lse = ops.dense_colsum_attn(q, k, v, prev_lse, tm)
                 else:
@@ -190,7 +194,15 @@
                                   torch.ops.chipmunk.dense_colsum_attn(q, k, v, prev_lse))
                 lse[..., k.shape[-2]:, :] = 0
                 self.storage.set_lse_constants(lse)
-                if cfg["should_compress_indices"]:
+                if packed_sel is not None:
+                    packed, bit_counts, mask_shape = packed_sel
+                    self.mask_shape[self.layer_counter.cur_model_invocation_per_step] = mask_shape
+                    packed = packed.view(-1)
+                    self.storage.set_indices(packed)
+                    ragged = ops.mask_to_ragged_indices(packed, mask_shape, multiple_of, bm, bool(amd_key("attn", "sorted_indices")),
+                                                        bit_counts=bit_counts)
+                    self._remember_indices(None, ragged[2], ragged[:2])
+                elif cfg["should_compress_indices"]:
                     if mask is not None:
                         pass
                     elif tk > 0:
diff --git a/chipmunk_amd/ops/__init__.py b/chipmunk_amd/ops/__init__.py
--- a/chipmunk_amd/ops/__init__.py
+++ b/chipmunk_amd/ops/__init__.py
@@ -1,7 +1,7 @@
 from .mlp import run_e2e as mlp
 from .indexed_io import (copy_indices, topk_indices, mask_to_indices, scatter_add, packed_mask_to_indices,
-                         mask_to_sorted_indices, mask_to_ragged_indices, topk_mask, manual_seed, TOPK_MASK_MAX_N)
-from .attn import compact_indices, csp_attn, csp_attn_inplace, csp_attn_out, csp_attn_out_ragged, dense_attn, dense_colsum_attn, dense_colsum_topk_mask
+                         mask_to_sorted_indices, mask_to_ragged_indices, packed_bits_and_counts, topk_mask, manual_seed, TOPK_MASK_MAX_N)
+from .attn import compact_indices, csp_attn, csp_attn_inplace, csp_attn_out, csp_attn_out_ragged, dense_attn, dense_colsum_attn, dense_colsum_topk_mask, dense_colsum_topk_mask_packed
 from .patch import patchify, unpatchify, patchify_rope
 from .bitpack import bitpack, bitunpack
 from . import voxel
@@ -10,6 +10,7 @@
 __all__ = ["mlp", "copy_indices", "topk_indices", "mask_to_indices", "scatter_add", "csp_attn", "dense_attn",
            "dense_colsum_attn", "patchify", "unpatchify", "patchify_rope", "bitpack", "bitunpack",
            "packed_mask_to_indices", "mask_to_sorted_indices", "csp_attn_inplace", "csp_attn_out", "topk_mask", "TOPK_MASK_MAX_N", "voxel", "manual_seed", "qkv_split_norm", "dense_colsum_topk_mask", "compact_indices", "csp_attn_out_ragged", "residual_ln_modulate",
-           "split_heads_rownorm", "wan_rope_table", "mask_to_ragged_indices"]
+           "split_heads_rownorm", "wan_rope_table", "mask_to_ragged_indices", "packed_bits_and_counts",
+           "dense_colsum_topk_mask_packed"]
 
 from . import _fake
diff --git a/chipmunk_amd/ops/_fake.py b/chipmunk_amd/ops/_fake.py
--- a/chipmunk_amd/ops/_fake.py
+++ b/chipmunk_amd/ops/_fake.py
@@ -100,6 +100,13 @@
         return [_o_like(q, token_major_o), q.new_empty((B, H, G, k.shape[2]), dtype=torch.bool),
                 q.new_empty((B, H, Nq, 1), dtype=torch.float32)]
 
+    @lib.register_fake("chipmunk::dense_colsum_topk_mask_packed")
+    def _(q, k, v, p, k_top, random_amount, groups, static_mask, token_major_o=False):
+        B, H, Nq, D = q.shape
+        G = (Nq + 191) // 192
+        return [_o_like(q, token_major_o), q.new_empty((B, H, G, k.shape[2] // 8), dtype=torch.uint8),
+                q.new_empty((B, H, G), dtype=torch.int32), q.new_empty((B, H, Nq, 1), dtype=torch.float32)]
+
     @lib.register_fake("chipmunk::qkv_split_norm")
     def _(qkv, q_weight, k_weight, heads, eps, freqs_cos=None, freqs_sin=None):
         out = qkv.new_empty((3, 1, heads, qkv.shape[0], 128))
diff --git a/chipmunk_amd/ops/attn.py b/chipmunk_amd/ops/attn.py
--- a/chipmunk_amd/ops/attn.py
+++ b/chipmunk_amd/ops/attn.py
@@ -47,7 +47,9 @@
 
 
 def dense_colsum_topk_mask(q: torch.Tensor, k: torch.Tensor, v: torch.Tensor, p: torch.Tensor, k_top: int, random_amount: float,
-                           groups, static_mask, token_major_o: bool = False) -> Tuple[torch.Tensor, torch.Tensor, torch.Tensor]:
+                           groups, static_mask, token_major_o: bool = False, packed: bool = False):
+    if packed:
+        return dense_colsum_topk_mask_packed(q, k, v, p, k_top, random_amount, groups, static_mask, token_major_o)
     n = q.shape[-2]
     padded = _pad_len(n)
     assert p.shape[-2] in (n, padded), "p must be the l vector of the previous full step"
@@ -57,6 +59,19 @@
     if padded != n:
         l = F.pad(l, (0, 0, 0, padded - n))
     return o, mask, l
+
+
+def dense_colsum_topk_mask_packed(q: torch.Tensor, k: torch.Tensor, v: torch.Tensor, p: torch.Tensor, k_top: int, random_amount: float,
+                                  groups, static_mask, token_major_o: bool = False):
+    n = q.shape[-2]
+    padded = _pad_len(n)
+    assert p.shape[-2] in (n, padded), "p must be the l vector of the previous full step"
+    o, packed, bit_counts, l = torch.ops.chipmunk.dense_colsum_topk_mask_packed(
+        _last_dim_contiguous(q), _last_dim_contiguous(k), _last_dim_contiguous(v), p[..., :n, :].contiguous(), k_top, random_amount, groups,
+        static_mask, token_major_o)
+    if padded != n:
+        l = F.pad(l, (0, 0, 0, padded - n))
+    return o, packed, bit_counts, l
 
 
 def csp_attn(q: torch.Tensor, k: torch.Tensor, v: torch.Tensor, indices: torch.Tensor,
@@ -85,4 +100,4 @@
 
 
 __all__ = ["csp_attn", "csp_attn_inplace", "csp_attn_out", "csp_attn_out_ragged", "compact_indices", "dense_attn", "dense_colsum_attn",
-           "dense_colsum_topk_mask"]
+           "dense_colsum_topk_mask", "dense_colsum_topk_mask_packed"]
diff --git a/chipmunk_amd/ops/indexed_io.py b/chipmunk_amd/ops/indexed_io.py
--- a/chipmunk_amd/ops/indexed_io.py
+++ b/chipmunk_amd/ops/indexed_io.py
@@ -40,7 +40,9 @@
 
 
 def mask_to_ragged_indices(mask: torch.Tensor, shape: Sequence[int], multiple_of: int, pad_to_multiple_of: int,
-                           sorted: bool = True) -> List[torch.Tensor]:
+                           sorted: bool = True, bit_counts: Optional[torch.Tensor] = None) -> List[torch.Tensor]:
+    if mask.is_cuda and bit_counts is not None and mask.dtype == torch.uint8:
+        return torch.ops.chipmunk.mask_to_ragged_indices_counted(mask, list(shape), bit_counts, multiple_of, pad_to_multiple_of, sorted)
     if mask.is_cuda:
         return torch.ops.chipmunk.mask_to_ragged_indices(mask, list(shape), multiple_of, pad_to_multiple_of, sorted)
     if mask.dtype == torch.uint8:
@@ -65,6 +67,14 @@
     return [flat, offsets, counts.to(torch.int32).view(b, h, m)]
 
 
+def packed_bits_and_counts(mask: torch.Tensor):
+    n = mask.shape[-1]
+    assert n % 8 == 0
+    bits = (mask != 0).reshape(*mask.shape[:-1], n // 8, 8).to(torch.int32)
+    weights = (1 << torch.arange(8, dtype=torch.int32, device=mask.device))
+    return (bits * weights).sum(-1).to(torch.uint8), (mask != 0).sum(-1, dtype=torch.int32)
+
+
 def topk_mask(cs: torch.Tensor, k: int, random_amount: float = 0.0, groups: Optional[torch.Tensor] = None,
               static_mask: Optional[torch.Tensor] = None) -> torch.Tensor:
     return torch.ops.chipmunk.topk_mask(cs, k, random_amount, groups, static_mask)
diff --git a/chipmunk_amd/util/config.py b/chipmunk_amd/util/config.py
--- a/chipmunk_amd/util/config.py
+++ b/chipmunk_amd/util/config.py
@@ -81,6 +81,7 @@
     "attn.keep_unpacked_indices_offloaded": True,
     "attn.kept_indices_offloaded_budget_gb": 8.0,
     "attn.ragged_mask_to_indices": True,
+    "attn.packed_selection": True,
 }
 BASE_CONFIG["offloading"]["keep_resident_if_fits"] = AMD_EXTRA_KEYS["offloading.keep_resident_if_fits"]
 BASE_CONFIG["offloading"]["hbm_budget_gb"] = AMD_EXTRA_KEYS["offloading.hbm_budget_gb"]
@@ -97,6 +98,7 @@
 BASE_CONFIG["attn"]["keep_unpacked_indices_offloaded"] = AMD_EXTRA_KEYS["attn.keep_unpacked_indices_offloaded"]
 BASE_CONFIG["attn"]["kept_indices_offloaded_budget_gb"] = AMD_EXTRA_KEYS["attn.kept_indices_offloaded_budget_gb"]
 BASE_CONFIG["attn"]["ragged_mask_to_indices"] = AMD_EXTRA_KEYS["attn.ragged_mask_to_indices"]
+BASE_CONFIG["attn"]["packed_selection"] = AMD_EXTRA_KEYS["attn.packed_selection"]
 
 GLOBAL_CONFIG: Dict[str, Any] = copy.deepcopy(BASE_CONFIG)
 
diff --git a/include/chipmunk_hip.h b/include/chipmunk_hip.h
--- a/include/chipmunk_hip.h
+++ b/include/chipmunk_hip.h
@@ -57,6 +57,12 @@
                                             const int64_t *o_strides, float *l, int B, int H, int Nq, int Nk,
                                             const void *static_mask, int64_t static_stride, int static_rows,
                                             const void *group_flags, void *mask, int k_top, double random_amount, void *stream);
+int chipmunk_dense_colsum_topk_mask_packed_strided(const void *q, const void *k, const void *v, const int64_t q_strides[3],
+                                                   const int64_t k_strides[3], const int64_t v_strides[3], const float *p, void *o,
+                                                   const int64_t *o_strides, float *l, int B, int H, int Nq, int Nk,
+                                                   const void *static_mask, int64_t static_stride, int static_rows,
+                                                   const void *group_flags, void *packed, int32_t *bit_counts, int k_top,
+                                                   double random_amount, void *stream);
 
 int chipmunk_dense_colsum_attn(const void *q, const void *k, const void *v, const int64_t q_strides[3],
                                const int64_t k_strides[3], const int64_t v_strides[3], const float *p, void *o,
@@ -150,6 +156,11 @@
                              int multiple_of, void *stream);
 int chipmunk_mask_to_ragged_indices(const void *mask, int packed, int sorted, const int64_t *offsets, int32_t *flat, int64_t rows,
                                     int n, int multiple_of, void *stream);
+int chipmunk_bit_counts_to_row_counts(const int32_t *bit_counts, int32_t *counts, int64_t *lengths, int64_t rows, int n, int pad_n,
+                                      int multiple_of, void *stream);
+int chipmunk_topk_mask_packed(const void *cs, int64_t cs_stride, const void *static_mask, int64_t static_stride, int static_rows,
+                              const void *group_flags, void *packed, int32_t *bit_counts, int rows, int n, int k, double random_amount,
+                              void *stream);
 
 int chipmunk_copy_indices(const void *src, void *dst, const int32_t *inds, const int32_t *counts, int B, int M, int R,
                           int F, int elem_size, void *stream);
```

Result: no change. 0.5813, median of 2 (+0.0%).
